# ecpoppenheimer/TensorFlowRayTrace

Hardware: AMD Instinct MI355X
Metric: ray-surface intersection tests/sec (fwd+bwd) (higher is better)
Workload: dtype f32 ray state, f32 filter + f64 decisions

## Files before the change

### include/tfrt_hip.h

```cpp
#ifndef TFRT_HIP_H
#define TFRT_HIP_H

#include <stddef.h>
#include <stdint.h>

#ifdef __cplusplus
extern "C" {
#endif

#define TFRT_VERSION 107

#define TFRT_F32 0
#define TFRT_F64 1
#define TFRT_F16 2

#define TFRT_OPTICAL 0
#define TFRT_STOP 1
#define TFRT_TARGET 2

#define TFRT_CLS_ACTIVE 0
#define TFRT_CLS_FINISHED 1
#define TFRT_CLS_STOPPED 2
#define TFRT_CLS_DEAD 3

#define TFRT_COMPILE_ACTIVE 1u
#define TFRT_COMPILE_FINISHED 2u
#define TFRT_COMPILE_STOPPED 4u
#define TFRT_COMPILE_DEAD 8u

#define TFRT_E_BADARG (-1)
#define TFRT_E_WORKSPACE (-2)
#define TFRT_E_LAUNCH (-3)
#define TFRT_E_UNSUPPORTED (-4)

int tfrt_version(void);
const char* tfrt_strerror(int code);

int tfrt_build_faces_forward(const double* vertices, int64_t n_vertices, const int32_t* faces,
                             int64_t n_faces, double* face_verts, double* norm, void* stream);

int tfrt_build_faces_backward(const double* grad_face_verts, const double* grad_norm,
                              const double* face_verts, const int32_t* faces,
                              const uint8_t* update_mask, int64_t n_faces, int64_t n_vertices,
                              const int32_t* corner_start, const int32_t* corner_list,
                              double* grad_vertices, void* stream);

int tfrt_param_faces_forward(const double* zero_points, const double* vectors,
                             const double* parameters, int64_t n_vertices, const int32_t* faces,
                             int64_t n_faces, double* face_verts, double* norm, void* stream);
int tfrt_param_faces_backward(const double* grad_face_verts, const double* grad_norm,
                              const double* face_verts, const int32_t* faces,
                              const uint8_t* update_mask, const double* vectors, int64_t n_faces,
                              int64_t n_vertices, const int32_t* corner_start,
                              const int32_t* corner_list, double* grad_parameters, void* stream);

#define TFRT_MAX_SURFACES 8
typedef struct tfrt_face_surface {
  const double* zero_points;
  const double* vectors;
  const double* parameters;
  const int32_t* faces;
  int64_t n_vertices, n_faces;
  double* face_verts;
  double* norm;
  const double* copy_from;
} tfrt_face_surface;
typedef struct tfrt_face_surface_grad {
  const double* grad_face_verts;
  const double* grad_norm;
  const double* face_verts;
  const uint8_t* update_mask;
  const double* vectors;
  const int32_t* corner_start;
  const int32_t* corner_list;
  int64_t n_vertices;
  double* grad_parameters;
} tfrt_face_surface_grad;
int tfrt_param_faces_forward_multi(const tfrt_face_surface* surfaces, int32_t n_surfaces,
                                   void* stream);
int tfrt_param_faces_backward_multi(const tfrt_face_surface_grad* surfaces, int32_t n_surfaces,
                                    void* stream);

int tfrt_sgd_process(const void* grad, void* processed, void* param, int64_t n, int32_t dtype,
                     double scale, double clip, double sgd_learning_rate, void* stream);

int tfrt_sgd_process_dev(const void* grad, void* processed, void* param, int64_t n, int32_t dtype,
                         const double* hyper, void* stream);

typedef struct tfrt_goal_pending {
  const double* partial;
  int32_t n_partial;
  const int32_t* n_finished;
  int32_t n_fields;
  double* error_out;
  const int32_t* tests_lo_hi;
  int64_t* tests_total;
  const int32_t* partial_counts;
  int64_t n_faces;
  int32_t* counts_tail;
} tfrt_goal_pending;

int tfrt_sgd_process_multi(int32_t n_tensors, const void* const* grad, void* const* processed,
                           void* const* param, const int64_t* n, const double* hyper,
                           void* stream);

int tfrt_sgd_process_multi_finish(int32_t n_tensors, const void* const* grad,
                                  void* const* processed, void* const* param, const int64_t* n,
                                  const double* hyper, const tfrt_goal_pending* pending,
                                  void* stream);

int tfrt_sgd_momentum_multi(int32_t n_tensors, const void* const* grad, void* const* processed,
                            void* const* param, void* const* velocity, const int64_t* n,
                            const double* hyper, void* stream);

int tfrt_sgd_momentum_multi_finish(int32_t n_tensors, const void* const* grad,
                                   void* const* processed, void* const* param,
                                   void* const* velocity, const int64_t* n, const double* hyper,
                                   const tfrt_goal_pending* pending, void* stream);

int tfrt_adam_multi(int32_t n_tensors, const void* const* grad, void* const* processed,
                    void* const* param, void* const* m, void* const* v, const int64_t* n,
                    const double* hyper, double* state, uint32_t* ticket, void* stream);

int tfrt_adam_multi_finish(int32_t n_tensors, const void* const* grad, void* const* processed,
                           void* const* param, void* const* m, void* const* v, const int64_t* n,
                           const double* hyper, double* state, uint32_t* ticket,
                           const tfrt_goal_pending* pending, void* stream);

int tfrt_csr_matvec(const int64_t* crow_indices, const int64_t* col_indices, const double* values,
                    const double* x, double* y, int64_t n_rows, void* stream);

typedef struct tfrt_scene3d {
  const double* face_verts;
  const int32_t* catagory;
  const int32_t* mat_in;
  const int32_t* mat_out;
  const double* n_in;
  const double* n_out;
  int64_t n_faces;
  const double* n_table;
  int64_t n_table_stride;
  int32_t n_materials;
  double intersect_epsilion;
  double size_epsilion;
  double ray_start_epsilion;
  const uint8_t* face_grad_mask;
  const int32_t* cluster_order;
  int32_t n_table_uniform;
  int32_t deterministic;
  int32_t coherent_rays;
  int32_t coherent_only;
  double* grad_n_in;
  double* grad_n_out;
  double* clear_buffer;
  int64_t clear_count;
  int32_t in_place;
  const int32_t* ray_slot;
  const int32_t* wave_schedule;
} tfrt_scene3d;

typedef struct tfrt_ray_out {
  void* rays;
  int32_t* ray_id;
  int32_t* face;
  int64_t capacity;
} tfrt_ray_out;

size_t tfrt_trace3d_workspace_bytes(int64_t n_rays, int64_t n_faces, int32_t max_passes,
                                    int32_t state_dtype);

#define TFRT_COUNTS_PER_PASS 8
#define TFRT_COUNTS_LEN(max_passes) (8 * ((max_passes) + 1))

int tfrt_trace3d_forward(const void* src_rays, int64_t src_stride, int64_t n_rays,
                         const tfrt_scene3d* scene, double new_ray_length,
                         double dead_ray_length, int32_t max_passes, int32_t state_dtype,
                         uint32_t flags, tfrt_ray_out* finished, tfrt_ray_out* active,
                         tfrt_ray_out* stopped, tfrt_ray_out* dead, void* unfinished,
                         int32_t* unfinished_id, int32_t* counts, void* workspace,
                         size_t workspace_bytes, void* stream);

int tfrt_trace3d_compact(const void* src_rays, int64_t src_stride, int64_t n_rays,
                         double dead_ray_length, int32_t max_passes, int32_t state_dtype,
                         uint32_t flags, tfrt_ray_out* finished, tfrt_ray_out* active,
                         tfrt_ray_out* stopped, tfrt_ray_out* dead, void* unfinished,
                         int32_t* unfinished_id, int32_t* counts, int64_t n_faces,
                         const int32_t* ray_slot, void* workspace, size_t workspace_bytes,
                         void* stream);

int tfrt_trace3d_in_place(const tfrt_scene3d* scene, int64_t n_rays, int32_t max_passes);

int tfrt_trace3d_executed(int64_t n_rays, int64_t n_faces, int32_t max_passes, int32_t state_dtype,
                          const void* workspace, size_t workspace_bytes, int64_t* executed,
                          void* stream);

int tfrt_trace3d_wave_schedule(int64_t n_rays, int64_t n_faces, int32_t max_passes,
                               int32_t state_dtype, const void* workspace, size_t workspace_bytes,
                               int32_t* schedule_out, void* stream);

int tfrt_trace3d_wave_rows(int64_t n_rays, int64_t n_faces, int32_t max_passes, int32_t state_dtype,
                           const void* workspace, size_t workspace_bytes, uint32_t* rows_out,
                           void* stream);

int tfrt_trace3d_backward(const void* src_rays, int64_t src_stride, int64_t n_rays,
                          const tfrt_scene3d* scene, double new_ray_length,
                          double dead_ray_length, int32_t max_passes, int32_t state_dtype,
                          const double* grad_finished, int64_t cap_finished,
                          const double* grad_active, int64_t cap_active,
                          const double* grad_stopped, int64_t cap_stopped,
                          const double* grad_dead, int64_t cap_dead, double* grad_face_verts,
                          double* grad_src_rays, const int32_t* counts, void* workspace,
                          size_t workspace_bytes, void* stream);

size_t tfrt_goal_error3d_workspace_bytes(int64_t capacity);
int tfrt_goal_error3d(const void* finished_rays, int64_t capacity, const int32_t* finished_id,
                      int32_t state_dtype, const int32_t* counts, int32_t max_passes,
                      const int32_t* fields, int32_t n_fields, const double* goal,
                      int64_t goal_stride, int64_t goal_ray_stride, double* grad_finished,
                      double* error_out, double* zero_buffer, int64_t zero_count,
                      int64_t* tests_total, void* workspace, size_t workspace_bytes,
                      void* stream);

int tfrt_goal_error3d_deferred(const void* finished_rays, int64_t capacity,
                               const int32_t* finished_id, int32_t state_dtype,
                               const int32_t* counts, int32_t max_passes, const int32_t* fields,
                               int32_t n_fields, const double* goal, int64_t goal_stride,
                               int64_t goal_ray_stride, double* grad_finished, double* error_out,
                               double* zero_buffer, int64_t zero_count, int64_t* tests_total,
                               void* workspace, size_t workspace_bytes,
                               tfrt_goal_pending* pending, void* stream);
int tfrt_goal_finish(const tfrt_goal_pending* pending, void* stream);

size_t tfrt_density_error_workspace_bytes(int64_t n, int32_t nx, int32_t ny);
int tfrt_density_error(const void* rows, int64_t stride, int64_t n, int32_t state_dtype,
                       const int32_t* mask, int32_t row_x, int32_t row_y, const double* goal,
                       int32_t nx, int32_t ny, double x0, double x1, double sx, double y0,
                       double y1, double sy, double oob_weight, double* grad, int64_t grad_stride,
                       double* error_out, int64_t* hq, int32_t splat_variant, void* workspace,
                       size_t workspace_bytes, void* stream);

int tfrt_density_error_fields(const void* rows, int64_t stride, int64_t n, int32_t state_dtype,
                              int32_t dimension, const int32_t* mask, int32_t field_x,
                              int32_t field_y, const double* goal, int32_t nx, int32_t ny,
                              double x0, double x1, double sx, double y0, double y1, double sy,
                              double oob_weight, double* grad, int64_t grad_stride,
                              double* error_out, int64_t* hq, int32_t splat_variant,
                              void* workspace, size_t workspace_bytes, void* stream);

size_t tfrt_spot_error_workspace_bytes(int64_t n, int32_t n_groups);
int tfrt_spot_error(const void* rows, int64_t stride, int64_t n, int32_t state_dtype,
                    const int32_t* mask, int32_t row_x, int32_t row_y, const int32_t* group,
                    int64_t n_source, const int32_t* perm, int32_t n_groups, double x0, double x1,
                    double qsx, double y0, double y1, double qsy, int32_t qbits,
                    double oob_weight, double* grad, int64_t grad_stride, double* error_out,
                    int64_t* acc, int32_t variant, void* workspace, size_t workspace_bytes,
                    void* stream);

int tfrt_spot_error_fields(const void* rows, int64_t stride, int64_t n, int32_t state_dtype,
                           int32_t dimension, const int32_t* mask, int32_t field_x,
                           int32_t field_y, const int32_t* group, int64_t n_source,
                           const int32_t* perm, int32_t n_groups, double x0, double x1, double qsx,
                           double y0, double y1, double qsy, int32_t qbits, double oob_weight,
                           double* grad, int64_t grad_stride, double* error_out, int64_t* acc,
                           int32_t variant, void* workspace, size_t workspace_bytes, void* stream);

int tfrt_density_error_weighted(const void* rows, int64_t stride, int64_t n, int32_t state_dtype,
                                int32_t dimension, const int32_t* mask, int32_t field_x,
                                int32_t field_y, const double* goal, const double* weight,
                                int64_t n_source, const int32_t* perm, int32_t nx, int32_t ny,
                                double x0, double x1, double sx, double y0, double y1, double sy,
                                double oob_weight, double* grad, int64_t grad_stride,
                                double* error_out, int64_t* hq, int32_t splat_variant,
                                void* workspace, size_t workspace_bytes, void* stream);

size_t tfrt_spot_error_weighted_workspace_bytes(int64_t n, int32_t n_groups);
int tfrt_spot_error_weighted(const void* rows, int64_t stride, int64_t n, int32_t state_dtype,
                             int32_t dimension, const int32_t* mask, int32_t field_x,
                             int32_t field_y, const int32_t* group, const double* weight,
                             int32_t wbits, int64_t n_source, const int32_t* perm,
                             int32_t n_groups, double x0, double x1, double qsx, double y0,
                             double y1, double qsy, int32_t qbits, double oob_weight, double* grad,
                             int64_t grad_stride, double* error_out, int64_t* acc, int32_t variant,
                             void* workspace, size_t workspace_bytes, void* stream);

size_t tfrt_trace3d_backward_goal_workspace_bytes(int64_t n_rays);
int tfrt_trace3d_backward_goal(const void* src_rays, int64_t src_stride, int64_t n_rays,
                               const tfrt_scene3d* scene, double new_ray_length,
                               double dead_ray_length, int32_t max_passes, int32_t state_dtype,
                               const tfrt_ray_out* finished, const int32_t* fields,
                               int32_t n_fields, const double* goal, int64_t goal_stride,
                               int64_t goal_ray_stride, double* error_out, int64_t* tests_total,
                               void* goal_workspace, size_t goal_workspace_bytes,
                               tfrt_goal_pending* pending, const double* grad_active,
                               int64_t cap_active, const double* grad_stopped,
                               int64_t cap_stopped, const double* grad_dead, int64_t cap_dead,
                               double* grad_face_verts, double* grad_src_rays,
                               const int32_t* counts, void* workspace, size_t workspace_bytes,
                               void* stream);

#define TFRT_PROF_INTERSECT 0
#define TFRT_PROF_REACT 1
#define TFRT_PROF_BACKWARD 2
#define TFRT_PROF_ACCUMULATE 3
int tfrt_profile_enable(int enable);
int tfrt_profile_read(float* ms, int32_t max_records);
int tfrt_profile_read_kind(int32_t kind, float* ms, int32_t max_records);


size_t tfrt_intersect3d_workspace_bytes(int64_t n_rays, int64_t n_faces);
int tfrt_intersect3d(const void* rays, int64_t stride, int64_t n_rays, int32_t state_dtype,
                     const double* face_verts, int64_t n_faces, double intersect_epsilion,
// ... 279 lines not shown
```

### tensorflowraytrace_amd/_lib.py

```python
import ctypes
import os
import typing

HERE = os.path.dirname(os.path.abspath(__file__))
LIB_PATH = os.environ.get("TFRT_LIB_PATH") or os.path.join(HERE, "libtfrt_hip.so")

ABI_VERSION = 107
F32, F64, F16 = 0, 1, 2
OPTICAL, STOP, TARGET = 0, 1, 2
CLS_ACTIVE, CLS_FINISHED, CLS_STOPPED, CLS_DEAD = 0, 1, 2, 3
COMPILE_ACTIVE, COMPILE_FINISHED, COMPILE_STOPPED, COMPILE_DEAD = 1, 2, 4, 8
COUNTS_PER_PASS = 8

c_i32, c_i64, c_f64, c_u32 = ctypes.c_int32, ctypes.c_int64, ctypes.c_double, ctypes.c_uint32
c_vp, c_sz = ctypes.c_void_p, ctypes.c_size_t


class Scene3D(ctypes.Structure):
    _fields_ = [
        ("face_verts", c_vp), ("catagory", c_vp), ("mat_in", c_vp), ("mat_out", c_vp),
        ("n_in", c_vp), ("n_out", c_vp), ("n_faces", c_i64),
        ("n_table", c_vp), ("n_table_stride", c_i64), ("n_materials", c_i32),
        ("intersect_epsilion", c_f64), ("size_epsilion", c_f64), ("ray_start_epsilion", c_f64),
        ("face_grad_mask", c_vp), ("cluster_order", c_vp), ("n_table_uniform", c_i32),
        ("deterministic", c_i32), ("coherent_rays", c_i32), ("coherent_only", c_i32),
        ("grad_n_in", c_vp), ("grad_n_out", c_vp), ("clear_buffer", c_vp), ("clear_count", c_i64),
        ("in_place", c_i32), ("ray_slot", c_vp), ("wave_schedule", c_vp),
    ]


class Scene2D(ctypes.Structure):
    _fields_ = [
        ("seg", c_vp), ("seg_cat", c_vp), ("seg_mat_in", c_vp), ("seg_mat_out", c_vp),
        ("seg_n_in", c_vp), ("seg_n_out", c_vp), ("n_segments", c_i64),
        ("arc", c_vp), ("arc_cat", c_vp), ("arc_mat_in", c_vp), ("arc_mat_out", c_vp),
        ("arc_n_in", c_vp), ("arc_n_out", c_vp), ("n_arcs", c_i64),
        ("n_table", c_vp), ("n_table_stride", c_i64), ("n_materials", c_i32),
        ("intersect_epsilion", c_f64), ("size_epsilion", c_f64), ("ray_start_epsilion", c_f64),
        ("finite_tir_gradient", c_i32),
        ("grad_seg_n_in", c_vp), ("grad_seg_n_out", c_vp),
        ("grad_arc_n_in", c_vp), ("grad_arc_n_out", c_vp),
        ("deterministic", c_i32),
    ]


MAX_SURFACES = 8


class FaceSurface(ctypes.Structure):
    _fields_ = [("zero_points", ctypes.c_void_p), ("vectors", ctypes.c_void_p),
                ("parameters", ctypes.c_void_p), ("faces", ctypes.c_void_p),
                ("n_vertices", ctypes.c_int64), ("n_faces", ctypes.c_int64),
                ("face_verts", ctypes.c_void_p), ("norm", ctypes.c_void_p),
                ("copy_from", ctypes.c_void_p)]


class FaceSurfaceGrad(ctypes.Structure):
    _fields_ = [("grad_face_verts", ctypes.c_void_p), ("grad_norm", ctypes.c_void_p),
                ("face_verts", ctypes.c_void_p), ("update_mask", ctypes.c_void_p),
                ("vectors", ctypes.c_void_p), ("corner_start", ctypes.c_void_p),
                ("corner_list", ctypes.c_void_p), ("n_vertices", ctypes.c_int64),
                ("grad_parameters", ctypes.c_void_p)]


class GoalPending(ctypes.Structure):
    _fields_ = [("partial", ctypes.c_void_p), ("n_partial", ctypes.c_int32),
                ("n_finished", ctypes.c_void_p), ("n_fields", ctypes.c_int32),
                ("error_out", ctypes.c_void_p), ("tests_lo_hi", ctypes.c_void_p),
                ("tests_total", ctypes.c_void_p), ("partial_counts", ctypes.c_void_p),
                ("n_faces", ctypes.c_int64), ("counts_tail", ctypes.c_void_p)]


class RayOut(ctypes.Structure):
    _fields_ = [("rays", c_vp), ("ray_id", c_vp), ("face", c_vp), ("capacity", c_i64)]


class PointsProgram(ctypes.Structure):
    _fields_ = [("kind", c_i32), ("stream", c_i32), ("count", c_i64), ("table", c_vp),
                ("p", c_f64 * 4), ("scale", c_f64 * 3), ("quat", c_f64 * 4), ("shift", c_f64 * 3),
                ("has_scale", c_i32), ("has_quat", c_i32), ("has_shift", c_i32),
                ("reserved0", c_i32), ("seed", ctypes.c_uint64), ("epoch", c_vp),
                ("x_count", c_i32), ("y_count", c_i32), ("density", c_vp),
                ("rank_density", c_vp), ("rank_scale", c_f64)]


class Source3DProgram(ctypes.Structure):
    _fields_ = [("kind", c_i32), ("swap", c_i32), ("a", PointsProgram), ("b", PointsProgram),
                ("center", c_f64 * 3), ("quat", c_f64 * 4), ("has_quat", c_i32),
                ("reserved0", c_i32), ("ray_length", c_f64), ("n_rays", c_i64),
                ("pool", c_vp), ("pool_count", c_i64), ("sigma_start", c_f64 * 3),
                ("sigma_end", c_f64 * 3), ("pool_downsample", c_i32), ("pool_stream", c_i32),
                ("pool_seed", ctypes.c_uint64), ("pool_epoch", c_vp)]


class SamplesProgram(ctypes.Structure):
    _fields_ = [("kind", c_i32), ("stream", c_i32), ("count", c_i64), ("table", c_vp),
                ("columns", c_i32), ("reserved0", c_i32), ("lo", c_f64), ("hi", c_f64),
                ("rank_scale", c_f64), ("p0", c_f64 * 2), ("p1", c_f64 * 2),
                ("seed", ctypes.c_uint64), ("epoch", c_vp)]


class Source2DProgram(ctypes.Structure):
    _fields_ = [("kind", c_i32), ("swap", c_i32), ("a", SamplesProgram), ("b", SamplesProgram),
                ("center", c_f64 * 2), ("central_angle", c_f64), ("rot", c_f64 * 2),
                ("ray_length", c_f64),
                ("n_rays", c_i64),
                ("pool", c_vp), ("pool_count", c_i64), ("sigma_start", c_f64 * 2),
                ("sigma_end", c_f64 * 2), ("pool_downsample", c_i32), ("pool_stream", c_i32),
                ("pool_seed", ctypes.c_uint64), ("pool_epoch", c_vp)]


PTS_TABLE, PTS_CIRCLE, PTS_SQUARE, PTS_SPHERE_UNIFORM, PTS_SPHERE_LAMBERT = 0, 1, 2, 3, 4
PTS_DENSITY = 5
SRC_APERTURE, SRC_POINT, SRC_ANGULAR, SRC_POOL = 0, 1, 2, 3
SMP_TABLE, SMP_UNIFORM_ANGLE, SMP_LAMBERT_ANGLE, SMP_BEAM, SMP_APERTURE_POINTS = 0, 1, 2, 3, 4

_P = ctypes.POINTER

SIGNATURES = {
    "tfrt_version": (c_i32, []),
    "tfrt_strerror": (ctypes.c_char_p, [c_i32]),
    "tfrt_profile_enable": (c_i32, [c_i32]),
    "tfrt_profile_read": (c_i32, [c_vp, c_i32]),
    "tfrt_profile_read_kind": (c_i32, [c_i32, c_vp, c_i32]),
    "tfrt_build_faces_forward": (c_i32, [c_vp, c_i64, c_vp, c_i64, c_vp, c_vp, c_vp]),
    "tfrt_build_faces_backward": (c_i32, [c_vp, c_vp, c_vp, c_vp, c_vp, c_i64, c_i64, c_vp, c_vp,
                                          c_vp, c_vp]),
    "tfrt_param_faces_forward": (c_i32, [c_vp, c_vp, c_vp, c_i64, c_vp, c_i64, c_vp, c_vp, c_vp]),
    "tfrt_param_faces_backward": (c_i32, [c_vp, c_vp, c_vp, c_vp, c_vp, c_vp, c_i64, c_i64, c_vp,
                                          c_vp, c_vp, c_vp]),
    "tfrt_param_faces_forward_multi": (c_i32, [c_vp, c_i32, c_vp]),
    "tfrt_param_faces_backward_multi": (c_i32, [c_vp, c_i32, c_vp]),
    "tfrt_line_intersect": (c_i32, [c_i64, c_i64, c_vp, c_i64, c_i64, c_vp, c_i64, c_i64, c_f64,
                                    c_vp, c_vp, c_vp, c_vp, c_vp, c_vp]),
    "tfrt_line_triangle_intersect": (c_i32, [c_i64, c_i64, c_vp, c_i64, c_i64, c_vp, c_i64, c_i64,
                                             c_f64, c_vp, c_vp, c_vp, c_vp, c_vp, c_vp, c_vp, c_vp]),
    "tfrt_line_circle_intersect": (c_i32, [c_i64, c_i64, c_vp, c_i64, c_i64, c_vp, c_i64, c_i64,
                                           c_f64, c_vp, c_vp, c_vp, c_vp, c_vp]),
    "tfrt_sgd_process": (c_i32, [c_vp, c_vp, c_vp, c_i64, c_i32, c_f64, c_f64, c_f64, c_vp]),
    "tfrt_sgd_process_dev": (c_i32, [c_vp, c_vp, c_vp, c_i64, c_i32, c_vp, c_vp]),
    "tfrt_sgd_process_multi": (c_i32, [c_i32, c_vp, c_vp, c_vp, c_vp, c_vp, c_vp]),
    "tfrt_sgd_process_multi_finish": (c_i32, [c_i32, c_vp, c_vp, c_vp, c_vp, c_vp, c_vp, c_vp]),
    "tfrt_sgd_momentum_multi": (c_i32, [c_i32, c_vp, c_vp, c_vp, c_vp, c_vp, c_vp, c_vp]),
    "tfrt_sgd_momentum_multi_finish": (c_i32, [c_i32, c_vp, c_vp, c_vp, c_vp, c_vp, c_vp, c_vp,
                                               c_vp]),
    "tfrt_adam_multi": (c_i32, [c_i32, c_vp, c_vp, c_vp, c_vp, c_vp, c_vp, c_vp, c_vp, c_vp, c_vp]),
    "tfrt_adam_multi_finish": (c_i32, [c_i32, c_vp, c_vp, c_vp, c_vp, c_vp, c_vp, c_vp, c_vp, c_vp,
                                       c_vp, c_vp]),
    "tfrt_csr_matvec": (c_i32, [c_vp, c_vp, c_vp, c_vp, c_vp, c_i64, c_vp]),
    "tfrt_trace3d_workspace_bytes": (c_sz, [c_i64, c_i64, c_i32, c_i32]),
    "tfrt_trace3d_forward": (c_i32, [
        c_vp, c_i64, c_i64, _P(Scene3D), c_f64, c_f64, c_i32, c_i32, c_u32,
        _P(RayOut), _P(RayOut), _P(RayOut), _P(RayOut), c_vp, c_vp, c_vp, c_vp, c_sz, c_vp]),
    "tfrt_trace3d_compact": (c_i32, [
        c_vp, c_i64, c_i64, c_f64, c_i32, c_i32, c_u32,
        _P(RayOut), _P(RayOut), _P(RayOut), _P(RayOut), c_vp, c_vp, c_vp, c_i64, c_vp, c_vp, c_sz,
        c_vp]),
    "tfrt_trace3d_in_place": (c_i32, [_P(Scene3D), c_i64, c_i32]),
    "tfrt_trace3d_executed": (c_i32, [c_i64, c_i64, c_i32, c_i32, c_vp, c_sz, c_vp, c_vp]),
    "tfrt_trace3d_wave_schedule": (c_i32, [c_i64, c_i64, c_i32, c_i32, c_vp, c_sz, c_vp, c_vp]),
    "tfrt_trace3d_wave_rows": (c_i32, [c_i64, c_i64, c_i32, c_i32, c_vp, c_sz, c_vp, c_vp]),
    "tfrt_trace3d_backward": (c_i32, [
        c_vp, c_i64, c_i64, _P(Scene3D), c_f64, c_f64, c_i32, c_i32,
        c_vp, c_i64, c_vp, c_i64, c_vp, c_i64, c_vp, c_i64, c_vp, c_vp, c_vp, c_vp, c_sz, c_vp]),
    "tfrt_goal_error3d_workspace_bytes": (c_sz, [c_i64]),
    "tfrt_goal_error3d": (c_i32, [c_vp, c_i64, c_vp, c_i32, c_vp, c_i32, c_vp, c_i32, c_vp, c_i64,
                                  c_i64, c_vp, c_vp, c_vp, c_i64, c_vp, c_vp, c_sz, c_vp]),
    "tfrt_goal_error3d_deferred": (c_i32, [c_vp, c_i64, c_vp, c_i32, c_vp, c_i32, c_vp, c_i32, c_vp, c_i64,
                                  c_i64, c_vp, c_vp, c_vp, c_i64, c_vp, c_vp, c_sz, c_vp, c_vp]),
    "tfrt_goal_finish": (c_i32, [c_vp, c_vp]),
    "tfrt_density_error_workspace_bytes": (c_sz, [c_i64, c_i32, c_i32]),
    "tfrt_density_error": (c_i32, [
        c_vp, c_i64, c_i64, c_i32, c_vp, c_i32, c_i32, c_vp, c_i32, c_i32,
        c_f64, c_f64, c_f64, c_f64, c_f64, c_f64, c_f64,
        c_vp, c_i64, c_vp, c_vp, c_i32, c_vp, c_sz, c_vp]),
    "tfrt_density_error_fields": (c_i32, [
        c_vp, c_i64, c_i64, c_i32, c_i32, c_vp, c_i32, c_i32, c_vp, c_i32, c_i32,
        c_f64, c_f64, c_f64, c_f64, c_f64, c_f64, c_f64,
        c_vp, c_i64, c_vp, c_vp, c_i32, c_vp, c_sz, c_vp]),
    "tfrt_spot_error_workspace_bytes": (c_sz, [c_i64, c_i32]),
    "tfrt_spot_error": (c_i32, [
        c_vp, c_i64, c_i64, c_i32, c_vp, c_i32, c_i32,
        c_vp, c_i64, c_vp, c_i32,
        c_f64, c_f64, c_f64, c_f64, c_f64, c_f64, c_i32, c_f64,
        c_vp, c_i64, c_vp, c_vp, c_i32, c_vp, c_sz, c_vp]),
    "tfrt_spot_error_fields": (c_i32, [
        c_vp, c_i64, c_i64, c_i32, c_i32, c_vp, c_i32, c_i32,
        c_vp, c_i64, c_vp, c_i32,
        c_f64, c_f64, c_f64, c_f64, c_f64, c_f64, c_i32, c_f64,
        c_vp, c_i64, c_vp, c_vp, c_i32, c_vp, c_sz, c_vp]),
    "tfrt_density_error_weighted": (c_i32, [
        c_vp, c_i64, c_i64, c_i32, c_i32, c_vp, c_i32, c_i32, c_vp,
        c_vp, c_i64, c_vp, c_i32, c_i32,
        c_f64, c_f64, c_f64, c_f64, c_f64, c_f64, c_f64,
        c_vp, c_i64, c_vp, c_vp, c_i32, c_vp, c_sz, c_vp]),
    "tfrt_spot_error_weighted_workspace_bytes": (c_sz, [c_i64, c_i32]),
    "tfrt_spot_error_weighted": (c_i32, [
        c_vp, c_i64, c_i64, c_i32, c_i32, c_vp, c_i32, c_i32,
        c_vp, c_vp, c_i32, c_i64, c_vp, c_i32,
        c_f64, c_f64, c_f64, c_f64, c_f64, c_f64, c_i32, c_f64,
        c_vp, c_i64, c_vp, c_vp, c_i32, c_vp, c_sz, c_vp]),
    "tfrt_trace3d_backward_goal_workspace_bytes": (c_sz, [c_i64]),
    "tfrt_trace3d_backward_goal": (c_i32, [
        c_vp, c_i64, c_i64, c_vp, c_f64, c_f64, c_i32, c_i32,
        c_vp, c_vp, c_i32, c_vp, c_i64, c_i64, c_vp, c_vp, c_vp, c_sz, c_vp,
        c_vp, c_i64, c_vp, c_i64, c_vp, c_i64, c_vp, c_vp, c_vp, c_vp, c_sz, c_vp]),
    "tfrt_intersect3d_workspace_bytes": (c_sz, [c_i64, c_i64]),
    "tfrt_intersect3d": (c_i32, [
        c_vp, c_i64, c_i64, c_i32, c_vp, c_i64, c_f64, c_f64, c_f64,
        c_vp, c_vp, c_vp, c_vp, c_vp, c_vp, c_vp, c_vp, c_vp, c_sz, c_vp]),
    "tfrt_snell3d": (c_i32, [c_i64] + [c_vp] * 9 + [c_f64, c_vp, c_vp]),
    "tfrt_snell2d": (c_i32, [c_i64] + [c_vp] * 7 + [c_f64, c_vp, c_vp]),
    "tfrt_selftest_f64": (c_i32, [c_i32, c_i64, c_vp, c_vp, c_vp, c_vp]),
    "tfrt_segment_intersection": (c_i32, [
        c_vp, c_i64, c_i64, c_i32, c_vp, c_i64, c_f64, c_f64, c_f64,
# ... 102 lines not shown
```

### tensorflowraytrace_amd/csrc/tfrt_faces.hip

```cpp
#include "tfrt_common.h"

namespace tfrt {

__global__ __launch_bounds__(BLOCK) void k_build_faces(const double* __restrict__ vertices,
                                                       int64_t V, const int32_t* __restrict__ faces,
                                                       int64_t F, double* __restrict__ fverts,
                                                       double* __restrict__ norm) {
  const int64_t f = (int64_t)blockIdx.x * BLOCK + threadIdx.x;
  if (f >= F) return;
  double P[9];
#pragma unroll
  for (int c = 0; c < 3; ++c) {
    int64_t v = faces[3 * f + c];
    if (v < 0 || v >= V) v = 0;
#pragma unroll
    for (int k = 0; k < 3; ++k) P[3 * c + k] = vertices[3 * v + k];
  }
#pragma unroll
  for (int q = 0; q < 9; ++q) fverts[9 * f + q] = P[q];
  if (norm != nullptr) {
    double N[3], C[3], clen;
    face_normal(P, N, C, &clen);
    norm[3 * f] = N[0];
    norm[3 * f + 1] = N[1];
    norm[3 * f + 2] = N[2];
  }
}

__global__ __launch_bounds__(BLOCK) void k_build_faces_bwd(
    const double* __restrict__ g_fverts, const double* __restrict__ g_norm,
    const double* __restrict__ fverts, const int32_t* __restrict__ faces,
    const uint8_t* __restrict__ mask, int64_t F, int64_t V, double* __restrict__ g_vertices) {
  const int64_t f = (int64_t)blockIdx.x * BLOCK + threadIdx.x;
  if (f >= F) return;
  double g[9];
#pragma unroll
  for (int q = 0; q < 9; ++q) g[q] = g_fverts ? g_fverts[9 * f + q] : 0.0;
  if (g_norm != nullptr) {
    double P[9], N[3], C[3], clen;
#pragma unroll
    for (int q = 0; q < 9; ++q) P[q] = fverts[9 * f + q];
    face_normal(P, N, C, &clen);
    const double gn[3] = {g_norm[3 * f], g_norm[3 * f + 1], g_norm[3 * f + 2]};
    const double nn = dot3(N, gn);
    double Cb[3];
    for (int k = 0; k < 3; ++k) Cb[k] = (gn[k] - N[k] * nn) / clen;
    const double A[3] = {P[3] - P[0], P[4] - P[1], P[5] - P[2]};
    const double B[3] = {P[6] - P[3], P[7] - P[4], P[8] - P[5]};
    double Ab[3], Bb[3];
    cross3(B, Cb, Ab);
    cross3(Cb, A, Bb);
    for (int k = 0; k < 3; ++k) {
      g[k] -= Ab[k];
      g[3 + k] += Ab[k] - Bb[k];
      g[6 + k] += Bb[k];
    }
  }
#pragma unroll
  for (int c = 0; c < 3; ++c) {
    if (mask != nullptr && mask[3 * f + c] == 0) continue;
    const int64_t v = faces[3 * f + c];
    if (v < 0 || v >= V) continue;
#pragma unroll
    for (int k = 0; k < 3; ++k) {
      const double x = g[3 * c + k];
      if (x != 0.0) unsafeAtomicAdd(g_vertices + 3 * v + k, x);
    }
  }
}

#pragma clang fp contract(off)
__global__ __launch_bounds__(BLOCK) void k_param_faces(
    const double* __restrict__ zero, const double* __restrict__ vectors,
    const double* __restrict__ params, int64_t V, const int32_t* __restrict__ faces, int64_t F,
    double* __restrict__ fverts, double* __restrict__ norm) {
  const int64_t f = (int64_t)blockIdx.x * BLOCK + threadIdx.x;
  if (f >= F) return;
  double P[9];
#pragma unroll
  for (int c = 0; c < 3; ++c) {
    int64_t v = faces[3 * f + c];
    if (v < 0 || v >= V) v = 0;
    const double p = params[v];
#pragma unroll
    for (int k = 0; k < 3; ++k) {
      const double step = p * vectors[3 * v + k];
      P[3 * c + k] = zero[3 * v + k] + step;
    }
  }
#pragma unroll
  for (int q = 0; q < 9; ++q) fverts[9 * f + q] = P[q];
  if (norm != nullptr) {
    double N[3], C[3], clen;
    face_normal(P, N, C, &clen);
    norm[3 * f] = N[0];
    norm[3 * f + 1] = N[1];
    norm[3 * f + 2] = N[2];
  }
}

__device__ inline void face_grad(const double* __restrict__ g_fverts,
                                 const double* __restrict__ g_norm,
                                 const double* __restrict__ fverts, int64_t f, double g[9]) {
#pragma unroll
  for (int q = 0; q < 9; ++q) g[q] = g_fverts ? g_fverts[9 * f + q] : 0.0;
  if (g_norm != nullptr) {
    double P[9], N[3], C[3], clen;
#pragma unroll
    for (int q = 0; q < 9; ++q) P[q] = fverts[9 * f + q];
    face_normal(P, N, C, &clen);
    const double gn[3] = {g_norm[3 * f], g_norm[3 * f + 1], g_norm[3 * f + 2]};
    const double nn = dot3(N, gn);
    double Cb[3];
    for (int k = 0; k < 3; ++k) Cb[k] = (gn[k] - N[k] * nn) / clen;
    const double A[3] = {P[3] - P[0], P[4] - P[1], P[5] - P[2]};
    const double B[3] = {P[6] - P[3], P[7] - P[4], P[8] - P[5]};
    double Ab[3], Bb[3];
    cross3(B, Cb, Ab);
    cross3(Cb, A, Bb);
    for (int k = 0; k < 3; ++k) {
      g[k] -= Ab[k];
      g[3 + k] += Ab[k] - Bb[k];
      g[6 + k] += Bb[k];
    }
  }
}

__global__ __launch_bounds__(BLOCK) void k_param_faces_bwd(
    const double* __restrict__ g_fverts, const double* __restrict__ g_norm,
    const double* __restrict__ fverts, const int32_t* __restrict__ faces,
    const uint8_t* __restrict__ mask, const double* __restrict__ vectors, int64_t F, int64_t V,
    double* __restrict__ g_params) {
  const int64_t f = (int64_t)blockIdx.x * BLOCK + threadIdx.x;
  if (f >= F) return;
  double g[9];
  face_grad(g_fverts, g_norm, fverts, f, g);
#pragma unroll
  for (int c = 0; c < 3; ++c) {
    if (mask != nullptr && mask[3 * f + c] == 0) continue;
    const int64_t v = faces[3 * f + c];
    if (v < 0 || v >= V) continue;
    const double x = g[3 * c] * vectors[3 * v] + g[3 * c + 1] * vectors[3 * v + 1] +
                     g[3 * c + 2] * vectors[3 * v + 2];
    if (x != 0.0) unsafeAtomicAdd(g_params + v, x);
  }
}

constexpr int GATHER_LANES = 8;

__global__ __launch_bounds__(BLOCK) void k_build_faces_bwd_gather(
    const double* __restrict__ g_fverts, const double* __restrict__ g_norm,
    const double* __restrict__ fverts, const uint8_t* __restrict__ mask,
    const int32_t* __restrict__ corner_start, const int32_t* __restrict__ corner_list, int64_t V,
    double* __restrict__ g_vertices) {
  const int64_t t = (int64_t)blockIdx.x * BLOCK + threadIdx.x;
  const int64_t v = t / GATHER_LANES;
  const int sub = (int)(t % GATHER_LANES);
  double acc[3] = {0.0, 0.0, 0.0};
  if (v < V) {
    for (int q = corner_start[v] + sub; q < corner_start[v + 1]; q += GATHER_LANES) {
      const int fc = corner_list[q], f = fc / 3, c = fc - 3 * f;
      if (mask != nullptr && mask[fc] == 0) continue;
      double g[9];
      face_grad(g_fverts, g_norm, fverts, f, g);
      acc[0] += g[3 * c];
      acc[1] += g[3 * c + 1];
      acc[2] += g[3 * c + 2];
    }
  }
#pragma unroll
  for (int d = GATHER_LANES / 2; d > 0; d >>= 1)
    for (int k = 0; k < 3; ++k) acc[k] += __shfl_xor(acc[k], d, 64);
  if (v < V && sub == 0) {
    g_vertices[3 * v] = acc[0];
    g_vertices[3 * v + 1] = acc[1];
    g_vertices[3 * v + 2] = acc[2];
  }
}

__global__ __launch_bounds__(BLOCK) void k_param_faces_bwd_gather(
    const double* __restrict__ g_fverts, const double* __restrict__ g_norm,
    const double* __restrict__ fverts, const uint8_t* __restrict__ mask,
    const double* __restrict__ vectors, const int32_t* __restrict__ corner_start,
    const int32_t* __restrict__ corner_list, int64_t V, double* __restrict__ g_params) {
  const int64_t t = (int64_t)blockIdx.x * BLOCK + threadIdx.x;
  const int64_t v = t / GATHER_LANES;
  const int sub = (int)(t % GATHER_LANES);
  double acc = 0.0;
  if (v < V) {
    for (int q = corner_start[v] + sub; q < corner_start[v + 1]; q += GATHER_LANES) {
      const int fc = corner_list[q], f = fc / 3, c = fc - 3 * f;
      if (mask != nullptr && mask[fc] == 0) continue;
      double g[9];
      face_grad(g_fverts, g_norm, fverts, f, g);
      acc += g[3 * c] * vectors[3 * v] + g[3 * c + 1] * vectors[3 * v + 1] +
             g[3 * c + 2] * vectors[3 * v + 2];
    }
  }
#pragma unroll
  for (int d = GATHER_LANES / 2; d > 0; d >>= 1) acc += __shfl_xor(acc, d, 64);
  if (v < V && sub == 0) g_params[v] = acc;
}

struct FaceSurfaces {
  int32_t count;
  int32_t first_block[TFRT_MAX_SURFACES + 1];
  tfrt_face_surface s[TFRT_MAX_SURFACES];
};
struct FaceSurfaceGrads {
  int32_t count;
  int32_t first_block[TFRT_MAX_SURFACES + 1];
  tfrt_face_surface_grad s[TFRT_MAX_SURFACES];
};

#pragma clang fp contract(off)
__global__ __launch_bounds__(BLOCK) void k_param_faces_multi(FaceSurfaces b) {
  int k = 0;
  while (k + 1 < b.count && (int)blockIdx.x >= b.first_block[k + 1]) ++k;
  const tfrt_face_surface& u = b.s[k];
  const int64_t f = (int64_t)((int)blockIdx.x - b.first_block[k]) * BLOCK + threadIdx.x;
  if (f >= u.n_faces) return;
  if (u.copy_from != nullptr) {
#pragma unroll
    for (int q = 0; q < 9; ++q) u.face_verts[9 * f + q] = u.copy_from[9 * f + q];
    return;
  }
  double P[9];
#pragma unroll
  for (int c = 0; c < 3; ++c) {
    int64_t v = u.faces[3 * f + c];
    if (v < 0 || v >= u.n_vertices) v = 0;
    const double p = u.parameters[v];
#pragma unroll
    for (int q = 0; q < 3; ++q) {
      const double step = p * u.vectors[3 * v + q];
      P[3 * c + q] = u.zero_points[3 * v + q] + step;
    }
  }
#pragma unroll
  for (int q = 0; q < 9; ++q) u.face_verts[9 * f + q] = P[q];
  if (u.norm != nullptr) {
    double N[3], C[3], clen;
    face_normal(P, N, C, &clen);
    u.norm[3 * f] = N[0];
    u.norm[3 * f + 1] = N[1];
    u.norm[3 * f + 2] = N[2];
  }
}

__global__ __launch_bounds__(BLOCK) void k_param_faces_bwd_gather_multi(FaceSurfaceGrads b) {
  int k = 0;
  while (k + 1 < b.count && (int)blockIdx.x >= b.first_block[k + 1]) ++k;
  const tfrt_face_surface_grad& u = b.s[k];
  const int64_t t = (int64_t)((int)blockIdx.x - b.first_block[k]) * BLOCK + threadIdx.x;
  const int64_t v = t / GATHER_LANES;
  const int sub = (int)(t % GATHER_LANES);
  double acc = 0.0;
  if (v < u.n_vertices) {
    for (int q = u.corner_start[v] + sub; q < u.corner_start[v + 1]; q += GATHER_LANES) {
      const int fc = u.corner_list[q], f = fc / 3, c = fc - 3 * f;
      if (u.update_mask != nullptr && u.update_mask[fc] == 0) continue;
      double g[9];
      face_grad(u.grad_face_verts, u.grad_norm, u.face_verts, f, g);
      acc += g[3 * c] * u.vectors[3 * v] + g[3 * c + 1] * u.vectors[3 * v + 1] +
             g[3 * c + 2] * u.vectors[3 * v + 2];
    }
  }
#pragma unroll
  for (int d = GATHER_LANES / 2; d > 0; d >>= 1) acc += __shfl_xor(acc, d, 64);
  if (v < u.n_vertices && sub == 0) u.grad_parameters[v] = acc;
}

__global__ __launch_bounds__(BLOCK) void k_snell3d(int64_t n, const double* xs, const double* ys,
                                                   const double* zs, const double* xe,
                                                   const double* ye, const double* ze,
                                                   const double* norm, const double* n_in,
                                                   const double* n_out, double L, double* out) {
  const int64_t i = (int64_t)blockIdx.x * BLOCK + threadIdx.x;
  if (i >= n) return;
  const double s[3] = {xs[i], ys[i], zs[i]}, h[3] = {xe[i], ye[i], ze[i]};
  const double N[3] = {norm[3 * i], norm[3 * i + 1], norm[3 * i + 2]};
  const Snell3 f = snell3d(s, h, N, n_in[i], n_out[i]);
  for (int k = 0; k < 3; ++k) {
    out[k * n + i] = h[k];
    out[(3 + k) * n + i] = advance(h[k], L, f.w[k]);
  }
}

__global__ __launch_bounds__(BLOCK) void k_snell2d(int64_t n, const double* xs, const double* ys,
                                                   const double* xe, const double* ye,
                                                   const double* norm, const double* n_in,
                                                   const double* n_out, double L, double* out) {
  const int64_t i = (int64_t)blockIdx.x * BLOCK + threadIdx.x;
  if (i >= n) return;
  const double a = snell2d_angle(xs[i], ys[i], xe[i], ye[i], norm[i], n_in[i], n_out[i]);
  out[i] = xe[i];
  out[n + i] = ye[i];
  out[2 * n + i] = advance(xe[i], L, cos(a));
  out[3 * n + i] = advance(ye[i], L, sin(a));
}

__global__ __launch_bounds__(BLOCK) void k_selftest_f64(int op, int64_t n, const double* a,
                                                        const double* b, double* out) {
  const int64_t i = (int64_t)blockIdx.x * BLOCK + threadIdx.x;
  if (i >= n) return;
  const double x = a[i], y = b ? b[i] : 0.0;
  double r;
  switch (op) {
    case TFRT_SELFTEST_DIV: r = x / y; break;
    case TFRT_SELFTEST_SQRT: r = sqrt(x); break;
    case TFRT_SELFTEST_RSQRT: r = 1.0 / sqrt(x); break;
    case TFRT_SELFTEST_MULADD: r = advance(x, y, y); break;
    case TFRT_SELFTEST_ADJ_RCP: r = adj_rcp(x); break;
    case TFRT_SELFTEST_ADJ_RSQRT: r = adj_rsqrt(x); break;
    default: r = 0.0;
  }
  out[i] = r;
}

}

using namespace tfrt;

extern "C" {

int tfrt_version(void) { return TFRT_VERSION; }

const char* tfrt_strerror(int code) {
  switch (code) {
    case 0: return "ok";
    case TFRT_E_BADARG: return "bad argument (null pointer, negative size, stride < n, or too many faces)";
    case TFRT_E_WORKSPACE: return "workspace too small (query tfrt_*_workspace_bytes)";
    case TFRT_E_LAUNCH: return "HIP kernel launch failed";
    case TFRT_E_UNSUPPORTED: return "unsupported state dtype or option";
    default: return "unknown tfrt error";
  }
}

int tfrt_build_faces_forward(const double* vertices, int64_t n_vertices, const int32_t* faces,
                             int64_t n_faces, double* face_verts, double* norm, void* stream) {
  if (n_faces < 0 || n_vertices < 0) return TFRT_E_BADARG;
  if (n_faces == 0) return 0;
  if (!vertices || !faces || !face_verts || n_vertices == 0) return TFRT_E_BADARG;
  hipLaunchKernelGGL(k_build_faces, dim3(cdiv(n_faces, BLOCK)), dim3(BLOCK), 0,
                     static_cast<hipStream_t>(stream), vertices, n_vertices, faces, n_faces,
                     face_verts, norm);
  return hipGetLastError() == hipSuccess ? 0 : TFRT_E_LAUNCH;
}

int tfrt_build_faces_backward(const double* grad_face_verts, const double* grad_norm,
                              const double* face_verts, const int32_t* faces,
                              const uint8_t* update_mask, int64_t n_faces, int64_t n_vertices,
                              const int32_t* corner_start, const int32_t* corner_list,
                              double* grad_vertices, void* stream) {
  if (n_faces < 0 || n_vertices < 0) return TFRT_E_BADARG;
  if (n_faces == 0) return 0;
  if (!faces || !grad_vertices || (!grad_face_verts && !grad_norm) ||
      (grad_norm && !face_verts) || ((corner_start == nullptr) != (corner_list == nullptr)))
    return TFRT_E_BADARG;
  if (corner_start != nullptr) {
    hipLaunchKernelGGL(k_build_faces_bwd_gather, dim3(cdiv(n_vertices * GATHER_LANES, BLOCK)),
                       dim3(BLOCK), 0,
                       static_cast<hipStream_t>(stream), grad_face_verts, grad_norm, face_verts,
                       update_mask, corner_start, corner_list, n_vertices, grad_vertices);
    return hipGetLastError() == hipSuccess ? 0 : TFRT_E_LAUNCH;
  }
  hipLaunchKernelGGL(k_build_faces_bwd, dim3(cdiv(n_faces, BLOCK)), dim3(BLOCK), 0,
                     static_cast<hipStream_t>(stream), grad_face_verts, grad_norm, face_verts,
                     faces, update_mask, n_faces, n_vertices, grad_vertices);
  return hipGetLastError() == hipSuccess ? 0 : TFRT_E_LAUNCH;
}

int tfrt_param_faces_forward(const double* zero_points, const double* vectors,
                             const double* parameters, int64_t n_vertices, const int32_t* faces,
                             int64_t n_faces, double* face_verts, double* norm, void* stream) {
  if (n_faces < 0 || n_vertices < 0) return TFRT_E_BADARG;
  if (n_faces == 0) return 0;
  if (!zero_points || !vectors || !parameters || !faces || !face_verts || n_vertices == 0)
    return TFRT_E_BADARG;
  hipLaunchKernelGGL(k_param_faces, dim3(cdiv(n_faces, BLOCK)), dim3(BLOCK), 0,
                     static_cast<hipStream_t>(stream), zero_points, vectors, parameters,
                     n_vertices, faces, n_faces, face_verts, norm);
  return hipGetLastError() == hipSuccess ? 0 : TFRT_E_LAUNCH;
}

int tfrt_param_faces_backward(const double* grad_face_verts, const double* grad_norm,
                              const double* face_verts, const int32_t* faces,
                              const uint8_t* update_mask, const double* vectors, int64_t n_faces,
                              int64_t n_vertices, const int32_t* corner_start,
                              const int32_t* corner_list, double* grad_parameters, void* stream) {
  if (n_faces < 0 || n_vertices < 0) return TFRT_E_BADARG;
  if (n_faces == 0) return 0;
  if (!faces || !vectors || !grad_parameters || (!grad_face_verts && !grad_norm) ||
      (grad_norm && !face_verts) || ((corner_start == nullptr) != (corner_list == nullptr)))
    return TFRT_E_BADARG;
  if (corner_start != nullptr) {
    hipLaunchKernelGGL(k_param_faces_bwd_gather, dim3(cdiv(n_vertices * GATHER_LANES, BLOCK)),
                       dim3(BLOCK), 0,
                       static_cast<hipStream_t>(stream), grad_face_verts, grad_norm, face_verts,
                       update_mask, vectors, corner_start, corner_list, n_vertices,
                       grad_parameters);
    return hipGetLastError() == hipSuccess ? 0 : TFRT_E_LAUNCH;
  }
  hipLaunchKernelGGL(k_param_faces_bwd, dim3(cdiv(n_faces, BLOCK)), dim3(BLOCK), 0,
                     static_cast<hipStream_t>(stream), grad_face_verts, grad_norm, face_verts,
                     faces, update_mask, vectors, n_faces, n_vertices, grad_parameters);
  return hipGetLastError() == hipSuccess ? 0 : TFRT_E_LAUNCH;
}

int tfrt_param_faces_forward_multi(const tfrt_face_surface* surfaces, int32_t n_surfaces,
                                   void* stream) {
  if (n_surfaces < 0 || n_surfaces > TFRT_MAX_SURFACES || (n_surfaces > 0 && !surfaces))
    return TFRT_E_BADARG;
  FaceSurfaces b;
  int blocks = 0;
  for (int k = 0; k < TFRT_MAX_SURFACES; ++k) {
    b.first_block[k] = blocks;
    if (k >= n_surfaces) {
      b.s[k] = tfrt_face_surface{};
      continue;
    }
    const tfrt_face_surface& u = surfaces[k];
    if (u.n_faces < 0 || u.n_vertices < 0) return TFRT_E_BADARG;
    if (u.n_faces > 0) {
      if (!u.face_verts) return TFRT_E_BADARG;
      if (!u.copy_from &&
          (!u.zero_points || !u.vectors || !u.parameters || !u.faces || u.n_vertices == 0))
        return TFRT_E_BADARG;
    }
    b.s[k] = u;
    blocks += cdiv(u.n_faces, BLOCK);
  }
  b.first_block[TFRT_MAX_SURFACES] = blocks;
  b.count = n_surfaces;
  if (blocks == 0) return 0;
  hipLaunchKernelGGL(k_param_faces_multi, dim3(blocks), dim3(BLOCK), 0,
                     static_cast<hipStream_t>(stream), b);
  return hipGetLastError() == hipSuccess ? 0 : TFRT_E_LAUNCH;
}

int tfrt_param_faces_backward_multi(const tfrt_face_surface_grad* surfaces, int32_t n_surfaces,
                                    void* stream) {
  if (n_surfaces < 0 || n_surfaces > TFRT_MAX_SURFACES || (n_surfaces > 0 && !surfaces))
    return TFRT_E_BADARG;
  FaceSurfaceGrads b;
  int blocks = 0;
  for (int k = 0; k < TFRT_MAX_SURFACES; ++k) {
    b.first_block[k] = blocks;
    if (k >= n_surfaces) {
      b.s[k] = tfrt_face_surface_grad{};
      continue;
    }
    const tfrt_face_surface_grad& u = surfaces[k];
    if (u.n_vertices < 0) return TFRT_E_BADARG;
    if (u.n_vertices > 0 &&
        (!u.vectors || !u.grad_parameters || !u.corner_start || !u.corner_list ||
         (!u.grad_face_verts && !u.grad_norm) || (u.grad_norm && !u.face_verts)))
      return TFRT_E_BADARG;
    b.s[k] = u;
    blocks += cdiv(u.n_vertices * GATHER_LANES, BLOCK);
  }
  b.first_block[TFRT_MAX_SURFACES] = blocks;
  b.count = n_surfaces;
  if (blocks == 0) return 0;
  hipLaunchKernelGGL(k_param_faces_bwd_gather_multi, dim3(blocks), dim3(BLOCK), 0,
                     static_cast<hipStream_t>(stream), b);
  return hipGetLastError() == hipSuccess ? 0 : TFRT_E_LAUNCH;
}

int tfrt_snell3d(int64_t n, const double* x_start, const double* y_start, const double* z_start,
                 const double* x_end, const double* y_end, const double* z_end,
                 const double* norm, const double* n_in, const double* n_out,
                 double new_ray_length, double* out6, void* stream) {
  if (n < 0) return TFRT_E_BADARG;
  if (n == 0) return 0;
  if (!x_start || !y_start || !z_start || !x_end || !y_end || !z_end || !norm || !n_in ||
      !n_out || !out6)
    return TFRT_E_BADARG;
  hipLaunchKernelGGL(k_snell3d, dim3(cdiv(n, BLOCK)), dim3(BLOCK), 0,
                     static_cast<hipStream_t>(stream), n, x_start, y_start, z_start, x_end, y_end,
                     z_end, norm, n_in, n_out, new_ray_length, out6);
  return hipGetLastError() == hipSuccess ? 0 : TFRT_E_LAUNCH;
}

int tfrt_snell2d(int64_t n, const double* x_start, const double* y_start, const double* x_end,
                 const double* y_end, const double* norm, const double* n_in,
                 const double* n_out, double new_ray_length, double* out4, void* stream) {
  if (n < 0) return TFRT_E_BADARG;
  if (n == 0) return 0;
  if (!x_start || !y_start || !x_end || !y_end || !norm || !n_in || !n_out || !out4)
    return TFRT_E_BADARG;
  hipLaunchKernelGGL(k_snell2d, dim3(cdiv(n, BLOCK)), dim3(BLOCK), 0,
                     static_cast<hipStream_t>(stream), n, x_start, y_start, x_end, y_end, norm,
                     n_in, n_out, new_ray_length, out4);
  return hipGetLastError() == hipSuccess ? 0 : TFRT_E_LAUNCH;
}

int tfrt_selftest_f64(int op, int64_t n, const double* a, const double* b, double* out,
                      void* stream) {
  if (n < 0 || op < TFRT_SELFTEST_DIV || op > TFRT_SELFTEST_ADJ_RSQRT) return TFRT_E_BADARG;
  if (n == 0) return 0;
  if (!a || !out || (!b && (op == TFRT_SELFTEST_DIV || op == TFRT_SELFTEST_MULADD)))
    return TFRT_E_BADARG;
  hipLaunchKernelGGL(k_selftest_f64, dim3(cdiv(n, BLOCK)), dim3(BLOCK), 0,
                     static_cast<hipStream_t>(stream), op, n, a, b, out);
  return hipGetLastError() == hipSuccess ? 0 : TFRT_E_LAUNCH;
}

}
```

### tensorflowraytrace_amd/csrc/tfrt_trace3d.hip

```cpp
#include <vector>

#include <type_traits>
#include "tfrt_common.h"
#include "goal_finish.h"
#include "wave_schedule.h"

namespace tfrt {

constexpr int TILE = 512;
constexpr int KC = 24;

constexpr int ERR_CAPACITY = 1;


__global__ __launch_bounds__(BLOCK) void k_center(const double* __restrict__ fverts, int M,
                                                  double* __restrict__ c0, int32_t* nrays0, int n,
                                                  int32_t* tail8, unsigned int* scan_ticket) {
  if (nrays0 != nullptr) {
    if (threadIdx.x == 0) *nrays0 = n;
    if (threadIdx.x < 8) tail8[threadIdx.x] = 0;
    if (threadIdx.x == 0 && scan_ticket != nullptr) *scan_ticket = 0u;
  }
  __shared__ double red[WAVES][3];
  __shared__ double ctr[3];
// ... 2366 lines not shown
      int at = base[cls] + rank;
      for (int w = 0; w < wave; ++w) at += wcnt[w][cls];
      if (at < G) sched[at] = g;
    }
    __syncthreads();
    if (tid < WAVE_SCHED_CLASSES) {
      int t = 0;
      for (int w = 0; w < 16; ++w) t += wcnt[w][tid];
      base[tid] += t;
    }
    __syncthreads();
  }
}

__global__ __launch_bounds__(64) void k_inplace_count(const uint8_t* __restrict__ rec_cls, int64_t n,
                                                      int N, int P, const int32_t* __restrict__ slot_of,
                                                      uint32_t* __restrict__ wcount, int wstride) {
  const int lane = threadIdx.x, qwave = blockIdx.x;
  const int r = qwave * 64 + lane;
  bool alive = r < N;
  const int64_t i = alive ? slot_of[r] : 0;
  int p = 0;
  for (; p < P; ++p) {
    if (__ballot(alive) == 0ull) break;
    const int cls = alive ? ((int)rec_cls[(size_t)p * n + i] & 3) : -1;
    uint32_t word = 0u;
#pragma unroll
    for (int c = 0; c < 4; ++c) word |= (uint32_t)__popcll(__ballot(cls == c)) << (8 * c);
    if (lane == 0) wcount[(size_t)p * wstride + qwave] = word;
    if (cls != CLS_ACTIVE) alive = false;
  }
  for (int pp = p + lane; pp < P; pp += 64) wcount[(size_t)pp * wstride + qwave] = 0u;
}

template <typename T>
struct GatherArgs {
  const T* src;
  int64_t src_stride;
  int32_t N, P, bundle, nwaves;
  const T* rays_ws;
  const int32_t* rec_tri;
  const double* rec_t;
  const uint8_t* rec_cls;
  int32_t* rec_slot;
  int64_t n;
  const int4* wbase;
  int32_t wstride;
  const int32_t* slot_of;
  const int32_t* counts;
  uint32_t flags;
  double dead_len;
  tfrt_ray_out fin, act, stp, dead;
  T* unfinished;
  int32_t* unfinished_id;
  int32_t* err;
};

template <typename T>
__global__ __launch_bounds__(64) void k_inplace_gather(GatherArgs<T> a) {
  const int lane = threadIdx.x, qwave = blockIdx.x;
  const int q = qwave * a.bundle + lane;
  const bool has = lane < a.bundle && q < a.N;
  const int rid = has ? q : 0;
  const int64_t i = a.slot_of != nullptr ? a.slot_of[rid] : rid;
  bool alive = has, ok = true;
  int p = 0;
  for (; p < a.P; ++p) {
    if (__ballot(alive) == 0ull) break;
    const size_t at = (size_t)p * a.n + i;
    const int cls = alive ? ((int)a.rec_cls[at] & 3) : -1;
    int rank = 0;
#pragma unroll
    for (int c = 0; c < 4; ++c) {
      const unsigned long long m = __ballot(cls == c);
      if (cls == c) rank = rank_below(m);
    }
    if (alive) {
      const int4 wb = a.wbase[(size_t)p * a.wstride + qwave];
      const int in_pass = (cls == 0 ? wb.x : (cls == 1 ? wb.y : (cls == 2 ? wb.z : wb.w))) + rank;
      const int64_t gslot = (int64_t)a.counts[(size_t)p * TFRT_COUNTS_PER_PASS + 4 + cls] + in_pass;
      const uint32_t want = cls == CLS_DEAD       ? TFRT_COMPILE_DEAD
                            : cls == CLS_FINISHED ? TFRT_COMPILE_FINISHED
                            : cls == CLS_STOPPED  ? TFRT_COMPILE_STOPPED
                                                  : TFRT_COMPILE_ACTIVE;
      if (a.flags & want) {
        a.rec_slot[at] = (int32_t)gslot;
        const T* rin = p == 0 ? a.src : a.rays_ws + (size_t)(p - 1) * 6 * a.n;
        const int64_t sin = p == 0 ? a.src_stride : a.n;
        double s[3], e[3];
        load_ray3(rin, sin, i, s, e);
        if (cls == CLS_DEAD) {
          double e2[3] = {e[0], e[1], e[2]};
          if (a.dead_len != 0.0)
            for (int k = 0; k < 3; ++k) e2[k] = advance_between(s[k], a.dead_len, e[k]);
          ok = emit<T>(a.dead, gslot, s, e2, rid, -1) && ok;
        } else {
          const int tri = a.rec_tri[at];
          double h[3];
          hit_point(s, e, a.rec_t[at], h);
          const tfrt_ray_out& o = cls == CLS_FINISHED ? a.fin : (cls == CLS_STOPPED ? a.stp : a.act);
          ok = emit<T>(o, gslot, s, h, rid, tri) && ok;
        }
      }
      if (cls != CLS_ACTIVE) alive = false;
    }
  }
  if (!ok) atomicOr(a.err, ERR_CAPACITY);
  if (p == a.P && a.P > 0 && a.unfinished != nullptr) {
    const unsigned long long m = __ballot(alive);
    if (alive) {
      const int slot = a.wbase[(size_t)(a.P - 1) * a.wstride + qwave].x + rank_below(m);
      const T* rin = a.rays_ws + (size_t)(a.P - 1) * 6 * a.n;
#pragma unroll
      for (int k = 0; k < 6; ++k) a.unfinished[(int64_t)k * a.N + slot] = rin[k * a.n + i];
      if (a.unfinished_id != nullptr) a.unfinished_id[slot] = rid;
    }
  }
}


template <typename G>
__device__ __forceinline__ void add6(const G* g, int64_t cap, int64_t slot, double a[3],
                                     double b[3]) {
  if (g == nullptr) return;
  for (int k = 0; k < 3; ++k) {
    a[k] += static_cast<double>(g[k * cap + slot]);
    b[k] += static_cast<double>(g[(3 + k) * cap + slot]);
  }
}

template <typename T>
struct SweepStore {
  using type = float;
};
template <>
struct SweepStore<double> {
  using type = double;
};

template <typename T>
__device__ __forceinline__ int backward_ray(
    int i, const T* __restrict__ rays_in, int64_t stride_in, const int32_t* __restrict__ ray_id_in,
    const int32_t* __restrict__ rec_tri, const double* __restrict__ rec_t,
    const uint8_t* __restrict__ rec_cls, const int32_t* __restrict__ rec_slot,
    const int32_t* __restrict__ pass_counts, const tfrt_scene3d& sc, double L, double dead_len,
    const typename SweepStore<T>::type* __restrict__ g_child, int64_t child_stride,
    const double* __restrict__ g_fin, int64_t cap_fin, const double* __restrict__ g_act,
    int64_t cap_act, const double* __restrict__ g_stp, int64_t cap_stp,
    const double* __restrict__ g_dead, int64_t cap_dead,
    typename SweepStore<T>::type* __restrict__ g_out, double* __restrict__ g_src_out,
    int64_t out_stride, double gP[9]);


constexpr int WSUM_SLOTS = 32, WSUM_CELLS = 592;
__device__ __forceinline__ constexpr int wsum_stride(int copies) {
  return WSUM_SLOTS * 9 * 2 / copies + 2;
}
static_assert(8 * wsum_stride(8) <= WSUM_CELLS && 4 * wsum_stride(4) <= WSUM_CELLS &&
              2 * wsum_stride(2) <= WSUM_CELLS, "wacc holds every tier");

__device__ __forceinline__ void wsum_clear(double* wacc) {
  for (int k = 2 * (threadIdx.x & 63); k < WSUM_CELLS; k += 128)
    *reinterpret_cast<double2*>(wacc + k) = make_double2(0.0, 0.0);
  wave_fence();
}
template <int COPIES>
__device__ __forceinline__ void wsum_fold(double* wacc, const int32_t* wface, int K, int lane,
                                          double* __restrict__ g_fverts) {
  for (int k = lane; k < K; k += 64) {
    double* w = wacc + k;
    double v = w[0];
#pragma unroll
    for (int c = 1; c < COPIES; ++c) v += w[c * wsum_stride(COPIES)];
#pragma unroll
    for (int c = 0; c < COPIES; ++c) w[c * wsum_stride(COPIES)] = 0.0;
    if (v != 0.0) {
      const int f = k / 9;
      unsafeAtomicAdd(g_fverts + 9 * (int64_t)wface[f] + (k - 9 * f), v);
    }
  }
}
__device__ __forceinline__ void wave_face_sums(int tri, const double gP[9], double* wacc,
                                               int32_t* wface, double* __restrict__ g_fverts) {
  const int lane = threadIdx.x & 63;
  int slot = -1, ns = 0;
  unsigned long long todo = __ballot(tri >= 0);
  if (todo == 0ull) return;
  while (todo != 0ull && ns < WSUM_SLOTS) {
    const int leader = __ffsll((long long)todo) - 1;
    const int k = __builtin_amdgcn_readlane(tri, leader);
    const bool mine = tri == k;
    if (mine) slot = ns;
    if (lane == leader) wface[ns] = k;
    ++ns;
    todo &= ~__ballot(mine);
  }
  const int copies = ns <= 8 ? 8 : (ns <= 16 ? 4 : 2);
  if (tri >= 0) {
    if (slot >= 0) {
      double* w = &wacc[(lane & (copies - 1)) * wsum_stride(copies) + slot * 9];
#pragma unroll
      for (int c = 0; c < 9; ++c)
        if (gP[c] != 0.0) unsafeAtomicAdd(w + c, gP[c]);
    } else {
      double* gp = g_fverts + 9 * (int64_t)tri;
#pragma unroll
      for (int c = 0; c < 9; ++c)
        if (gP[c] != 0.0) unsafeAtomicAdd(gp + c, gP[c]);
    }
  }
  wave_fence();
  if (copies == 8) wsum_fold<8>(wacc, wface, ns * 9, lane, g_fverts);
  else if (copies == 4) wsum_fold<4>(wacc, wface, ns * 9, lane, g_fverts);
  else wsum_fold<2>(wacc, wface, ns * 9, lane, g_fverts);
  wave_fence();
}

template <typename T, int BW>
__global__ __launch_bounds__(64 * BW) void k_backward3d(
    const T* __restrict__ rays_in, int64_t stride_in, const int32_t* __restrict__ n_ptr,
    const int32_t* __restrict__ ray_id_in, const int32_t* __restrict__ rec_tri,
    const double* __restrict__ rec_t, const uint8_t* __restrict__ rec_cls,
    const int32_t* __restrict__ rec_slot, const int32_t* __restrict__ pass_counts,
    tfrt_scene3d sc, double L, double dead_len,
    const typename SweepStore<T>::type* __restrict__ g_child, int64_t child_stride,
    const double* __restrict__ g_fin, int64_t cap_fin, const double* __restrict__ g_act,
    int64_t cap_act, const double* __restrict__ g_stp, int64_t cap_stp,
    const double* __restrict__ g_dead, int64_t cap_dead,
    typename SweepStore<T>::type* __restrict__ g_out, double* __restrict__ g_src_out,
    int64_t out_stride, double* __restrict__ g_fverts,
    typename SweepStore<T>::type* __restrict__ stash_g, int32_t* __restrict__ stash_face,
    int wave_sums) {
  const int n = *n_ptr;
  const int q0 = blockIdx.x * (64 * BW) + threadIdx.x;
  const int i = q0;
  if (wave_sums) {
    if ((q0 & ~63) >= n) return;
    __shared__ __align__(16) double wacc[BW][WSUM_CELLS];
    __shared__ int32_t wface[BW][WSUM_SLOTS];
    const int wave = threadIdx.x >> 6;
    wsum_clear(wacc[wave]);
    double gP[9];
    int tri = -1;
    if (i < n)
      tri = backward_ray<T>(i, rays_in, stride_in, ray_id_in, rec_tri, rec_t, rec_cls, rec_slot,
                            pass_counts, sc, L, dead_len, g_child, child_stride, g_fin, cap_fin,
                            g_act, cap_act, g_stp, cap_stp, g_dead, cap_dead, g_out, g_src_out,
                            out_stride, gP);
    wave_face_sums(tri, gP, wacc[wave], wface[wave], g_fverts);
    return;
  }
  if (i >= n) return;
  double gP[9];
  const int tri = backward_ray<T>(i, rays_in, stride_in, ray_id_in, rec_tri, rec_t, rec_cls,
                                  rec_slot, pass_counts, sc, L, dead_len, g_child, child_stride,
                                  g_fin, cap_fin, g_act, cap_act, g_stp, cap_stp, g_dead, cap_dead,
                                  g_out, g_src_out, out_stride, gP);
  if (stash_face != nullptr) {
    stash_face[i] = tri;
    if (tri >= 0) {
      using S = typename SweepStore<T>::type;
      S* o = stash_g + 9 * (int64_t)i;
#pragma unroll
      for (int c = 0; c < 9; ++c) o[c] = static_cast<S>(gP[c]);
    }
    return;
  }
  if (tri >= 0) {
    double* gp = g_fverts + 9 * (int64_t)tri;
#pragma unroll
    for (int c = 0; c < 9; ++c) {
      if (gP[c] != 0.0) unsafeAtomicAdd(gp + c, gP[c]);
    }
  }
}

constexpr int FACE_WINDOW = 2048;

template <typename S>
__global__ __launch_bounds__(1024) void k_face_accumulate(
    const int32_t* __restrict__ nrays, int passes, int64_t pass_stride,
    const int32_t* __restrict__ stash_face, const S* __restrict__ stash_g, int chunk, int M,
    double* __restrict__ g_fverts) {
  __shared__ double acc[FACE_WINDOW * 9];
  const int lo = blockIdx.x * chunk;
  if (lo >= nrays[0]) return;
  const int w0 = blockIdx.y * FACE_WINDOW;
  const int w1 = min(M, w0 + FACE_WINDOW);
  for (int k = threadIdx.x; k < FACE_WINDOW * 9; k += 1024) acc[k] = 0.0;
  __syncthreads();
  for (int p = 0; p < passes; ++p) {
    const int hi = min(nrays[p], lo + chunk);
    const int32_t* __restrict__ face = stash_face + (int64_t)p * pass_stride;
    const S* __restrict__ terms = stash_g + 9 * (int64_t)p * pass_stride;
    constexpr int U = 4;
    for (int base = lo + threadIdx.x; base < hi; base += 1024 * U) {
      int t[U];
#pragma unroll
      for (int u = 0; u < U; ++u) {
        const int i = base + u * 1024;
        t[u] = i < hi ? face[i] : -1;
      }
      double g[U][9];
#pragma unroll
      for (int u = 0; u < U; ++u) {
        if (t[u] >= w0 && t[u] < w1) {
          const S* src = terms + 9 * (int64_t)(base + u * 1024);
#pragma unroll
          for (int c = 0; c < 9; ++c) g[u][c] = static_cast<double>(src[c]);
        }
      }
#pragma unroll
      for (int u = 0; u < U; ++u) {
        if (t[u] >= w0 && t[u] < w1) {
          double* a = acc + 9 * (t[u] - w0);
#pragma unroll
          for (int c = 0; c < 9; ++c)
            if (g[u][c] != 0.0) unsafeAtomicAdd(a + c, g[u][c]);
        }
      }
    }
  }
  __syncthreads();
  for (int k = threadIdx.x; k < (w1 - w0) * 9; k += 1024) {
    const double v = acc[k];
    if (v != 0.0) unsafeAtomicAdd(g_fverts + 9 * (int64_t)w0 + k, v);
  }
}

constexpr int FIXED_BITS = 40;

template <typename S>
__global__ __launch_bounds__(BLOCK) void k_stash_absmax(const int32_t* __restrict__ n_ptr,
                                                        const int32_t* __restrict__ stash_face,
                                                        const S* __restrict__ stash_g,
                                                        unsigned long long* __restrict__ maxbits) {
  const int n = *n_ptr;
  const int i = blockIdx.x * BLOCK + threadIdx.x;
  double m = 0.0;
  if (i < n && stash_face[i] >= 0) {
    const S* g = stash_g + 9 * (int64_t)i;
#pragma unroll
    for (int c = 0; c < 9; ++c) {
      const double a = fabs(static_cast<double>(g[c]));
      if (a > m && a < INFINITY) m = a;
    }
  }
#pragma unroll
  for (int d = 32; d > 0; d >>= 1) m = fmax(m, __shfl_xor(m, d, 64));
  if (lane_id() == 0 && m > 0.0) atomicMax(maxbits, (unsigned long long)__double_as_longlong(m));
}

__device__ __forceinline__ double fixed_scale(unsigned long long maxbits) {
  if (maxbits == 0ull) return 0.0;
  int e;
  (void)frexp(__longlong_as_double((long long)maxbits), &e);
  int shift = FIXED_BITS - e;
  if (shift > 1000) shift = 1000;
  return ldexp(1.0, shift);
}

template <typename S>
__global__ __launch_bounds__(BLOCK) void k_face_accumulate_fixed(
    const int32_t* __restrict__ n_ptr, const int32_t* __restrict__ stash_face,
    const S* __restrict__ stash_g, const unsigned long long* __restrict__ maxbits,
    unsigned long long* __restrict__ acc, uint8_t* __restrict__ flag) {
  const int n = *n_ptr;
  const int i = blockIdx.x * BLOCK + threadIdx.x;
  if (i >= n) return;
  const int f = stash_face[i];
  if (f < 0) return;
  const double scale = fixed_scale(*maxbits);
  const S* g = stash_g + 9 * (int64_t)i;
#pragma unroll
  for (int c = 0; c < 9; ++c) {
    const double x = static_cast<double>(g[c]);
    if (!(fabs(x) < INFINITY)) {
      flag[9 * (int64_t)f + c] = 1;
    } else {
      const long long q = llrint(x * scale);
      if (q != 0) atomicAdd(acc + 9 * (int64_t)f + c, (unsigned long long)q);
    }
  }
}

__global__ __launch_bounds__(BLOCK) void k_fixed_finish(int64_t m9,
                                                        const unsigned long long* __restrict__ max_this,
                                                        unsigned long long* __restrict__ max_next,
                                                        unsigned long long* __restrict__ acc,
                                                        uint8_t* __restrict__ flag,
                                                        double* __restrict__ g_fverts) {
  const int64_t i = (int64_t)blockIdx.x * BLOCK + threadIdx.x;
  const double scale = fixed_scale(*max_this);
  if (i < m9) {
    const long long q = (long long)acc[i];
    if (flag[i] != 0) {
      g_fverts[i] = __builtin_nan("");
    } else if (q != 0) {
      g_fverts[i] += (double)q / scale;
    }
    acc[i] = 0ull;
    flag[i] = 0;
  }
  if (i == 0) *max_next = 0ull;
}

template <typename T, bool GN = true>
__device__ __forceinline__ int backward_core(
    int i, int tape, int slot, const T* __restrict__ rays_in, int64_t stride_in,
    const int32_t* __restrict__ ray_id_in, const int32_t* __restrict__ rec_tri,
    const double* __restrict__ rec_t, const int32_t* __restrict__ pass_counts,
    const tfrt_scene3d& sc, double L, double dead_len, bool child_pass, const double child[6],
    const double* seed_fin,
    const double* __restrict__ g_fin, int64_t cap_fin, const double* __restrict__ g_act,
    int64_t cap_act, const double* __restrict__ g_stp, int64_t cap_stp,
    const double* __restrict__ g_dead, int64_t cap_dead, double gs[3], double ge[3],
    double gP[9], int tri_known = -2, const double* __restrict__ feta = nullptr,
    bool slot_global = false) {
  int face_out = -1;
  const int cls = tape & 3;
  double s[3], e[3];
  load_ray3(rays_in, stride_in, i, s, e);
  for (int k = 0; k < 3; ++k) gs[k] = ge[k] = 0.0;
  double P[9], t_rec = 0.0, n_in = 1.0, n_out = 1.0;
  int tri = tri_known;
  auto load_face = [&](bool with_indices) {
    const double* fp = sc.face_verts + 9 * (int64_t)tri;
#pragma unroll
    for (int q = 0; q < 9; ++q) P[q] = fp[q];
    t_rec = rec_t[i];
    if (with_indices) {
      if (feta != nullptr) {
        n_in = feta[4 * (int64_t)tri + 2];
        n_out = feta[4 * (int64_t)tri + 3];
      } else {
        face_indices(sc, tri, ray_id_in ? ray_id_in[i] : i, &n_in, &n_out);
      }
    }
  };
  const bool early = tri_known >= 0 && cls != CLS_DEAD;
  if (early) load_face(child_pass && cls == CLS_ACTIVE);

  if (cls == CLS_DEAD) {
    if (g_dead != nullptr) {
      double a[3] = {0, 0, 0}, b[3] = {0, 0, 0};
      add6(g_dead, cap_dead, slot, a, b);
      const double dl = (dead_len != 0.0) ? dead_len : 1.0;
      for (int k = 0; k < 3; ++k) {
        gs[k] = a[k] + (1.0 - dl) * b[k];
        ge[k] = dl * b[k];
      }
    }
  } else {
    double g_s[3] = {0, 0, 0}, g_h[3] = {0, 0, 0}, g_ce[3] = {0, 0, 0};
    bool has_child = false;
    if (cls == CLS_FINISHED) {
      if (seed_fin != nullptr) {
        for (int k = 0; k < 3; ++k) {
          g_s[k] += seed_fin[k];
          g_h[k] += seed_fin[3 + k];
        }
      } else {
        add6(g_fin, cap_fin, slot, g_s, g_h);
      }
    } else if (cls == CLS_STOPPED) {
      add6(g_stp, cap_stp, slot, g_s, g_h);
    } else {
      if (g_act != nullptr)
        add6(g_act, cap_act, (slot_global ? 0 : (int64_t)pass_counts[4 + CLS_ACTIVE]) + slot, g_s, g_h);
      if (child_pass) {
        has_child = true;
        for (int k = 0; k < 3; ++k) {
          g_h[k] += child[k];
          g_ce[k] += child[3 + k];
        }
      }
    }
    bool nz = has_child;
    for (int k = 0; k < 3; ++k) nz = nz || g_s[k] != 0.0 || g_h[k] != 0.0;
    if (nz) {
      if (!early) {
        if (tri_known < -1) tri = rec_tri[i];
        load_face(has_child);
      }
      double gn[2];
      const bool want_n = GN && has_child && sc.grad_n_in != nullptr && sc.n_table == nullptr;
      const int branch = ((tape & TAPE_INTERNAL) ? 1 : 0) | ((tape & TAPE_REFLECT) ? 2 : 0);
      adjoint3d(s, e, P, t_rec, has_child, n_in, n_out, L, g_s, g_h, g_ce, gs, ge, gP, gn, branch,
                want_n);
      if (want_n) {
        if (gn[0] != 0.0) unsafeAtomicAdd(sc.grad_n_in + tri, gn[0]);
        if (gn[1] != 0.0) unsafeAtomicAdd(sc.grad_n_out + tri, gn[1]);
      }
      if (sc.face_grad_mask == nullptr || sc.face_grad_mask[tri] != 0) face_out = tri;
    }
  }
  return face_out;
}

template <bool FIN = true, bool CHILD = true>
__device__ __forceinline__ int backward_core_loaded(
    int tape, int tri, bool child_pass, const double s[3], const double e[3], const double P[9],
    double t_rec, double n_a, double n_b, bool face_wanted, double L, const double child[6],
    const double seed[6], double gs[3], double ge[3], double gP[9]) {
  int face_out = -1;
  const int cls = tape & 3;
  for (int k = 0; k < 3; ++k) gs[k] = ge[k] = 0.0;
  if (cls != CLS_DEAD) {
    double g_s[3] = {0, 0, 0}, g_h[3] = {0, 0, 0}, g_ce[3] = {0, 0, 0};
    bool has_child = false;
    if (FIN && cls == CLS_FINISHED) {
      for (int k = 0; k < 3; ++k) {
        g_s[k] += seed[k];
        g_h[k] += seed[3 + k];
      }
    } else if (CHILD && cls == CLS_ACTIVE && child_pass) {
      has_child = true;
      for (int k = 0; k < 3; ++k) {
        g_h[k] += child[k];
        g_ce[k] += child[3 + k];
      }
    }
    bool nz = has_child;
    for (int k = 0; k < 3; ++k) nz = nz || g_s[k] != 0.0 || g_h[k] != 0.0;
    if (nz) {
      const int branch = ((tape & TAPE_INTERNAL) ? 1 : 0) | ((tape & TAPE_REFLECT) ? 2 : 0);
      const double ratios[2] = {n_a, n_b};
      adjoint3d(s, e, P, t_rec, has_child, 1.0, 1.0, L, g_s, g_h, g_ce, gs, ge, gP, nullptr,
                branch, false, face_wanted, ratios);
      if (face_wanted) face_out = tri;
    }
  }
  return face_out;
}

template <typename T>
__device__ __forceinline__ int backward_ray(
    int i, const T* __restrict__ rays_in, int64_t stride_in, const int32_t* __restrict__ ray_id_in,
    const int32_t* __restrict__ rec_tri, const double* __restrict__ rec_t,
    const uint8_t* __restrict__ rec_cls, const int32_t* __restrict__ rec_slot,
    const int32_t* __restrict__ pass_counts, const tfrt_scene3d& sc, double L, double dead_len,
    const typename SweepStore<T>::type* __restrict__ g_child, int64_t child_stride,
    const double* __restrict__ g_fin, int64_t cap_fin, const double* __restrict__ g_act,
    int64_t cap_act, const double* __restrict__ g_stp, int64_t cap_stp,
    const double* __restrict__ g_dead, int64_t cap_dead,
    typename SweepStore<T>::type* __restrict__ g_out, double* __restrict__ g_src_out,
    int64_t out_stride, double gP[9]) {
  const int tape = rec_cls[i];
  const int slot = rec_slot[i];
  double child[6] = {0, 0, 0, 0, 0, 0};
  const bool child_pass = g_child != nullptr;
  if (child_pass && (tape & 3) == CLS_ACTIVE) {
    for (int k = 0; k < 6; ++k) child[k] = static_cast<double>(g_child[k * child_stride + slot]);
  }
  double gs[3], ge[3];
  const int face_out = backward_core<T>(i, tape, slot, rays_in, stride_in, ray_id_in, rec_tri,
                                        rec_t, pass_counts, sc, L, dead_len, child_pass, child,
                                        nullptr, g_fin, cap_fin, g_act, cap_act, g_stp, cap_stp, g_dead,
                                        cap_dead, gs, ge, gP);
  if (g_out != nullptr) {
    using G = typename SweepStore<T>::type;
    for (int k = 0; k < 3; ++k) {
      g_out[k * out_stride + i] = static_cast<G>(gs[k]);
      g_out[(3 + k) * out_stride + i] = static_cast<G>(ge[k]);
    }
  } else if (g_src_out != nullptr) {
    for (int k = 0; k < 3; ++k) {
      g_src_out[k * out_stride + i] = gs[k];
      g_src_out[(3 + k) * out_stride + i] = ge[k];
    }
  }
  return face_out;
}

constexpr int CHAIN_MAXP = 8;

template <typename T>
struct ChainArgs {
  const T* src;
  int64_t src_stride;
  const T* rays_ws;
  const int32_t* nrays;
  const int32_t* rayid;
  const int32_t* rec_tri;
  const int32_t* rec_slot;
  const double* rec_t;
  const uint8_t* rec_cls;
  const int32_t* counts;
  int64_t n;
  int32_t P;
  double L, dead_len;
  const double *g_fin, *g_act, *g_stp, *g_dead;
  int64_t cap_fin, cap_act, cap_stp, cap_dead;
  double* g_src;
  int64_t N;
  double* g_fverts;
  const T* fin_rays;
  int64_t fin_cap;
  GoalFields gf;
  const double* goal;
  int64_t goal_stride, goal_ray_stride;
  double* partial;
  int32_t* partial_cnt;
  const double* feta;
  int32_t inplace;
  int32_t chain_in_lds;
};

#ifndef TFRT_CHAIN_WAVES
#define TFRT_CHAIN_WAVES 4
#endif
template <typename T, int BW, bool GOAL, bool GN>
__global__ __launch_bounds__(64 * BW)
__attribute__((amdgpu_waves_per_eu(TFRT_CHAIN_WAVES, TFRT_CHAIN_WAVES))) void k_backward_chain(
    ChainArgs<T> a, tfrt_scene3d sc) {
#pragma clang fp contract(off)
  const int n0 = a.nrays[0];
  const int i0 = blockIdx.x * (64 * BW) + threadIdx.x;
  if ((i0 & ~63) >= n0) {
    if (GOAL && (threadIdx.x & 63) == 0) {
      a.partial[i0 >> 6] = 0.0;
      if (a.partial_cnt != nullptr) a.partial_cnt[2 * (i0 >> 6)] = a.partial_cnt[2 * (i0 >> 6) + 1] = 0;
    }
    return;
  }
  __shared__ __align__(16) double wacc[BW][WSUM_CELLS];
  __shared__ int32_t wface[BW][WSUM_SLOTS];
  extern __shared__ int4 chain_lds[];
  const int lane = threadIdx.x & 63, wave = threadIdx.x >> 6;
  const int P = a.P;
  int4* chain = chain_lds + (size_t)wave * P * 64;
  wsum_clear(wacc[wave]);
  int last = -1;
  if (i0 < n0) {
    int j = i0;
    for (int p = 0; p < P; ++p) {
      const size_t at = (size_t)p * a.n + j;
      const int tape = a.rec_cls[at], tri = a.rec_tri[at];
      const int slot = a.inplace >= 2 ? j : a.rec_slot[at];
      if (a.chain_in_lds) chain[p * 64 + lane] = make_int4(j, tape, slot, tri);
      last = p;
      if ((tape & 3) != CLS_ACTIVE || p == P - 1) break;
      if (!a.inplace) j = slot;
    }
  }
  int top = last;
#pragma unroll
  for (int d = 32; d > 0; d >>= 1) top = max(top, __shfl_xor(top, d, 64));
  double child[6] = {0, 0, 0, 0, 0, 0};
  double err = 0.0;
  int n_fin = 0, n_entered = 0;
  for (int p = top; p >= 0; --p) {
    double gP[9];
    int tri = -1;
    bool fin_here = false;
    if (p <= last) {
      int4 rec;
      if (a.chain_in_lds) {
        rec = chain[p * 64 + lane];
      } else {
        const size_t at = (size_t)p * a.n + i0;
        rec = make_int4(i0, a.rec_cls[at], a.inplace >= 2 ? i0 : a.rec_slot[at], a.rec_tri[at]);
      }
      const int j = rec.x, tape = rec.y, slot = rec.z;
      const size_t off = (size_t)p * a.n;
      const T* rin = p == 0 ? a.src : a.rays_ws + (size_t)(p - 1) * 6 * a.n;
      const int64_t sin = p == 0 ? a.src_stride : a.n;
      const int32_t* idin = (p == 0 || a.inplace) ? nullptr : a.rayid + (size_t)(p - 1) * a.n;
      double seed[6] = {0, 0, 0, 0, 0, 0};
      if (GOAL && p == last && (tape & 3) == CLS_FINISHED) {
        fin_here = true;
        double fin_row[6] = {0, 0, 0, 0, 0, 0};
        if (a.inplace) {
          double s0[3], e0[3], h0[3];
          load_ray3(rin, sin, j, s0, e0);
          hit_point(s0, e0, a.rec_t[off + j], h0);
#pragma unroll
          for (int k = 0; k < 3; ++k) {
            fin_row[k] = s0[k];
            fin_row[3 + k] = static_cast<double>(static_cast<T>(h0[k]));
          }
        }
        for (int c = 0; c < a.gf.n; ++c) {
          const int row = a.gf.row[c];
          double out_c = 0.0;
          if (a.inplace) {
#pragma unroll
            for (int k = 0; k < 6; ++k)
              if (k == row) out_c = fin_row[k];
          } else {
            out_c = ldd(a.fin_rays, (int64_t)row * a.fin_cap + slot);
          }
          const double r = out_c -
                           a.goal[(int64_t)c * a.goal_stride + (int64_t)i0 * a.goal_ray_stride];
          const double g = 2.0 * r;
#pragma unroll
          for (int q = 0; q < 6; ++q)
            if (q == row) seed[q] = g;
          err += r * r;
        }
      }
      double gs[3], ge[3];
      tri = backward_core<T, GN>(j, tape, slot, rin, sin, idin, a.rec_tri + off, a.rec_t + off,
                                 a.counts + (size_t)p * TFRT_COUNTS_PER_PASS, sc, a.L, a.dead_len,
                                 p < P - 1, child, GOAL ? seed : nullptr, a.g_fin, a.cap_fin, a.g_act,
                             a.cap_act, a.g_stp, a.cap_stp, a.g_dead, a.cap_dead, gs, ge, gP,
                             rec.w, a.feta, a.inplace != 0);
      for (int k = 0; k < 3; ++k) {
        child[k] = gs[k];
        child[3 + k] = ge[k];
      }
    }
    if (GOAL) {
      n_fin += __popcll(__ballot(fin_here));
      n_entered += __popcll(__ballot(p <= last));
    }
    wave_face_sums(tri, gP, wacc[wave], wface[wave], a.g_fverts);
  }
  if (a.g_src != nullptr && i0 < n0) {
    for (int k = 0; k < 6; ++k) a.g_src[k * a.N + i0] = child[k];
  }
  if (GOAL) {
#pragma unroll
    for (int d = 32; d > 0; d >>= 1) err += __shfl_xor(err, d, 64);
    if (lane == 0) {
      a.partial[i0 >> 6] = err;
      if (a.partial_cnt != nullptr) {
        a.partial_cnt[2 * (i0 >> 6)] = n_fin;
        a.partial_cnt[2 * (i0 >> 6) + 1] = n_entered;
      }
    }
  }
}

template <typename T>
struct ChainGoalArgs {
  const T* src;
  int64_t src_stride;
  const T* rays_ws;
  const int32_t* nrays;
  const int32_t* rec_tri;
  const double* rec_t;
  const uint8_t* rec_cls;
  int64_t n;
  int32_t P;
  double L;
  double* g_src;
  int64_t N;
  double* g_fverts;
  GoalFields gf;
  const double* goal;
  int64_t goal_stride, goal_ray_stride;
  double* partial;
  int32_t* partial_cnt;
  const double* feta;
  const double* face_verts;
  const uint8_t* face_grad_mask;
  const int32_t* sched;
  int32_t ngroups;
  int32_t goal_col[6];
  uint32_t rows_packed;
  int32_t rows_ascending;
};

template <typename T>
static void chain_goal_columns(ChainGoalArgs<T>& g) {
  bool asc = true;
  for (int c = 1; c < g.gf.n; ++c) asc = asc && g.gf.row[c] > g.gf.row[c - 1];
  g.rows_ascending = asc ? 1 : 0;
  g.rows_packed = 0;
  for (int j = 0; j < 6; ++j) g.goal_col[j] = (!asc && j < g.gf.n) ? j : -1;
  for (int c = 0; c < g.gf.n; ++c) {
    g.rows_packed |= (uint32_t)(g.gf.row[c] & 7) << (4 * c);
    if (asc) g.goal_col[g.gf.row[c]] = c;
  }
}

template <typename U>
__device__ __forceinline__ U ld_scalar_base(const U* base, unsigned long long byte_offset) {
  unsigned long long v = reinterpret_cast<unsigned long long>(base);
  __asm__ volatile("" : "+s"(v));
  typedef const U __attribute__((address_space(1))) G;
  return *reinterpret_cast<G*>(v + byte_offset);
}
template <typename U>
__device__ __forceinline__ U ld_lane(const U* base, uint32_t i) {
  return ld_scalar_base(base, (unsigned long long)(i * (uint32_t)sizeof(U)));
}

template <typename T, bool FIN, bool CHILD>
__device__ __forceinline__ int chain_goal_pass(const ChainGoalArgs<T>& a, int p, int wave, int lane,
                                               int tape, int face, bool fin_lane, double child[6],
                                               double& err, double gP[9]) {
#pragma clang fp contract(off)
  const int cls = tape & 3;
  const size_t off = (size_t)p * a.n;
  const T* rin = p == 0 ? a.src : a.rays_ws + (size_t)(p - 1) * 6 * a.n;
  const int64_t sin = p == 0 ? a.src_stride : a.n;
  const bool child_pass = CHILD && p < a.P - 1;
  const bool fin_here = FIN && fin_lane;
  const bool on_face = face >= 0 && cls != CLS_DEAD;
  const bool with_child = on_face && child_pass && cls == CLS_ACTIVE;
  T ray_w[6];
  double t_rec = 0.0;
  double goal_w[6] = {0, 0, 0, 0, 0, 0};
  uint32_t lv = lane;
  __asm__ volatile("" : "+v"(lv));
  const size_t w0 = (size_t)wave * 64;
#pragma unroll
  for (int k = 0; k < 6; ++k) ray_w[k] = ld_lane(rin + k * sin + w0, lv);
  if (fin_here || on_face) t_rec = ld_lane(a.rec_t + off + w0, lv);
  if (FIN) {
    const int64_t gl = (int64_t)lv * a.goal_ray_stride;
#pragma unroll
    for (int j = 0; j < 6; ++j) {
      int cj = a.goal_col[j];
      __asm__ volatile("" : "+s"(cj));
      if (cj >= 0) {
        const double* gb = a.goal + (int64_t)cj * a.goal_stride + (int64_t)w0 * a.goal_ray_stride;
        if (fin_here) goal_w[j] = ld_scalar_base(gb, (unsigned long long)gl * sizeof(double));
      }
    }
  }
  double Pf[9] = {0, 0, 0, 0, 0, 0, 0, 0, 0}, n_a = 1.0, n_b = 1.0;
  uint8_t mask_w = 1;
  if (on_face) {
    const double* fp = a.face_verts + 9 * (int64_t)face;
#pragma unroll
    for (int q = 0; q < 9; ++q) Pf[q] = fp[q];
    if (a.face_grad_mask != nullptr && (with_child || (FIN && cls == CLS_FINISHED)))
      mask_w = a.face_grad_mask[face];
  }
  if (with_child) {
    n_a = a.feta[4 * (int64_t)face];
    n_b = a.feta[4 * (int64_t)face + 1];
  }
  double s0[3], e0[3];
#pragma unroll
  for (int k = 0; k < 3; ++k) {
    s0[k] = static_cast<double>(ray_w[k]);
    e0[k] = static_cast<double>(ray_w[3 + k]);
  }
  int mask_i = mask_w;
  __asm__ volatile("" : "+v"(mask_i));
  double seed[6] = {0, 0, 0, 0, 0, 0};
  if (fin_here) {
    double fin_row[6], h0[3];
    hit_point(s0, e0, t_rec, h0);
#pragma unroll
    for (int k = 0; k < 3; ++k) {
      fin_row[k] = s0[k];
      fin_row[3 + k] = static_cast<double>(static_cast<T>(h0[k]));
    }
    if (a.rows_ascending) {
#pragma unroll
      for (int k = 0; k < 6; ++k) {
        if (a.goal_col[k] >= 0) {
          const double r = fin_row[k] - goal_w[k];
          seed[k] = 2.0 * r;
          err += r * r;
        }
      }
    } else {
#pragma nounroll
      for (int c = 0; c < a.gf.n; ++c) {
        const int row = (a.rows_packed >> (4 * c)) & 7;
        double out_c = 0.0, goal_c = 0.0;
#pragma unroll
        for (int k = 0; k < 6; ++k) {
          if (k == row) out_c = fin_row[k];
          if (k == c) goal_c = goal_w[k];
        }
        const double r = out_c - goal_c;
        const double g = 2.0 * r;
#pragma unroll
        for (int q = 0; q < 6; ++q)
          if (q == row) seed[q] = g;
        err += r * r;
      }
    }
  }
  double gs[3], ge[3];
  const int tri = backward_core_loaded<FIN, CHILD>(tape, face, child_pass, s0, e0, Pf, t_rec, n_a,
                                                   n_b, mask_i != 0, a.L, child, seed, gs, ge, gP);
  for (int k = 0; k < 3; ++k) {
    child[k] = gs[k];
    child[3 + k] = ge[k];
  }
  return tri;
}

template <typename T>
__global__ __launch_bounds__(64)
__attribute__((amdgpu_waves_per_eu(TFRT_CHAIN_WAVES, TFRT_CHAIN_WAVES))) void k_backward_chain_goal_inplace(
    ChainGoalArgs<T> a) {
#pragma clang fp contract(off)
  const int n0 = a.nrays[0];
  int wave = blockIdx.x;
  if (a.sched != nullptr) {
    wave = __builtin_amdgcn_readfirstlane(a.sched[blockIdx.x]);
    if ((unsigned)wave >= (unsigned)a.ngroups) return;
  }
  const int i0 = wave * 64 + threadIdx.x;
  const int lane = threadIdx.x;
  if ((i0 & ~63) >= n0) {
    if (lane == 0) {
      a.partial[i0 >> 6] = 0.0;
      if (a.partial_cnt != nullptr) a.partial_cnt[2 * (i0 >> 6)] = a.partial_cnt[2 * (i0 >> 6) + 1] = 0;
    }
    return;
  }
  __builtin_assume(a.feta != nullptr);
  __shared__ __align__(16) double wacc[WSUM_CELLS];
  __shared__ int32_t wface[WSUM_SLOTS];
  extern __shared__ int2 chain_goal_lds[];
  int2* chain = chain_goal_lds;
  wsum_clear(wacc);
  const int P = a.P;
  int last = -1;
  if (i0 < n0) {
    for (int p = 0; p < P; ++p) {
      const size_t at = (size_t)p * a.n + i0;
      const int tape = a.rec_cls[at], tri = a.rec_tri[at];
      chain[p * 64 + lane] = make_int2(tape, tri);
      last = p;
      if ((tape & 3) != CLS_ACTIVE) break;
    }
  }
  int top = last;
#pragma unroll
  for (int d = 32; d > 0; d >>= 1) top = max(top, __shfl_xor(top, d, 64));
  top = __builtin_amdgcn_readfirstlane(top);
  double child[6] = {0, 0, 0, 0, 0, 0};
  double err = 0.0;
  int n_fin = 0, n_entered = 0;
  for (int p = top; p >= 0; --p) {
    double gP[9];
    int tri = -1;
    const bool here = p <= last;
    int tape = CLS_DEAD, face = -1;
    if (here) {
      const int2 rec = chain[p * 64 + lane];
      tape = rec.x;
      face = max(rec.y, -1);
    }
    const bool fin_here = here && p == last && (tape & 3) == CLS_FINISHED;
    const unsigned long long fin_m = __ballot(fin_here);
    const bool fin_role = here && fin_m != 0ull && !(p < P - 1 && (tape & 3) == CLS_ACTIVE);
    if (fin_role)
      tri = chain_goal_pass<T, true, false>(a, p, wave, lane, tape, face, fin_here, child, err, gP);
    if (here && !fin_role)
      tri = chain_goal_pass<T, false, true>(a, p, wave, lane, tape, face, false, child, err, gP);
    n_fin += __popcll(fin_m);
    n_entered += __popcll(__ballot(here));
    wave_face_sums(tri, gP, wacc, wface, a.g_fverts);
  }
  if (a.g_src != nullptr && i0 < n0) {
    for (int k = 0; k < 6; ++k) a.g_src[k * a.N + i0] = child[k];
  }
#pragma unroll
  for (int d = 32; d > 0; d >>= 1) err += __shfl_xor(err, d, 64);
  if (lane == 0) {
    a.partial[i0 >> 6] = err;
    if (a.partial_cnt != nullptr) {
      a.partial_cnt[2 * (i0 >> 6)] = n_fin;
      a.partial_cnt[2 * (i0 >> 6) + 1] = n_entered;
    }
  }
}


template <typename T>
__global__ __launch_bounds__(BLOCK) void k_finalize_seam(
    const T* __restrict__ rays, int64_t stride, int n, int chunks,
    const double* __restrict__ part_t, const int32_t* __restrict__ part_i, int64_t part_stride,
    const double* __restrict__ fverts, int M, double eps_int, double eps_size, double eps_start,
    double* x, double* y, double* z, uint8_t* valid, double* ray_u, double* trig_u,
    double* trig_v, int32_t* gather_trig) {
  const int i = blockIdx.x * BLOCK + threadIdx.x;
  if (i >= n) return;
  double bt = INFINITY;
  int bi = -1;
  for (int c = 0; c < chunks; ++c) {
    const double t = part_t[c * part_stride + i];
    if (t < bt) {
      bt = t;
      bi = part_i[c * part_stride + i];
    }
  }
  const int tri = bi < 0 ? 0 : bi;
  double s[3], e[3], P[9], h[3] = {0, 0, 0};
  TriHit th;
  th.ray_u = th.trig_u = th.trig_v = 0.0;
  th.valid = false;
  if (M > 0) {
    load_ray3(rays, stride, i, s, e);
    for (int q = 0; q < 9; ++q) P[q] = fverts[9 * (int64_t)tri + q];
    th = exact_triangle(s, e, P, eps_int, eps_size, eps_start);
    hit_point(s, e, th.ray_u, h);
  }
  x[i] = h[0];
  y[i] = h[1];
  z[i] = h[2];
  valid[i] = bi >= 0;
  ray_u[i] = bi >= 0 ? th.ray_u : INFINITY;
  trig_u[i] = th.trig_u;
  trig_v[i] = th.trig_v;
  gather_trig[i] = tri;
}


struct Plan3 {
  int R, ray_blocks, chunks, chunk_faces, nblk;
  int g_blocks, g_chunks, g_chunk_clusters;
};

struct Accel3 {
  const int32_t* order;
  int n_clusters;
  float4* csphere;
  int32_t* cface;
  float4* clsphere;
  float4* susphere;
  float4* crec;
};

static Plan3 make_plan(int64_t N, int64_t M) {
  Plan3 p;
  p.R = (N >= 32768) ? 4 : (N >= 8192 ? 2 : 1);
  p.ray_blocks = cdiv(N > 0 ? N : 1, (int64_t)BLOCK * p.R);
  int target = 4096;
  int chunks = cdiv(target, p.ray_blocks);
  const int max_chunks = cdiv(M > 0 ? M : 1, 256);
  if (chunks > max_chunks) chunks = max_chunks;
  if (chunks < 1) chunks = 1;
  p.chunk_faces = cdiv(M > 0 ? M : 1, chunks);
  p.chunks = cdiv(M > 0 ? M : 1, p.chunk_faces);
  p.nblk = cdiv(N > 0 ? N : 1, BLOCK);
  const int n_clusters = cdiv(M > 0 ? M : 1, 16);
  p.g_blocks = cdiv(N > 0 ? N : 1, (int64_t)BLOCK);
  int gtarget = 64;
  int gch = cdiv(gtarget, p.g_blocks);
  const int gmax = cdiv(n_clusters, 64);
  if (gch > gmax) gch = gmax;
  if (gch > p.chunks) gch = p.chunks;
  if (gch < 1) gch = 1;
  p.g_chunk_clusters = (cdiv(n_clusters, gch) + 7) / 8 * 8;
  p.g_chunks = cdiv(n_clusters, p.g_chunk_clusters);
  return p;
}

struct Layout3 {
  size_t c0, sphere, nrays, blockcnt, blockoff, rowtot, rowbase, ticket, part_t, part_i, prep;
  size_t csphere, cface, clsphere, susphere, crec, fnorm, feta, hist_a, hist_b, left_list, wcount,
      wbase, tape_args;
  size_t rays, rayid, lasttri, rec_tri, rec_slot, rec_t, rec_cls, gbuf, stash_g, stash_face, fix_acc,
      fix_flag, fix_max, total;
};

struct Carver {
  size_t o = 0;
  size_t operator()(size_t bytes) {
    const size_t at = o;
    o = align_up(o + bytes);
    return at;
  }
};

static Layout3 make_layout(int64_t N, int64_t M, int P, int dtype, const Plan3& pl) {
  Layout3 L;
  const size_t esz = state_bytes(dtype);
  const size_t n = N > 0 ? N : 1, m = M > 0 ? M : 1;
  Carver take;
  L.c0 = take(4 * sizeof(double));
  L.sphere = take(m * sizeof(float4));
  L.nrays = take((P + 2) * sizeof(int32_t));
  L.blockcnt = take((size_t)pl.nblk * 4 * sizeof(int32_t));
  L.blockoff = take((size_t)pl.nblk * 4 * sizeof(int32_t));
  L.rowtot = take((size_t)cdiv(pl.nblk, 1024) * 4 * sizeof(int32_t));
  L.rowbase = take((size_t)cdiv(pl.nblk, 1024) * 4 * sizeof(int32_t));
  L.ticket = take(sizeof(unsigned int));
  L.part_t = take((size_t)pl.chunks * n * sizeof(double));
  L.part_i = take((size_t)pl.chunks * n * sizeof(int32_t));
  L.prep = take((size_t)8 * n * sizeof(float));
  const size_t ncl = (m + CLUSTER - 1) / CLUSTER;
  L.csphere = take(ncl * CLUSTER * sizeof(float4));
  L.cface = take(ncl * CLUSTER * sizeof(int32_t));
  L.clsphere = take(ncl * sizeof(float4));
  L.susphere = take((ncl + SUPER - 1) / SUPER * sizeof(float4));
  L.crec = take(ncl * CLUSTER * 3 * sizeof(float4));
  L.fnorm = take(m * 3 * sizeof(double));
  L.feta = take(m * 4 * sizeof(double));
  L.hist_a = take(((size_t)pl.nblk * 4 + 1) * sizeof(int32_t));
  L.hist_b = take(((size_t)pl.nblk * 4 + 1) * sizeof(int32_t));
  L.left_list = take((n + 63) / 64 * sizeof(int32_t));
  L.wcount = take((size_t)(2 * (P > 0 ? P : 1) + 2) * inplace_wstride(n) * sizeof(uint32_t));
  L.wbase = take((size_t)(P > 0 ? P : 1) * inplace_wstride(n) * sizeof(int4));
  L.tape_args = take(sizeof(InplaceTape));
  L.rays = take((size_t)P * 6 * n * esz);
  L.rayid = take((size_t)P * n * sizeof(int32_t));
  L.lasttri = take((size_t)P * n * sizeof(int32_t));
  L.rec_tri = take((size_t)P * n * sizeof(int32_t));
  L.rec_slot = take((size_t)P * n * sizeof(int32_t));
  L.rec_t = take((size_t)P * n * sizeof(double));
  L.rec_cls = take((size_t)P * n);
  L.gbuf = take((size_t)2 * 6 * n * sizeof(double));
  L.stash_g = take((size_t)(P > 0 ? P : 1) * 9 * n * sizeof(double));
  L.stash_face = take((size_t)(P > 0 ? P : 1) * n * sizeof(int32_t));
// ... 406 lines not shown

  if (M <= 0) hipLaunchKernelGGL(k_init<>, dim3(1), dim3(64), 0, st, nrays, (int)N, tail, ticket);
  if (M <= 0 && sc->clear_buffer != nullptr && sc->clear_count > 0)
    (void)hipMemsetAsync(sc->clear_buffer, 0, (size_t)sc->clear_count * sizeof(double), st);
  const Accel3 ac = {has_hierarchy(sc, M) ? sc->cluster_order : nullptr,
                     cdiv(M > 0 ? M : 1, CLUSTER), f4(lay.csphere), i32(lay.cface),
                     f4(lay.clsphere), f4(lay.susphere), f4(lay.crec)};
  const bool coherent = sc->coherent_rays != 0 && ac.order != nullptr && N >= 64;
  if (coherent) {
    pl.g_blocks = cdiv(N, (int64_t)BLOCK);
    pl.g_chunks = 1;
    pl.g_chunk_clusters = (ac.n_clusters + 7) / 8 * 8;
  }
  const bool inplace = inplace_trace(sc, N, M, P);
  const bool rows_in_place = inplace && sc->in_place == 2;
  const bool other_sets = (c.act && c.act->rays) || (c.stp && c.stp->rays) ||
                          (c.dead && c.dead->rays) || c.unfinished != nullptr;
  if (rows_in_place && (!c.fin || !c.fin->rays || !c.fin->face || !c.fin->ray_id ||
                        c.fin->capacity < N || other_sets))
    return TFRT_E_BADARG;
  const InplaceWaves waves = inplace_waves(N);
  const InplaceTape it =
      inplace ? inplace_tape_of(tape, sc, ft, c.L, waves, rows_in_place ? c.fin : nullptr)
              : InplaceTape{};
  if (M > 0) {
    if (ac.order != nullptr) {
      const int cl_blocks = cdiv((int64_t)ac.n_clusters * CLUSTER, BLOCK);
      const int n_super = cdiv(ac.n_clusters, SUPER);
      hipLaunchKernelGGL(k_hierarchy_spheres, dim3(n_super + cl_blocks), dim3(BLOCK), 0, st,
                         sc->face_verts, M, ac.order, c0, sc->size_epsilion, ac.n_clusters,
                         n_super, ac.csphere, ac.cface, ac.clsphere, ac.crec, ac.susphere, nrays,
                         (int)N, tail, ticket, hist_ab[0],
                         (coherent && !inplace) ? pl.nblk * 4 + 1 : 0, ft,
                         sc->clear_buffer, sc->clear_buffer ? sc->clear_count : 0, it,
                         inplace ? tape.tape_args : nullptr);
    } else {
      hipLaunchKernelGGL(k_center, dim3(1), dim3(BLOCK), 0, st, sc->face_verts, M, c0, nrays,
                         (int)N, tail, ticket);
      hipLaunchKernelGGL(k_spheres, dim3(cdiv(M, BLOCK)), dim3(BLOCK), 0, st, sc->face_verts, M,
                         c0, sc->size_epsilion, sphere, ft, sc->clear_buffer,
                         sc->clear_buffer ? sc->clear_count : 0);
    }
  }
  if (inplace) {
    const InplaceArgs<T> a = inplace_args_of<T>(c, tape, waves);
    const int n_groups_waves = a.sched != nullptr ? a.ngroups << a.gshift : a.nwaves;
    const BeamScene bs = {ac.susphere, ac.clsphere, ac.csphere, ac.crec, sc->face_verts, c0,
                          ac.n_clusters, cdiv(ac.n_clusters, SUPER), sc->intersect_epsilion,
                          sc->size_epsilion, sc->ray_start_epsilion};
    {
      ProfScope prof(TFRT_PROF_INTERSECT, st);
      if (rows_in_place)
        hipLaunchKernelGGL((k_trace_inplace_rows<T>), dim3(n_groups_waves), dim3(64), 0, st, a, bs);
      else
        hipLaunchKernelGGL((k_trace_inplace<T>), dim3(n_groups_waves), dim3(64), 0, st, a, bs);
    }
    const bool want_rows = !rows_in_place && ((c.fin && c.fin->rays) || other_sets);
    if (want_rows) return inplace_gather_t<T>(c, M, sc->ray_slot, lay);
    return hipGetLastError() == hipSuccess ? 0 : TFRT_E_LAUNCH;
  }
  const int chunks_used = ac.order == nullptr ? pl.chunks : pl.g_chunks;
  float* prep = tape.template at<float>(lay.prep);
  const Intersect3 isect = {pl, st, &ac, sphere, sc->face_verts, c0, M, sc->intersect_epsilion,
                            sc->size_epsilion, sc->ray_start_epsilion, prep,
                            tape.template at<double>(lay.part_t), i32(lay.part_i), n};
  for (int p = 0; p < P; ++p) {
    const PassIn<T> in = tape.input(p, c.src, c.src_stride);
    int32_t* pass_counts = c.counts + (size_t)p * TFRT_COUNTS_PER_PASS;
    Classify3 fz = {sc->catagory, tape.rec_tri(p), tape.rec_t(p), tape.rec_cls(p), blockcnt};
    Ordered3 od;
    if (coherent) {
      od.nq = (int)N;
      od.hist = hist_ab[p & 1];
      od.left_list = left_list, od.left_count = od.hist + (size_t)pl.nblk * 4;
      od.left_total = tail + 7;
      od.coherent_only = sc->coherent_only != 0;
      od.n_super = cdiv(ac.n_clusters, SUPER);
      fz.blockcnt = od.hist;
    }
    const IntersectPass3<T> pass = {in.rays, in.stride, nrays + p, in.last, p > 0,
                                    &fz, coherent ? &od : nullptr};
    const bool classified = launch_intersect<T>(isect, pass);
    int32_t* blockcnt_p = coherent ? od.hist : blockcnt;
    if (!classified)
      hipLaunchKernelGGL(k_classify3d, dim3(pl.nblk), dim3(BLOCK), 0, st, nrays + p, chunks_used,
                         isect.part_t, isect.part_i, n, sc->catagory, tape.rec_tri(p),
                         tape.rec_t(p), tape.rec_cls(p), blockcnt_p);
    const bool grid_scan = pl.nblk >= SCAN_GRID_MIN_ROWS;
    SelfScan ss;
    if (coherent) {
      ss.hist_next = hist_ab[(p + 1) & 1];
      ss.hist_rows = pl.nblk;
    }
    if (pl.nblk <= SELF_SCAN_MAX_BLOCKS) {
      ss.blockcnt = blockcnt_p;
      ss.prev_counts = p > 0 ? c.counts + (size_t)(p - 1) * TFRT_COUNTS_PER_PASS : nullptr;
      ss.counts_row = pass_counts;
      ss.totals = tail;
      ss.n_next = nrays + p + 1;
      ss.n_tests = reinterpret_cast<unsigned long long*>(tail + 4);
      ss.M = M;
    } else if (grid_scan)
      hipLaunchKernelGGL(k_scan3d, dim3(cdiv(pl.nblk, 1024)), dim3(1024), 0, st, nrays + p,
                         blockcnt_p, blockoff, rowtot, rowbase, ticket, pass_counts,
                         tail, nrays + p + 1, reinterpret_cast<unsigned long long*>(tail + 4), M);
    else
      hipLaunchKernelGGL(k_scan3d_one, dim3(1), dim3(1024), 0, st, nrays + p, blockcnt_p,
                         blockoff, pass_counts, tail, nrays + p + 1,
                         reinterpret_cast<unsigned long long*>(tail + 4), M);
    ProfScope prof_react(TFRT_PROF_REACT, st);
    hipLaunchKernelGGL((k_react3d<T>), dim3(pl.nblk), dim3(BLOCK), 0, st, in.rays, in.stride,
                       nrays + p, in.ids, tape.rec_tri(p), tape.rec_t(p), tape.rec_cls(p),
                       blockoff, grid_scan ? rowbase : static_cast<int32_t*>(nullptr),
                       pass_counts, *sc, c.L, c.dead_len, c.flags, tape.rays_out(p), n, tape.ids(p),
                       tape.last(p), tape.rec_slot(p), c.fin ? *c.fin : NO_RAYS,
                       c.act ? *c.act : NO_RAYS, c.stp ? *c.stp : NO_RAYS,
                       c.dead ? *c.dead : NO_RAYS, tail + 6,
                       (p + 1 < P && !coherent) ? prep : nullptr, n, c0, ss, ft.fnorm, ft.feta);
  }
  if (c.unfinished != nullptr && P > 0) {
    hipLaunchKernelGGL((k_copy_rays<T, 6>), dim3(pl.nblk), dim3(BLOCK), 0, st, tape.rays_out(P - 1),
                       n, tape.ids(P - 1), nrays + P, static_cast<T*>(c.unfinished), (int64_t)N,
                       c.unfinished_id);
  }
  return hipGetLastError() == hipSuccess ? 0 : TFRT_E_LAUNCH;
}

template <typename T>
static int trace3d_backward_t(const SweepCall3& c) {
  const tfrt_scene3d* sc = c.sc;
  const int64_t N = c.N;
  const int P = c.P;
  hipStream_t st = c.st;
  const int M = (int)sc->n_faces;
  const Frame3 fr(N, M, P, c.dtype);
  if (fr.check(c.workspace_bytes)) return TFRT_E_WORKSPACE;
  const Layout3& lay = fr.lay;
  const Plan3& pl = fr.pl;
  const Tape3<const T> tape(c.workspace, lay, N);
  const Tape3<T> own(c.workspace, lay, N);
  const int32_t* nrays = tape.nrays;
  using G = typename SweepStore<T>::type;
  G* gbuf = own.template at<G>(lay.gbuf);
  G* stash_g_all = own.template at<G>(lay.stash_g);
  int32_t* stash_face_all = own.template at<int32_t>(lay.stash_face);
  unsigned long long* fix_acc = own.template at<unsigned long long>(lay.fix_acc);
  uint8_t* fix_flag = own.template at<uint8_t>(lay.fix_flag);
  unsigned long long* fix_max = own.template at<unsigned long long>(lay.fix_max);
  const int64_t n = (int64_t)tape.n;
  const int windows = cdiv(M > 0 ? M : 1, FACE_WINDOW);
  const bool ordered = sc->deterministic != 0 && M > 0 && c.g_fverts != nullptr;
  const bool wave_sums = !ordered && sc->coherent_rays != 0 && M > 0 && c.g_fverts != nullptr;
  const bool stash = ordered || (!wave_sums && M > 0 && N >= 16384 && windows <= 32);
  if (ordered)
    (void)hipMemsetAsync(fix_acc, 0, lay.total - lay.fix_acc, st);
  int acc_chunk = 8192;
  while (acc_chunk > 1024 && (int64_t)cdiv(N, acc_chunk) * windows < 256) acc_chunk /= 2;

  const bool inplace = inplace_trace(sc, N, M, P);
  const bool class_grads = c.g_fin || c.g_act || c.g_stp || c.g_dead;
  const int tape_mode = !inplace ? 0
                        : (sc->in_place == 2 ? 3 : ((class_grads || c.goal == nullptr) ? 1 : 2));
  const bool chain = wave_sums && P >= 1 && (P <= CHAIN_MAXP || inplace);
  const bool goal_inplace = chain && c.goal != nullptr && tape_mode == 2 && P <= CHAIN_MAXP &&
                            per_face_indices(sc) && sc->grad_n_in == nullptr;
  if (inplace && !wave_sums) return TFRT_E_UNSUPPORTED;
  if (c.goal != nullptr && !chain) return TFRT_E_UNSUPPORTED;
  if (chain && tape_mode == 3 &&
      (c.g_act || c.g_stp || c.g_dead || c.goal != nullptr || c.cap_fin < N))
    return TFRT_E_BADARG;

  if (chain) {
    const ChainArgs<T> a = chain_args_of<T>(c, tape, tape_mode);
    ProfScope prof_bwd(TFRT_PROF_BACKWARD, st);
    if (N > 0 && goal_inplace) {
      hipLaunchKernelGGL((k_backward_chain_goal_inplace<T>), dim3(cdiv(N, 64)), dim3(64),
                         (size_t)P * 64 * sizeof(int2), st, chain_goal_args_of(a, sc));
    } else if (N > 0) {
      using Kernel = void (*)(ChainArgs<T>, tfrt_scene3d);
      const Kernel kernel[2][2] = {
          {k_backward_chain<T, 1, false, false>, k_backward_chain<T, 1, false, true>},
          {k_backward_chain<T, 1, true, false>, k_backward_chain<T, 1, true, true>}};
      const size_t chain_lds = a.chain_in_lds ? (size_t)P * 64 * sizeof(int4) : 0;
      hipLaunchKernelGGL(kernel[c.goal != nullptr][sc->grad_n_in != nullptr], dim3(cdiv(N, 64)),
                         dim3(64), chain_lds, st, a, *sc);
    }
    return hipGetLastError() == hipSuccess ? 0 : TFRT_E_LAUNCH;
  }
  for (int p = P - 1; p >= 0; --p) {
    const PassIn<T> in = tape.input(p, c.src, c.src_stride);
    const G* g_child = (p == P - 1) ? nullptr : gbuf + (size_t)((p + 1) & 1) * 6 * n;
    G* g_out = p == 0 ? nullptr : gbuf + (size_t)(p & 1) * 6 * n;
    double* g_src_out = p == 0 ? c.g_src : nullptr;
    const int64_t out_stride = p == 0 ? N : n;
    G* stash_g = stash_g_all + (size_t)p * 9 * n;
    int32_t* stash_face = stash_face_all + (size_t)p * n;
    ProfScope prof_bwd(TFRT_PROF_BACKWARD, st);
    constexpr int BWD_BW = 1;
    hipLaunchKernelGGL((k_backward3d<T, BWD_BW>), dim3(cdiv(N, 64 * BWD_BW)), dim3(64 * BWD_BW), 0,
                       st, in.rays, in.stride, nrays + p, in.ids, tape.rec_tri(p), tape.rec_t(p),
                       tape.rec_cls(p), tape.rec_slot(p),
                       c.counts + (size_t)p * TFRT_COUNTS_PER_PASS, *sc, c.L, c.dead_len, g_child,
                       n, c.g_fin, c.cap_fin, c.g_act, c.cap_act, c.g_stp, c.cap_stp,
                       c.g_dead, c.cap_dead, g_out, g_src_out, out_stride, c.g_fverts,
                       stash ? stash_g : nullptr, stash ? stash_face : nullptr, wave_sums ? 1 : 0);
    if (ordered) {
      unsigned long long* mx = fix_max + ((P - 1 - p) & 1);
      hipLaunchKernelGGL((k_stash_absmax<G>), dim3(pl.nblk), dim3(BLOCK), 0, st, nrays + p, stash_face,
                         stash_g, mx);
      hipLaunchKernelGGL((k_face_accumulate_fixed<G>), dim3(pl.nblk), dim3(BLOCK), 0, st, nrays + p,
                         stash_face, stash_g, mx, fix_acc, fix_flag);
      hipLaunchKernelGGL(k_fixed_finish, dim3(cdiv((int64_t)M * 9, BLOCK)), dim3(BLOCK), 0, st,
                         (int64_t)M * 9, mx, fix_max + (((P - 1 - p) & 1) ^ 1), fix_acc,
                         fix_flag, c.g_fverts);
    }
  }
  if (stash && !ordered && P > 0) {
    ProfScope prof_acc(TFRT_PROF_ACCUMULATE, st);
    hipLaunchKernelGGL((k_face_accumulate<G>), dim3(cdiv(N, acc_chunk), windows), dim3(1024), 0, st,
                       nrays, P, n, stash_face_all, stash_g_all, acc_chunk, M, c.g_fverts);
  }
  return hipGetLastError() == hipSuccess ? 0 : TFRT_E_LAUNCH;
}

}

using namespace tfrt;

extern "C" {

size_t tfrt_trace3d_workspace_bytes(int64_t n_rays, int64_t n_faces, int32_t max_passes,
                                    int32_t state_dtype) {
  if (n_rays < 0 || n_faces < 0 || max_passes < 0) return 0;
  return Frame3(n_rays, n_faces, max_passes, state_dtype).lay.total;
}

int tfrt_trace3d_forward(const void* src_rays, int64_t src_stride, int64_t n_rays,
                         const tfrt_scene3d* scene, double new_ray_length,
                         double dead_ray_length, int32_t max_passes, int32_t state_dtype,
                         uint32_t flags, tfrt_ray_out* finished, tfrt_ray_out* active,
                         tfrt_ray_out* stopped, tfrt_ray_out* dead, void* unfinished,
                         int32_t* unfinished_id, int32_t* counts, void* workspace,
                         size_t workspace_bytes, void* stream) {
  if (!scene_ok(scene) || n_rays < 0 || n_rays >= (1ll << 31) - 4096 || max_passes < 0 ||
      !counts || !workspace || (n_rays > 0 && !src_rays) || src_stride < n_rays)
    return TFRT_E_BADARG;
  const TraceCall<tfrt_scene3d> c = {
      src_rays, src_stride, n_rays, scene, new_ray_length, dead_ray_length, max_passes,
      state_dtype, flags, finished, active, stopped, dead, unfinished, unfinished_id, counts,
      workspace, workspace_bytes, static_cast<hipStream_t>(stream)};
  return dispatch_state(state_dtype, TFRT_E_UNSUPPORTED, [&](auto tag) {
    return trace3d_forward_t<typename decltype(tag)::type>(c);
  });
}

int tfrt_trace3d_in_place(const tfrt_scene3d* scene, int64_t n_rays, int32_t max_passes) {
  if (!scene_ok(scene) || n_rays < 0 || max_passes < 0) return TFRT_E_BADARG;
  return inplace_trace(scene, n_rays, scene->n_faces, max_passes) ? 1 : 0;
}

int tfrt_trace3d_executed(int64_t n_rays, int64_t n_faces, int32_t max_passes, int32_t state_dtype,
                          const void* workspace, size_t workspace_bytes, int64_t* executed,
                          void* stream) {
  if (n_rays < 64 || n_faces < 0 || max_passes < 1 || !workspace || !executed) return TFRT_E_BADARG;
  const Frame3 fr(n_rays, n_faces, max_passes, state_dtype);
  if (fr.check(workspace_bytes)) return TFRT_E_WORKSPACE;
  const InplaceWaves w = inplace_waves(n_rays);
  const uint32_t* rows =
      Tape3<const void>(workspace, fr.lay, n_rays).wcount + (size_t)max_passes * w.wstride;
  hipLaunchKernelGGL(k_inplace_work, dim3(2), dim3(BLOCK), 0, static_cast<hipStream_t>(stream), rows,
                     w.nwaves, w.wstride, reinterpret_cast<unsigned long long*>(executed));
  return hipGetLastError() == hipSuccess ? 0 : TFRT_E_LAUNCH;
}

int tfrt_trace3d_wave_schedule(int64_t n_rays, int64_t n_faces, int32_t max_passes,
                               int32_t state_dtype, const void* workspace, size_t workspace_bytes,
                               int32_t* schedule_out, void* stream) {
  if (n_rays < 64 || n_rays >= (1ll << 31) - 4096 || n_faces < 0 || max_passes < 1 || !workspace ||
      !schedule_out)
    return TFRT_E_BADARG;
  const Frame3 fr(n_rays, n_faces, max_passes, state_dtype);
  if (fr.check(workspace_bytes)) return TFRT_E_WORKSPACE;
  const InplaceWaves w = inplace_waves(n_rays);
  hipLaunchKernelGGL(k_wave_schedule, dim3(1), dim3(1024), 0, static_cast<hipStream_t>(stream),
                     Tape3<const void>(workspace, fr.lay, n_rays).wcount, w.wstride,
                     (int)max_passes, w.nwaves, 64 / w.bundle, w.ngroups, schedule_out);
  return hipGetLastError() == hipSuccess ? 0 : TFRT_E_LAUNCH;
}

int tfrt_trace3d_wave_rows(int64_t n_rays, int64_t n_faces, int32_t max_passes, int32_t state_dtype,
                           const void* workspace, size_t workspace_bytes, uint32_t* rows_out,
                           void* stream) {
  if (n_rays < 64 || n_rays >= (1ll << 31) - 4096 || n_faces < 0 || max_passes < 1 || !workspace)
    return TFRT_E_BADARG;
  const Frame3 fr(n_rays, n_faces, max_passes, state_dtype);
  if (fr.check(workspace_bytes)) return TFRT_E_WORKSPACE;
  const InplaceWaves w = inplace_waves(n_rays);
  if (rows_out != nullptr &&
      hipMemcpy2DAsync(rows_out, (size_t)w.nwaves * sizeof(uint32_t),
                       Tape3<const void>(workspace, fr.lay, n_rays).wcount,
                       (size_t)w.wstride * sizeof(uint32_t), (size_t)w.nwaves * sizeof(uint32_t),
                       (size_t)max_passes + 2, hipMemcpyDeviceToDevice,
                       static_cast<hipStream_t>(stream)) != hipSuccess)
    return TFRT_E_LAUNCH;
  return w.nwaves;
}

int tfrt_trace3d_compact(const void* src_rays, int64_t src_stride, int64_t n_rays,
                         double dead_ray_length, int32_t max_passes, int32_t state_dtype,
                         uint32_t flags, tfrt_ray_out* finished, tfrt_ray_out* active,
                         tfrt_ray_out* stopped, tfrt_ray_out* dead, void* unfinished,
                         int32_t* unfinished_id, int32_t* counts, int64_t n_faces,
                         const int32_t* ray_slot, void* workspace, size_t workspace_bytes,
                         void* stream) {
  if (n_rays < 64 || n_rays >= (1ll << 31) - 4096 || max_passes < 1 || !counts || !workspace ||
      !src_rays || src_stride < n_rays || n_faces < 0)
    return TFRT_E_BADARG;
  const Frame3 fr(n_rays, n_faces, max_passes, state_dtype);
  if (fr.check(workspace_bytes)) return TFRT_E_WORKSPACE;
  const TraceCall<tfrt_scene3d> c = {
      src_rays, src_stride, n_rays, nullptr, 0.0, dead_ray_length, max_passes, state_dtype, flags,
      finished, active, stopped, dead, unfinished, unfinished_id, counts, workspace,
      workspace_bytes, static_cast<hipStream_t>(stream)};
  return dispatch_state(state_dtype, TFRT_E_UNSUPPORTED, [&](auto tag) {
    return inplace_gather_t<typename decltype(tag)::type>(c, n_faces, ray_slot, fr.lay);
  });
}

int tfrt_trace3d_backward(const void* src_rays, int64_t src_stride, int64_t n_rays,
                          const tfrt_scene3d* scene, double new_ray_length,
                          double dead_ray_length, int32_t max_passes, int32_t state_dtype,
                          const double* grad_finished, int64_t cap_finished,
                          const double* grad_active, int64_t cap_active,
                          const double* grad_stopped, int64_t cap_stopped,
                          const double* grad_dead, int64_t cap_dead, double* grad_face_verts,
                          double* grad_src_rays, const int32_t* counts, void* workspace,
                          size_t workspace_bytes, void* stream) {
  if (!scene_ok(scene) || n_rays < 0 || max_passes < 0 || !counts || !workspace ||
// ... 171 lines not shown
```

### tensorflowraytrace_amd/csrc/trace_math.h

```cpp
#pragma once
#include <math.h>

#if defined(__HIPCC__)
#define TFRT_HD __host__ __device__ __forceinline__
#else
#define TFRT_HD inline
#endif

namespace tfrt {

constexpr int CLS_ACTIVE = 0;
constexpr int CLS_FINISHED = 1;
constexpr int CLS_STOPPED = 2;
constexpr int CLS_DEAD = 3;

constexpr int CAT_OPTICAL = 0, CAT_STOP = 1, CAT_TARGET = 2;

struct TriHit {
  double ray_u, trig_u, trig_v;
  bool valid;
};

TFRT_HD TriHit exact_triangle(const double s[3], const double e[3], const double P[9],
                              double eps_int, double eps_size, double eps_start) {
// ... 54 lines not shown
TFRT_HD void face_normal(const double P[9], double N[3], double C[3], double* clen) {
#pragma clang fp contract(off)
  const double A[3] = {P[3] - P[0], P[4] - P[1], P[5] - P[2]};
  const double B[3] = {P[6] - P[3], P[7] - P[4], P[8] - P[5]};
  cross3(A, B, C);
  const double len = sqrt(dot3(C, C));
  *clen = len;
  N[0] = C[0] / len;
  N[1] = C[1] / len;
  N[2] = C[2] / len;
}

TFRT_HD double l2_normalize3(const double v[3], double o[3]) {
#pragma clang fp contract(off)
  double sq = dot3(v, v);
  if (sq < 1e-12) sq = 1e-12;
  const double inv = 1.0 / sqrt(sq);
  o[0] = v[0] * inv;
  o[1] = v[1] * inv;
  o[2] = v[2] * inv;
  return inv;
}

struct Snell3 {
  double u[3], n[3];
  double nu, eta, k;
  bool reflect;
  double w[3];
};

TFRT_HD void snell_normal(const double P[9], double n[3]) {
  double N[3], C[3], clen;
  face_normal(P, N, C, &clen);
  l2_normalize3(N, n);
}

TFRT_HD void snell_ratios(double n_in, double n_out, double* n1, double* n2) {
#pragma clang fp contract(off)
  const bool in_safe = n_in != 0.0, out_safe = n_out != 0.0;
  const double nis = in_safe ? n_in : 1.0, nos = out_safe ? n_out : 1.0;
  *n1 = out_safe ? nis / nos : 0.0;
  *n2 = in_safe ? nos / nis : 0.0;
}

TFRT_HD Snell3 snell3d_core(const double s[3], const double h[3], const double un[3], double n1,
                            double n2, bool mirror) {
#pragma clang fp contract(off)
  Snell3 o;
  const double r[3] = {h[0] - s[0], h[1] - s[1], h[2] - s[2]};
  l2_normalize3(r, o.u);
  o.n[0] = un[0];
  o.n[1] = un[1];
  o.n[2] = un[2];
  o.nu = dot3(o.n, o.u);
  const bool internal = o.nu > 0.0;
  o.eta = internal ? n1 : n2;
  const double nu_eta = o.eta * o.nu;
  o.k = 1.0 - o.eta * o.eta + nu_eta * nu_eta;
  const bool tir = o.k < 0.0;
  o.reflect = tir || mirror;
  if (o.reflect) {
    for (int i = 0; i < 3; ++i) o.w[i] = -2.0 * o.nu * o.n[i] + o.u[i];
  } else {
    const double sg = (o.nu > 0.0) ? 1.0 : ((o.nu < 0.0) ? -1.0 : 0.0);
    const double alpha = sg * sqrt(o.k) - nu_eta;
    for (int i = 0; i < 3; ++i) o.w[i] = alpha * o.n[i] + o.eta * o.u[i];
  }
  return o;
}

TFRT_HD Snell3 snell3d_unit(const double s[3], const double h[3], const double un[3],
                            double n_in, double n_out) {
  double n1, n2;
  snell_ratios(n_in, n_out, &n1, &n2);
  return snell3d_core(s, h, un, n1, n2, n_in == 0.0);
}

TFRT_HD Snell3 snell3d(const double s[3], const double h[3], const double norm[3],
                       double n_in, double n_out) {
  double un[3];
  l2_normalize3(norm, un);
  return snell3d_unit(s, h, un, n_in, n_out);
}

TFRT_HD double fmod_floor(double x, double m) {
  double r = fmod(x, m);
  if (r != 0.0 && ((r < 0.0) != (m < 0.0))) r += m;
  return r;
}

TFRT_HD double snell2d_angle(double xs, double ys, double xe, double ye, double norm,
                             double n_in, double n_out) {
#pragma clang fp contract(off)
  const double PI = 3.141592653589793;
  norm = fmod_floor(norm, 2 * PI);
  double ray_angle = atan2(ys - ye, xs - xe);
  ray_angle = fmod_floor(ray_angle, 2 * PI);
  double theta1 = norm - ray_angle;
  if (theta1 > PI) theta1 = theta1 - 2 * PI;
  if (theta1 < -PI) theta1 = theta1 + 2 * PI;
  const bool internal = fabs(theta1) >= PI / 2;
  const bool in_safe = n_in != 0.0, out_safe = n_out != 0.0;
  const double nis = in_safe ? n_in : 1.0, nos = out_safe ? n_out : 1.0;
  const double n1 = out_safe ? nis / nos : 0.0;
  const double n2 = in_safe ? nos / nis : 0.0;
  const double n = internal ? n1 : n2;
  if (!internal) norm = norm + PI;
  if (internal) theta1 = theta1 + PI;
  const double theta2 = n * sin(theta1);
  if (fabs(theta2) <= 1.0 && n != 0.0) return norm - asin(theta2);
  return norm + theta1 + PI;
}

TFRT_HD double adj_rcp(double x) {
#if defined(__HIP_DEVICE_COMPILE__)
  double r = __builtin_amdgcn_rcp(x);
  r = __builtin_fma(__builtin_fma(-x, r, 1.0), r, r);
  r = __builtin_fma(__builtin_fma(-x, r, 1.0), r, r);
  return r;
#else
  return 1.0 / x;
#endif
}
TFRT_HD double adj_rsqrt(double x) {
#if defined(__HIP_DEVICE_COMPILE__)
  double y = __builtin_amdgcn_rsq(x);
  double e = __builtin_fma(-x * y, y, 1.0);
  y = __builtin_fma(0.5 * y, e, y);
  e = __builtin_fma(-x * y, y, 1.0);
  y = __builtin_fma(0.5 * y, e, y);
  return y;
#else
  return 1.0 / sqrt(x);
#endif
}

TFRT_HD double adj_dot3(const double a[3], const double b[3]) {
#if defined(__HIP_DEVICE_COMPILE__)
  return __builtin_fma(a[2], b[2], __builtin_fma(a[1], b[1], a[0] * b[0]));
#else
  return dot3(a, b);
#endif
}
TFRT_HD void adj_cross3(const double a[3], const double b[3], double o[3]) {
#if defined(__HIP_DEVICE_COMPILE__)
  o[0] = __builtin_fma(a[1], b[2], -(a[2] * b[1]));
  o[1] = __builtin_fma(a[2], b[0], -(a[0] * b[2]));
  o[2] = __builtin_fma(a[0], b[1], -(a[1] * b[0]));
#else
  cross3(a, b, o);
#endif
}

TFRT_HD void adjoint3d(const double s[3], const double e[3], const double P[9], double ray_u,
                       bool has_child, double n_in, double n_out, double L,
                       const double g_s[3], const double g_h[3], const double g_ce[3],
                       double gs[3], double ge[3], double gP[9], double* gn = nullptr,
                       int branch = -1, bool gn_wanted = true, bool face_terms = true,
                       const double* ratios = nullptr) {
  if (gn != nullptr) gn[0] = gn[1] = 0.0;
  const double d[3] = {e[0] - s[0], e[1] - s[1], e[2] - s[2]};
  const double E1[3] = {P[3] - P[0], P[4] - P[1], P[5] - P[2]};
  const double E2[3] = {P[6] - P[0], P[7] - P[1], P[8] - P[2]};
  double C[3];
  adj_cross3(E1, E2, C);
  const double t = ray_u;
  double h[3] = {s[0] + t * d[0], s[1] + t * d[1], s[2] + t * d[2]};

  double hb[3] = {g_h[0], g_h[1], g_h[2]};
  double sb[3] = {g_s[0], g_s[1], g_s[2]};
  double Cn[3] = {0.0, 0.0, 0.0};

  if (has_child) {
    const double inv_c = adj_rsqrt(adj_dot3(C, C));
    const double n[3] = {C[0] * inv_c, C[1] * inv_c, C[2] * inv_c};
    const double r[3] = {h[0] - s[0], h[1] - s[1], h[2] - s[2]};
    const double rsq = adj_dot3(r, r);
    const bool clamped = rsq < 1e-12;
    const double inv_r = clamped ? 1e6 : adj_rsqrt(rsq);
    const double u[3] = {r[0] * inv_r, r[1] * inv_r, r[2] * inv_r};
    const double nu = adj_dot3(n, u);
    const bool in_safe = n_in != 0.0, out_safe = n_out != 0.0;
    const double nis = in_safe ? n_in : 1.0, nos = out_safe ? n_out : 1.0;
    const bool internal = branch >= 0 ? (branch & 1) != 0 : nu > 0.0;
    const double eta = ratios != nullptr
                           ? (internal ? ratios[0] : ratios[1])
                           : (internal ? (out_safe ? nis / nos : 0.0) : (in_safe ? nos / nis : 0.0));
    const double nu_eta = eta * nu;
    double k = 1.0 - eta * eta + nu_eta * nu_eta;
    const bool reflect = branch >= 0 ? (branch & 2) != 0 : ((k < 0.0) || (n_in == 0.0));
    if (!reflect && k < 0.0) k = 0.0;
    double wb[3], ub[3], nb[3];
    for (int i = 0; i < 3; ++i) {
      hb[i] += g_ce[i];
      wb[i] = L * g_ce[i];
    }
    double nub;
    if (reflect) {
      nub = -2.0 * adj_dot3(wb, n);
      for (int i = 0; i < 3; ++i) {
        ub[i] = wb[i];
        nb[i] = -2.0 * nu * wb[i];
      }
    } else {
      const double sg = branch >= 0 ? (internal ? 1.0 : (nu < 0.0 ? -1.0 : 0.0))
                                    : ((nu > 0.0) ? 1.0 : ((nu < 0.0) ? -1.0 : 0.0));
      const double irk = k > 0.0 ? adj_rsqrt(k) : INFINITY;
      const double rk = k > 0.0 ? k * irk : 0.0;
      const double alpha = sg * rk - nu_eta;
      const double ab = adj_dot3(wb, n);
      nub = ab * (sg * eta * nu_eta * irk - eta);
      if (gn != nullptr && gn_wanted) {
        const double etab = adj_dot3(wb, u) + ab * (sg * eta * (nu * nu - 1.0) * irk - nu);
        if (internal) {
          if (out_safe) {
            gn[0] = in_safe ? etab / nos : 0.0;
            gn[1] = -etab * eta / nos;
          }
        } else if (in_safe) {
          gn[1] = out_safe ? etab / nis : 0.0;
          gn[0] = -etab * eta / nis;
        }
      }
      for (int i = 0; i < 3; ++i) {
        nb[i] = alpha * wb[i];
        ub[i] = eta * wb[i];
      }
    }
    for (int i = 0; i < 3; ++i) {
      nb[i] += nub * u[i];
      ub[i] += nub * n[i];
    }
    if (!clamped) {
      const double uu = adj_dot3(u, ub);
      for (int i = 0; i < 3; ++i) {
        const double rb = (ub[i] - u[i] * uu) * inv_r;
        hb[i] += rb;
        sb[i] -= rb;
      }
    } else {
      for (int i = 0; i < 3; ++i) {
        hb[i] += ub[i] * 1e6;
        sb[i] -= ub[i] * 1e6;
      }
    }
    if (face_terms) {
      const double nn = adj_dot3(n, nb);
      for (int i = 0; i < 3; ++i) Cn[i] = (nb[i] - n[i] * nn) * inv_c;
    }
  }

  double db[3];
  double tb = 0.0;
  for (int i = 0; i < 3; ++i) {
    sb[i] += hb[i];
    tb += hb[i] * d[i];
    db[i] = t * hb[i];
  }
  const double den = adj_dot3(d, C);
  const double numb = tb * adj_rcp(den);
  const double denb = -numb * t;
  if (face_terms) {
    double Cb[3];
    for (int i = 0; i < 3; ++i) Cb[i] = Cn[i] + (numb * (P[i] - s[i]) + denb * d[i]);
    double E1b[3], E2b[3];
    adj_cross3(E2, Cb, E1b);
    adj_cross3(Cb, E1, E2b);
    for (int i = 0; i < 3; ++i) {
      gP[3 + i] = E1b[i];
      gP[6 + i] = E2b[i];
      gP[i] = numb * C[i] - (E1b[i] + E2b[i]);
    }
  }
  for (int i = 0; i < 3; ++i) {
    sb[i] -= numb * C[i];
    db[i] += denb * C[i];
    ge[i] = db[i];
    gs[i] = sb[i] - db[i];
  }
}

}
```

### tensorflowraytrace_amd/fused_step.py

```python
import ctypes
import gc

import numpy as np
import torch

from . import _lib, ops
from . import distributed as tdist
from ._lib import RayOut, check

_GEO3 = ("x_start", "y_start", "z_start", "x_end", "y_end", "z_end")
_GEO2 = ("x_start", "y_start", "x_end", "y_end")
_FIELDS3 = _GEO3 + ("x_dir", "y_dir", "z_dir")
_FIELDS2 = _GEO2 + ("x_dir", "y_dir")

_CLASS_FLAGS = (("finished", _lib.COMPILE_FINISHED), ("active", _lib.COMPILE_ACTIVE),
                ("stopped", _lib.COMPILE_STOPPED), ("dead", _lib.COMPILE_DEAD))


class _NotInPlace(RuntimeError):
    """The fixed-shape path of a RowwiseError needs an in-place trace; this step takes the generic
    path instead."""


class GoalError:

    def __init__(self, fields=("y_end", "z_end"), goal=None, rowwise=False):
        self.fields = tuple(fields)
        self.rowwise = bool(rowwise)
        if not self.fields or any(f not in _GEO3 for f in self.fields):
            raise ValueError(f"GoalError: fields must be taken from {_GEO3}, got {fields!r}")
        if goal is None:
            raise ValueError("GoalError: a goal (callable or tensor) is required")
        if len(set(self.fields)) != len(self.fields):
            raise ValueError(f"GoalError: duplicate fields in {fields!r}")
        self.rows = [_GEO3.index(f) for f in self.fields]
        self.goal = goal
        self._cache = None

    def rows_for(self, dimension):
        if dimension == 3:
            return self.rows
        bad = [f for f in self.fields if f not in _GEO2]
        if bad:
            raise ValueError(f"GoalError: field(s) {bad} do not exist on a {dimension}-D engine "
                             f"(fields of its rays: {_GEO2})")
        return [_GEO2.index(f) for f in self.fields]

    def table(self, src, by_ray=False):
        if hasattr(src, "cache_key"):
            vals, key = [src], src.cache_key
        else:
            vals = list(src.values()) if hasattr(src, "values") else [src[k] for k in src.keys()]
            key = tuple((id(v), getattr(v, "_version", None)) for v in vals)
        key = (key, bool(by_ray))
        if self._cache is not None and self._cache[0] == key:
            return self._cache[1]
        g = self.goal(src) if callable(self.goal) else self.goal
        if hasattr(src, "n_rays"):
            n, dev = src.n_rays, src.device
        else:
            n, dev = src["x_start"].shape[0], src["x_start"].device
        g = torch.as_tensor(g, dtype=torch.float64, device=dev).detach()
        if g.dim() == 1:
            g = g.reshape(-1, 1)
        if tuple(g.shape) != (n, len(self.fields)):
            raise ValueError(f"GoalError: goal has shape {tuple(g.shape)}, expected "
                             f"({n}, {len(self.fields)}) -- one row per source ray")
        table = g.contiguous() if by_ray else g.t().contiguous()
        self._cache = (key, table, vals)
        return table

    def __call__(self, engine):
        self.rows_for(engine.dimension)
        fin = engine.finished_rays
        if not bool(fin):
            return torch.zeros((0, len(self.fields)), dtype=torch.float64)
        ids = engine.last_trace["finished_id"].long()
        table = self.table(engine._trace_src)
        out = torch.stack([fin[f] for f in self.fields], dim=1).double()
        return (out - table[:, ids].t()) ** 2


class RowwiseError:

    def __init__(self, fn):
        if not callable(fn):
            raise ValueError("RowwiseError: fn must be callable")
        self.fn = fn
        self.rows = []

    def __call__(self, engine):
        return self.fn(engine.finished_rays)


def _field_codes(what, fields, dimension):
    names = _FIELDS3 if dimension == 3 else _FIELDS2
    bad = [f for f in fields if f not in names]
    if bad:
        raise ValueError(f"{what}: field(s) {bad} do not exist on a {dimension}-D engine "
                         f"(fields of its rays: {names})")
    return [names.index(f) for f in fields]


def _geometry_block(engine, fin):
    dim = engine.dimension
    return dim, torch.stack([fin[f] for f in (_GEO3 if dim == 3 else _GEO2)], dim=0)


def _source_buffer(owner, name, given, convert, src, what, noun, keep=False):
    if hasattr(src, "n_rays"):
        n, dev = src.n_rays, src.device
    else:
        n, dev = src["x_start"].shape[0], src["x_start"].device
    value = getattr(owner, name)
    if callable(given):
        if hasattr(src, "cache_key"):
            vals, key = [src], src.cache_key
        else:
            vals = list(src.values()) if hasattr(src, "values") else [src[k] for k in src.keys()]
            key = tuple((id(v), getattr(v, "_version", None)) for v in vals)
        hit = owner._caches.get(name)
        if hit is None or hit[0] != key:
            new = convert(given(src), dev)
            if keep and value is not None and value.shape == new.shape \
                    and value.device == new.device:
                value.copy_(new)
            else:
                value = new
                setattr(owner, name, value)
            owner._caches[name] = (key, vals)
    elif value.device != dev:
        value = value.to(dev)
        setattr(owner, name, value)
    if value.numel() != n:
        raise ValueError(f"{what}: {value.numel()} {noun}s for {n} source rays -- one {noun} per "
                         "source ray")
    return value


def _as_weights(what, weights, device):
    w = weights if isinstance(weights, torch.Tensor) else torch.as_tensor(np.asarray(weights))
    if w.dim() != 1 or not w.dtype.is_floating_point:
        raise ValueError(f"{what}: weights must be floats of shape (N,), one weight per source "
                         f"ray; got shape {tuple(w.shape)}, {w.dtype}")
    w = w.detach().to(device=device, dtype=torch.float64)
    if w.numel() == 0:
        raise ValueError(f"{what}: at least one weight must be > 0")
    if not (w.is_cuda and torch.cuda.is_current_stream_capturing()):
        if not bool(torch.isfinite(w).all()) or bool((w < 0).any()):
            raise ValueError(f"{what}: weights must be finite and >= 0")
        if not bool((w > 0).any()):
            raise ValueError(f"{what}: at least one weight must be > 0")
# ... 289 lines not shown

class _SpotTerms(torch.autograd.Function):

    @staticmethod
    def forward(ctx, block, erf, labels, ids, weights=None, dimension=None, codes=None):
        rows = block.detach().contiguous()
        ctx.chained = codes is not None
        if codes is None:
            codes = (0, 1)[:rows.shape[0]]
        err, grad, acc = erf.evaluate(rows, codes[0], codes[1] if len(codes) == 2 else -1, labels,
                                      perm=ids, dimension=dimension, weights=weights)
        ctx.save_for_backward(grad)
        ctx.dtype = block.dtype
        if ctx.chained:
            link = ops._link_torch(rows, dimension)
            v = torch.stack([ops._link_field_torch(link, c, dimension) for c in codes], dim=0)
            return _spot_terms(erf, v, labels, ids, acc, weights)
        half = 0.5 * grad
        return _spot_terms(erf, rows.double(), labels, ids, acc, weights,
                           inside=half * half if weights is None else None)

    @staticmethod
    def backward(ctx, upstream):
        grad, = ctx.saved_tensors
        if not ctx.chained:
            return (upstream.t() * grad).to(ctx.dtype), None, None, None, None, None, None
        if upstream.shape[1] == 2 and not torch.equal(upstream[:, 0], upstream[:, 1]):
            raise ValueError("SpotError with a direction field: the upstream gradient must weigh "
                             "both fields of a ray alike")
        return (upstream[:, 0] * grad).to(ctx.dtype), None, None, None, None, None, None


class _RowFields:

    def __init__(self, geo, inherited):
        self._geo, self._inh = geo, inherited

    def __getitem__(self, key):
        if key in self._geo:
            return self._geo[key]
        return self._inh(key)

    def keys(self):
        return list(self._geo.keys())

    def __bool__(self):
        return True


class _HyperTable:

    def __init__(self, n, device, slots=8, width=3):
        self.width = width
        self.dev = torch.zeros((n, width), dtype=torch.float64, device=device)
        self._host = [torch.zeros((n, width), dtype=torch.float64).pin_memory()
                      for _ in range(slots)]
        self._events = [None] * slots
        self._at = 0
        self._current = None

    def set(self, rows):
        if rows == self._current:
            return
        k = self._at
        self._at = (k + 1) % len(self._host)
        if self._events[k] is not None:
            self._events[k].synchronize()
        self._host[k].copy_(torch.tensor(rows, dtype=torch.float64))
        self.dev.copy_(self._host[k], non_blocking=True)
        ev = torch.cuda.Event()
        ev.record(torch.cuda.current_stream(self.dev.device))
        self._events[k] = ev
        self._current = rows



class _Override:
    __slots__ = ("_sc", "_new", "_old")

    def __init__(self, sc, fields):
        self._sc, self._new = sc, fields

    def __enter__(self):
        sc = self._sc
        self._old = [(name, getattr(sc, name)) for name in self._new]
        for name, value in self._new.items():
            setattr(sc, name, value)
        return sc

    def __exit__(self, *exc):
        for name, value in self._old:
            setattr(self._sc, name, value)
        return False


def _override(sc, **fields):
    return _Override(sc, fields)


class _StepState:
    __slots__ = (
        "sig", "dim", "N", "M", "Ms", "Ma", "P", "dt", "flags", "capN",
        "full", "aux", "outs", "no_outs", "counts", "ints", "ws", "wsb",
        "err", "goal_ws", "gws", "fields",
        "g_fin", "g_fv", "g_n",
        "g_prim", "g_seg", "g_arc", "g_index",
        "rows", "row_face", "row_passes", "row_outs",
        "density_ws", "hq",
        "spot_ws", "acc",
        "chain_ws", "inherited",
        "sched", "sched_key", "sched_checked",
        "block", "stream", "perm", "inplace")

    def __init__(self, sig, block, dim, P, flags, fields, workspace_bytes):
        for name in self.__slots__:
            setattr(self, name, None)
        n_rows, dev = 2 * dim, block.device
        N = block.shape[1]
        capN = max(N, 1)
        self.sig, self.dim, self.N, self.P, self.flags, self.capN = sig, dim, N, P, flags, capN
        self.dt = ops._DT[block.dtype]
        ints = ops._IntPool(dev, True, _lib.COUNTS_PER_PASS * (P + 1), flags, capN, P)
        caps = {"finished": capN, "active": capN * max(P, 1), "stopped": capN, "dead": capN}
        full, aux, outs = {}, {"counts": ints.counts}, {}
        for name, flag in _CLASS_FLAGS:
            if flags & flag:
                rays = torch.empty((n_rows, caps[name]), dtype=block.dtype, device=dev)
                ids, faces = ints.take(caps[name]), ints.take(caps[name])
                full[name], aux[name + "_id"], aux[name + "_face"] = rays, ids, faces
                outs[name] = ops._ray_out(rays, ids, faces)
            else:
                aux[name + "_id"] = aux[name + "_face"] = None
                outs[name] = ops._ray_out(None, None, None)
        aux["unfinished"] = torch.empty((n_rows, 0), dtype=block.dtype, device=dev)
        aux["unfinished_id"] = torch.empty(0, dtype=torch.int32, device=dev)
        self.full, self.aux, self.outs = full, aux, outs
        self.no_outs = {name: ops._ray_out(None, None, None) for name, _ in _CLASS_FLAGS}
        self.counts, self.ints = ints.counts, ints
        wsb, gws = workspace_bytes
        self.ws, self.wsb = torch.empty(max(wsb, 1), dtype=torch.uint8, device=dev), wsb
        self.err = torch.zeros(3, dtype=torch.float64, device=dev)
        self.goal_ws, self.gws = torch.zeros(max(gws, 1), dtype=torch.uint8, device=dev), gws
        self.fields = (ctypes.c_int32 * n_rows)(*(list(fields) + [0] * n_rows)[:n_rows])

    def __getitem__(self, name):
        return getattr(self, name)


class FusedStep:

    fold_backward = True
    folded_backward = False
    in_place = False
    capture_collective = "auto"
    collective_in_graph = False
    schedule_min_waves = None

    def __init__(self, optimizer, graph="auto", graph_warmup=3):
        self.opt = optimizer
        self.graph_mode = graph
        self.graph_warmup = int(graph_warmup)
        self._state = None
        self._graphs = None
        self._stream = None
        self._last_sig = None
        self._eager_steps = 0
        self.tests_total = None
        self.steps = 0
        self.graph_replays = 0
        self.capture_error = None
        self.collective_capture_error = None
        self.untapped = False
        self._tap_checks = 0
        self._goal_perm = None
        self._goal_pending = None
        self._hyper = self._hyper_apply = None
        self._err_view = None
        self._flat_buf = self._flat = self._err_sink = None
        self._flat_views = False

    @staticmethod
    def eligible(optimizer, args, kwargs):
        eng = optimizer.engine
        erf = optimizer.error_function
        if not isinstance(erf, (GoalError, RowwiseError, DensityError, SpotError)) or args or kwargs:
            return False
        if (isinstance(erf, (RowwiseError, DensityError, SpotError)) and eng.dimension == 3
                and not FusedStep.rowwise_ready(eng)):
            return False
        if isinstance(erf, (DensityError, SpotError)) and tdist.is_distributed():
            return False
        if not bool(eng.optical_system):
            return False
        if eng.dimension == 2 and not FusedStep.eligible2d(optimizer):
            return False
        try:
            eng._reaction()
        except RuntimeError:
            return False
        return all(isinstance(p, torch.Tensor) and p.is_cuda and p.dtype == torch.float64
                   and p.is_contiguous() for p in optimizer.parameters)

    @staticmethod
    def eligible2d(optimizer):
        eng, erf = optimizer.engine, optimizer.error_function
        if not isinstance(erf, (GoalError, RowwiseError)) or tdist.is_distributed() \
                or eng._custom_ops():
            return False
        if eng.ray_shard not in (None, "auto"):
            return False
        if isinstance(erf, RowwiseError):
            return True
        try:
            erf.rows_for(2)
        except ValueError:
            return False
        return True

    @staticmethod
    def rowwise_ready(eng):
        return (eng.in_place is not False and eng.coherent is not False and not eng.deterministic
                and getattr(eng, "_visit_all_key", None) is not None
                and not getattr(eng, "_rowwise_off", False))

    def _buffers(self, block, fv, P, flags, index=False):
        N, M = block.shape[1], fv.shape[0]
        dt = ops._DT[block.dtype]
        rows = self.opt.error_function.rows
        sig = (N, M, P, dt, flags, str(block.device), tuple(rows), bool(index))
        st = self._state
        if st is None or st.sig != sig:
            L = _lib.lib()
            st = _StepState(sig, block, 3, P, flags, rows,
                            (L.tfrt_trace3d_workspace_bytes(N, M, P, dt),
                             L.tfrt_goal_error3d_workspace_bytes(max(N, 1))))
            dev = block.device
            st.M = M
            st.g_fin = torch.zeros((6, st.capN), dtype=torch.float64, device=dev)
            st.g_fv = torch.zeros((max(M, 1), 9), dtype=torch.float64, device=dev)
            if index:
                st.g_n = torch.zeros((2, max(M, 1)), dtype=torch.float64, device=dev)
            self._install(st)
        st.block, st.stream = block, ops._stream(block)
        return st

    def _buffers2d(self, block, det, P, flags, rows, index):
        N = block.shape[1]
        Ms, Ma = (0 if g is None else g.shape[0] for g in det)
        dt = ops._DT[block.dtype]
        index = tuple(i is not None for i in index)
        sig = (2, N, Ms, Ma, P, dt, flags, str(block.device), tuple(rows or ()), rows is None,
               index)
        st = self._state
        if st is None or st.sig != sig:
            L = _lib.lib()
            st = _StepState(sig, block, 2, P, flags, rows or (),
                            (L.tfrt_trace2d_workspace_bytes(N, Ms, Ma, P, dt),
                             L.tfrt_trace2d_backward_goal_workspace_bytes(N)))
            dev = block.device
            st.Ms, st.Ma = Ms, Ma
            n_index = 2 * (Ms + Ma) if any(index) else 0
            at = 4 * Ms + 5 * Ma
            g = st.g_prim = torch.zeros(max(at + n_index, 1), dtype=torch.float64, device=dev)
            st.g_seg, st.g_arc = g[:4 * Ms].view(Ms, 4), g[4 * Ms:at].view(Ma, 5)
            st.g_index = [None] * 4
            if n_index:
                cuts = (at, at + Ms, at + 2 * Ms, at + 2 * Ms + Ma, at + n_index)
                st.g_index = [g[a:b] if want else None
                              for a, b, want in zip(cuts, cuts[1:], index)]
            if rows is None:
                st.rows = torch.empty((4, st.capN), dtype=block.dtype, device=dev)
                st.row_face = torch.empty(st.capN, dtype=torch.int32, device=dev)
            self._install(st)
        st.block, st.stream = block, ops._stream(block)
        return st

    def _install(self, st):
        self._state = st
        self._graphs = None
        dev = st.err.device
        if self.tests_total is None or self.tests_total.device != dev:
            self.tests_total = torch.zeros(1, dtype=torch.int64, device=dev)

    def _lengths(self):
        eng = self.opt.engine
        return float(eng.new_ray_length), float(eng.dead_ray_length or 0.0)

    def _trace_forward(self, st, sc, outs):
        name = "tfrt_trace3d_forward" if st.dim == 3 else "tfrt_trace2d_forward"
        block = st.block
        check(getattr(_lib.lib(), name)(
            ops._p(block), block.shape[1], st.N, ctypes.byref(sc), *self._lengths(), st.P, st.dt,
            st.flags, ctypes.byref(outs["finished"]), ctypes.byref(outs["active"]),
            ctypes.byref(outs["stopped"]), ctypes.byref(outs["dead"]),
            None, None,
            ops._p(st.counts), ops._p(st.ws), st.wsb, st.stream), name)

    def _trace3d_backward(self, st, sc, seeds, capacity):
        block = st.block
        check(_lib.lib().tfrt_trace3d_backward(
            ops._p(block), block.shape[1], st.N, ctypes.byref(sc), *self._lengths(), st.P, st.dt,
            ops._p(seeds), capacity, None, 0, None, 0, None, 0, ops._p(st.g_fv), None,
            ops._p(st.counts), ops._p(st.ws), st.wsb, st.stream), "tfrt_trace3d_backward")

    @staticmethod
    def _goal_finish(pending, stream):
        check(_lib.lib().tfrt_goal_finish(ctypes.byref(pending), stream), "tfrt_goal_finish")

    def _enqueue_gradient(self):
        opt, eng = self.opt, self.opt.engine
        eng.clear_ray_history()
        from . import boundaries
        with boundaries.collect_taps() as tap_log:
            eng.optical_system.update()
        src = eng._source_set()
        if not src:
            raise RuntimeError("FusedStep: the optical system has no source rays")
        inputs = eng._trace_inputs(src)
        P, flags = int(opt.trace_depth), eng._flags() | _lib.COMPILE_FINISHED
        rowwise = isinstance(opt.error_function, (RowwiseError, DensityError, SpotError))
        if eng.dimension == 2:
            body = self._rowwise2d if rowwise else self._goal2d
        else:
            body = self._rowwise3d if rowwise else self._goal3d
        grads, st = body(src, inputs, tap_log, P, flags)
        self._publish_lazily(st, src)
        return ([None] * len(opt.parameters) if grads is None else grads), st.err

    def _goal3d(self, src, inputs, tap_log, P, flags):
        erf = self.opt.error_function
        block, scene, fv = inputs
        perm = self.opt.engine._trace_perm
        goal, goal_by_ray = self._goal_rows(erf, src, perm)
        fvc = self._faces(fv)
        index = self._index3d(scene, fvc)
        st = self._buffers(block, fvc, P, flags, any(n is not None for n in index))
        sink = self._err_sink
        if tdist.is_distributed() and sink is not None and st.err.data_ptr() != sink.data_ptr():
            st.err = sink
        sc = scene.struct(fvc)
        need_back = bool((fv.requires_grad or st.g_n is not None) and st.M > 0)
        folded = bool(self.fold_backward and need_back and sc.coherent_rays
                      and not sc.deterministic and 1 <= P <= 8)
        inplace = bool(folded and sc.in_place and st.N >= 64 and P >= 1)
        self.folded_backward, self.in_place = folded, inplace
        st.perm = perm
        st.inplace = (block, self._lengths()[1]) if inplace else None
        clear = {"clear_buffer": st.g_fv.data_ptr(), "clear_count": st.g_fv.numel()} if folded \
            else {}
        sched = self._wave_schedule(st) if inplace else None
        with _override(sc, in_place=1 if inplace else 0,
                       wave_schedule=None if sched is None else sched.data_ptr()):
            with _override(sc, **clear):
                self._trace_forward(st, sc, st.no_outs if inplace else st.outs)
            with self._index_grads3d(sc, st, need_back):
                self._goal_backward3d(st, sc, (goal, goal_by_ray), folded, need_back)
        if inplace:
            self._make_wave_schedule(st, perm)
        if not need_back:
            return None, st
        return self._parameter_gradients(*self._outs3d(fv, st, index), tap_log), st

    def _wave_schedule(self, st):
        given = self.opt.engine.wave_schedule
        if isinstance(given, torch.Tensor):
            key = (id(given), given._version)
            if st.sched_checked != key:
                if given.device != st.block.device:
                    raise RuntimeError("FusedStep: wave_schedule must be on the rays' device")
                ops.check_wave_schedule(given, st.N)
                st.sched_checked = key
            return given
        if given != "auto":
            if given is not False:
                raise ValueError("OpticalEngine.wave_schedule must be 'auto', False or an int32 "
                                 f"tensor, got {given!r}")
            return None
        return st.sched if st.sched_key is not None else None

    def _make_wave_schedule(self, st, perm):
        eng = self.opt.engine
        if not isinstance(eng.wave_schedule, str) or eng.wave_schedule != "auto":
            return
        G = ops.wave_groups(st.N)
        least = self.schedule_min_waves
        if least is None:
            least = 20 * torch.cuda.get_device_properties(st.block.device).multi_processor_count
        key = (id(perm), eng.optical_system.scene_signature())
        if G <= least or st.sched_key == key or torch.cuda.is_current_stream_capturing():
            return
        if st.sched is None:
            st.sched = torch.empty(G, dtype=torch.int32, device=st.block.device)
        ops.wave_schedule(st.N, st.M, st.P, st.block.dtype, st.ws, out=st.sched)
        st.sched_key = key

    def _goal_rows(self, erf, src, perm):
        if perm is None:
            return erf.table(src), False
        rowwise = bool(erf.rowwise and callable(erf.goal) and hasattr(src, "permuted"))
        base = None if rowwise else erf.table(src)
        gkey = (id(erf), src.cache_key if rowwise else id(base), id(perm), rowwise)
        cached = self._goal_perm
        if cached is None or cached[0] != gkey:
            if rowwise:
                rows, by_ray = erf.table(src.permuted(perm), by_ray=True), True
            else:
                rows, by_ray = ops.gather_rows(base, perm), False
            cached = self._goal_perm = (gkey, rows, perm, by_ray, base)
        return cached[1], cached[3]

    def _goal_backward3d(self, st, sc, goal_rows, folded, need_back):
        L = _lib.lib()
        goal, by_ray = goal_rows
        n_fields = len(self.opt.error_function.rows)
        strides = (1, goal.shape[1]) if by_ray else (goal.shape[1], 1)
        block, stream = st.block, st.stream
        several = tdist.is_distributed()
        pending = _lib.GoalPending()
        self._goal_pending = None
        if folded:
            if st.chain_ws is None:
                cwb = L.tfrt_trace3d_backward_goal_workspace_bytes(st.N)
                st.chain_ws = (torch.zeros(max(cwb, 1), dtype=torch.uint8, device=block.device), cwb)
            check(L.tfrt_trace3d_backward_goal(
                ops._p(block), block.shape[1], st.N, ctypes.byref(sc), *self._lengths(), st.P,
                st.dt, ctypes.byref(st.outs["finished"]), st.fields, n_fields, ops._p(goal),
                *strides, ops._p(st.err), ops._p(self.tests_total), ops._p(st.chain_ws[0]),
                st.chain_ws[1], ctypes.byref(pending), None, 0, None, 0, None, 0,
                ops._p(st.g_fv), None, ops._p(st.counts), ops._p(st.ws), st.wsb, stream),
                "tfrt_trace3d_backward_goal")
            if several:
                self._goal_finish(pending, stream)
        else:
            goal_args = (
                ops._p(st.full["finished"]), st.capN, ops._p(st.aux["finished_id"]), st.dt,
                ops._p(st.counts), st.P, st.fields, n_fields, ops._p(goal), *strides,
                ops._p(st.g_fin), ops._p(st.err), ops._p(st.g_fv) if need_back else None,
                st.g_fv.numel() if need_back else 0, ops._p(self.tests_total),
                ops._p(st.goal_ws), st.gws)
            if several:
                check(L.tfrt_goal_error3d(*goal_args, stream), "tfrt_goal_error3d")
            else:
                check(L.tfrt_goal_error3d_deferred(*goal_args, ctypes.byref(pending), stream),
                      "tfrt_goal_error3d_deferred")
        if not several:
            self._goal_pending = (pending, stream)
        if need_back and not folded:
            self._trace3d_backward(st, sc, st.g_fin, st.capN)

    @staticmethod
    def _faces(fv):
        fvc = fv.detach()
        if fvc.dtype != torch.float64 or not fvc.is_contiguous():
            raise RuntimeError("FusedStep: merged faces must be contiguous float64")
        return fvc

    @staticmethod
    def _index3d(scene, fvc):
        if scene.n_table is not None or fvc.shape[0] == 0:
            return (None, None)
        return tuple(n if isinstance(n, torch.Tensor) and n.requires_grad else None
                     for n in (scene.n_in_arg, scene.n_out_arg))

    @staticmethod
    def _outs3d(fv, st, index):
        outs, g_outs = ([fv], [st.g_fv]) if fv.requires_grad else ([], [])
        for k, n in enumerate(index):
            if n is not None:
                outs.append(n)
                g_outs.append(st.g_n[k, :n.shape[0]])
        return outs, g_outs

    @staticmethod
    def _index_grads3d(sc, st, on):
        g = st.g_n
        if not on or g is None:
            return _override(sc)
        g.zero_()
        return _override(sc, grad_n_in=g[0].data_ptr(), grad_n_out=g[1].data_ptr())

    def _rowwise3d(self, src, inputs, tap_log, P, flags):
        eng = self.opt.engine
        block, scene, fv = inputs
        perm = eng._trace_perm
        fvc = self._faces(fv)
        index = self._index3d(scene, fvc)
        st = self._buffers(block, fvc, P, flags, any(n is not None for n in index))
        N, M, dev = st.N, st.M, block.device
        sc = scene.struct(fvc)
        if not (scene.in_place and sc.coherent_rays
                and _lib.lib().tfrt_trace3d_in_place(ctypes.byref(sc), N, P) == 1):
            eng._rowwise_off = True
            raise _NotInPlace()
        if st.rows is None:
            st.rows = torch.zeros((6, st.capN), dtype=block.dtype, device=dev)
            st.row_face = torch.full((st.capN,), -1, dtype=torch.int32, device=dev)
            st.row_passes = torch.zeros(st.capN, dtype=torch.int32, device=dev)
            st.row_outs = dict(st.no_outs,
                               finished=ops._ray_out(st.rows, st.row_passes, st.row_face))
        need_back = bool((fv.requires_grad or st.g_n is not None) and M > 0)
        self.folded_backward, self.in_place = False, True
        self._goal_pending = None
        st.perm, st.inplace = perm, (block, self._lengths()[1])
        clear = {"clear_buffer": st.g_fv.data_ptr(), "clear_count": st.g_fv.numel()} if need_back \
            else {}
        grads = None
        with _override(sc, in_place=2, **clear):
            self._trace_forward(st, sc, st.row_outs)
            if isinstance(self.opt.error_function, (DensityError, SpotError)):
                if isinstance(self.opt.error_function, DensityError):
                    g64 = self._density_seeds3d(st, src, perm)
                else:
                    g64 = self._spot_seeds3d(st, src, perm)
                if not need_back:
                    g64 = None
            else:
                g64 = self._rowwise_seeds3d(st, src, perm, need_back)
            if g64 is not None:
                with self._index_grads3d(sc, st, True):
                    self._trace3d_backward(st, sc, g64, g64.shape[1])
                grads = self._parameter_gradients(*self._outs3d(fv, st, index), tap_log)
        return grads, st

    def _density_seeds3d(self, st, src, perm):
        erf = self.opt.error_function
        dev = st.rows.device
        goal = erf.goal_on(dev)
        if st.hq is None or st.hq.shape != goal.shape:
            nx, ny = goal.shape[-1], (goal.shape[0] if goal.dim() == 2 else 1)
            wsb = _lib.lib().tfrt_density_error_workspace_bytes(st.N, nx, ny)
            st.density_ws = torch.empty(max(wsb, 1), dtype=torch.uint8, device=dev)
            st.hq = torch.zeros(goal.shape, dtype=torch.int64, device=dev)
        rows = erf.rows
        erf.evaluate(st.rows[:, :st.N], rows[0], rows[1] if len(rows) == 2 else -1,
                     mask=st.row_face, dimension=3, weights=erf.weights_of(src), perm=perm,
                     grad=st.g_fin, err=st.err, hq=st.hq, workspace=st.density_ws)
        with torch.no_grad():
            self.tests_total += st.row_passes[:st.N].sum() * st.M
        return st.g_fin

    def _spot_seeds3d(self, st, src, perm):
        erf = self.opt.error_function
        dev = st.rows.device
        labels = erf.labels_of(src)
        weights = erf.weights_of(src)
        record = 4 if weights is None else 8
        if st.acc is None or tuple(st.acc.shape) != (erf.n_groups, record):
            wsb = _lib.lib().tfrt_spot_error_workspace_bytes(st.N, erf.n_groups)
            st.spot_ws = torch.empty(max(wsb, 1), dtype=torch.uint8, device=dev)
            st.acc = torch.zeros((erf.n_groups, record), dtype=torch.int64, device=dev)
        rows = erf.rows
        erf.evaluate(st.rows[:, :st.N], rows[0], rows[1] if len(rows) == 2 else -1, labels,
                     mask=st.row_face, perm=perm, dimension=3, weights=weights, grad=st.g_fin,
                     err=st.err, acc=st.acc, workspace=st.spot_ws)
        with torch.no_grad():
            self.tests_total += st.row_passes[:st.N].sum() * st.M
        return st.g_fin

    def _rowwise_seeds3d(self, st, src, perm, need_back):
        N, M, dev = st.N, st.M, st.rows.device
        if perm is None:
            inherited = src.__getitem__
        else:
            if st.inherited is None:
                st.inherited = {}
            cache = st.inherited

            def inherited(key):
                v = src[key]
                hit = cache.get(key)
                if hit is None or hit[0] is not v or hit[1] is not perm or hit[2] != v._version:
                    hit = cache[key] = (v, perm, v._version, v.index_select(0, perm.long()))
                return hit[3]
        leaf, e = self._rowwise_terms(st, _GEO3, inherited)
        mask = st.row_face[:N] >= 0
        err_sum = torch.where(mask.unsqueeze(1), e.double(), torch.zeros((), dtype=torch.float64,
                                                                       device=dev)).sum()
        terms = mask.sum().double() * e.shape[1]
        with torch.no_grad():
            st.err[0] = err_sum.detach()
            st.err[1] = terms
            st.err[2] = torch.where(terms > 0, err_sum.detach() / torch.clamp(terms, min=1.0),
                                    torch.full_like(terms, float("nan")))
            self.tests_total += st.row_passes[:N].sum() * M
        if need_back and err_sum.requires_grad:
            with torch.autograd.set_multithreading_enabled(False):
                g_rows, = torch.autograd.grad(err_sum, [leaf])
            return g_rows.to(torch.float64).contiguous()
        return None

    def _rowwise_terms(self, st, names, inherited):
        leaf = st.rows.detach().requires_grad_(True)
        geo = {name: leaf[k] for k, name in enumerate(names)}
        e = self.opt.error_function.fn(_RowFields(geo, inherited))
        if e.dim() == 1:
            e = e.reshape(-1, 1)
        if e.shape[0] != st.N or (st.dim == 2 and e.dim() != 2):
            raise RuntimeError(f"RowwiseError: fn returned {tuple(e.shape)}, expected one row "
                               f"per ray ({st.N})")
        return leaf, e

    def _parameter_gradients(self, outs, g_outs, tap_log):
        opt = self.opt
        grads = [None] * len(opt.parameters)
        capturing = torch.cuda.is_current_stream_capturing()
        inputs, owner = [], []
        for i, p in enumerate(opt.parameters):
            taps = tap_log.get(id(p), [])
            if not taps:
                self.untapped = True
            checked = self._tap_checks >= self.graph_warmup and not self.untapped
            if (capturing or checked) and taps:
                inputs.extend(taps)
                owner.extend([i] * len(taps))
            else:
                inputs.extend(taps + [p])
                owner.extend([i] * len(taps) + [-1 - i])
        with torch.autograd.set_multithreading_enabled(False):
            got = torch.autograd.grad(outs, inputs, grad_outputs=g_outs, allow_unused=True)
        total = {}
        for i, g in zip(owner, got):
            if g is None:
                continue
            if i < 0:
                total[-1 - i] = g
            else:
                grads[i] = g if grads[i] is None else grads[i] + g
        for i, g in total.items():
            if (not self.untapped and self._tap_checks < self.graph_warmup
                    and not self._same_gradient(grads[i], g)):
                self.untapped = True
                self.capture_error = RuntimeError(
                    f"FusedStep: parameter {i} reaches the faces without boundaries.tap "
                    "(its leaf gradient differs from the sum over its aliases): the step "
                    "is never captured in a launch graph")
            grads[i] = g
        if not capturing:
            self._tap_checks += 1
        return grads

    @staticmethod
    def _same_gradient(aliases, leaf):
        if aliases is None or not bool(torch.isfinite(leaf).eq(torch.isfinite(aliases)).all()):
            return False
        finite = dict(nan=0.0, posinf=0.0, neginf=0.0)
        return float(torch.nan_to_num(aliases - leaf, **finite).abs().max()) \
            <= 1e-9 * float(torch.nan_to_num(leaf, **finite).abs().max())

    def _setup2d(self, inputs, P, flags, rows):
        block, scene, _ = inputs
        geo = [None if k is None else k["geo"] for k in (scene.segments, scene.arcs)]
        det = [None if g is None else g.detach() for g in geo]
        if any(g is not None and (g.dtype != torch.float64 or not g.is_contiguous()) for g in det):
            raise RuntimeError("FusedStep: merged segments / arcs must be contiguous float64")
        index = [n if isinstance(n, torch.Tensor) and n.requires_grad and n.shape[0] > 0 else None
                 for n in scene.index_args()]
        st = self._buffers2d(block, det, P, flags, rows, index)
        st.perm = st.inplace = None
        back = [(g, grad) for g, grad in zip(geo, (st.g_seg, st.g_arc))
                if g is not None and g.requires_grad and g.shape[0] > 0]
        back += [(n, g) for n, g in zip(index, st.g_index) if n is not None]
        return st, scene.struct(det[0], det[1]), back

    @staticmethod
    def _index_grads2d(sc, st, on):
        return _override(sc, **{name: g.data_ptr() for name, g in zip(ops._GRAD_INDEX_2D, st.g_index)
                                if on and g is not None})

    def _goal2d(self, src, inputs, tap_log, P, flags):
        erf = self.opt.error_function
        rows = erf.rows_for(2)
        goal = erf.table(src)
        st, sc, back = self._setup2d(inputs, P, flags, rows)
        block = st.block
# ... 355 lines not shown
```

### tensorflowraytrace_amd/ops.py

```python
import ctypes

import numpy as np
import torch

from . import _lib
from ._lib import TfrtError, RayOut, Scene3D, check

_DT = {torch.float32: _lib.F32, torch.float64: _lib.F64, torch.float16: _lib.F16}


def _need_gpu(*tensors):
    for t in tensors:
        if t is not None and not t.is_cuda:
            raise TfrtError(
                "tfrt kernels need tensors on a HIP device (got a CPU tensor); the hot path has "
                "no CPU fallback")


def _p(t):
    return None if t is None else ctypes.c_void_p(t.data_ptr())


_raw_stream = getattr(torch._C, "_cuda_getCurrentRawStream", None)

# ... 43 lines not shown
    return _corner_cache[key][1], _corner_cache[key][2]


class _BuildFaces(torch.autograd.Function):

    @staticmethod
    def forward(ctx, vertices, faces, update_mask):
        _need_gpu(vertices, faces, update_mask)
        vertices = _c(vertices, torch.float64)
        F = faces.shape[0]
        corners = vertex_corners(faces, vertices.shape[0]) if F > 0 else None
        fv = torch.empty((F, 9), dtype=torch.float64, device=vertices.device)
        norm = torch.empty((F, 3), dtype=torch.float64, device=vertices.device)
        check(_lib.lib().tfrt_build_faces_forward(
            _p(vertices), vertices.shape[0], _p(faces), F, _p(fv), _p(norm), _stream(vertices)),
            "tfrt_build_faces_forward")
        ctx.save_for_backward(fv, faces, update_mask)
        ctx.n_vertices = vertices.shape[0]
        ctx.corners = corners
        ctx.set_materialize_grads(False)
        return fv, norm

    @staticmethod
    def backward(ctx, g_fv, g_norm):
        fv, faces, update_mask = ctx.saved_tensors
        g_fv = _c(g_fv, torch.float64)
        g_norm = _c(g_norm, torch.float64)
        if (g_fv is None and g_norm is None) or faces.shape[0] == 0:
            return torch.zeros((ctx.n_vertices, 3), dtype=torch.float64, device=fv.device), None, None
        start, lst = ctx.corners
        gv = torch.empty((ctx.n_vertices, 3), dtype=torch.float64, device=fv.device)
        check(_lib.lib().tfrt_build_faces_backward(
            _p(g_fv), _p(g_norm), _p(fv), _p(faces), _p(update_mask), faces.shape[0],
            ctx.n_vertices, _p(start), _p(lst), _p(gv), _stream(fv)), "tfrt_build_faces_backward")
        return gv, None, None


def build_faces(vertices, faces, update_mask=None):
    faces = _c(faces, torch.int32)
    if update_mask is not None:
        update_mask = _c(update_mask, torch.uint8)
    return _BuildFaces.apply(vertices, faces, update_mask)


class _ParamFaces(torch.autograd.Function):

    @staticmethod
    def forward(ctx, parameters, zero_points, vectors, faces, update_mask):
        _need_gpu(parameters, zero_points, vectors, faces, update_mask)
        parameters = _c(parameters, torch.float64).reshape(-1)
        V, F = zero_points.shape[0], faces.shape[0]
        if parameters.shape[0] != V or vectors.shape != zero_points.shape:
            raise TfrtError("param_faces: parameters (V,), zero_points (V,3) and vectors (V,3) "
                            "must describe the same vertices")
        corners = vertex_corners(faces, V) if F > 0 else None
        fv = torch.empty((F, 9), dtype=torch.float64, device=parameters.device)
        norm = torch.empty((F, 3), dtype=torch.float64, device=parameters.device)
        check(_lib.lib().tfrt_param_faces_forward(
            _p(zero_points), _p(vectors), _p(parameters), V, _p(faces), F, _p(fv), _p(norm),
            _stream(parameters)), "tfrt_param_faces_forward")
        ctx.save_for_backward(fv, faces, update_mask, vectors)
        ctx.shape = parameters.shape
        ctx.corners = corners
        ctx.set_materialize_grads(False)
        return fv, norm

    @staticmethod
    def backward(ctx, g_fv, g_norm):
        fv, faces, update_mask, vectors = ctx.saved_tensors
        g_fv = _c(g_fv, torch.float64)
        g_norm = _c(g_norm, torch.float64)
        if (g_fv is None and g_norm is None) or faces.shape[0] == 0:
            return torch.zeros(ctx.shape, dtype=torch.float64, device=fv.device), None, None, None, None
        start, lst = ctx.corners
        gp = torch.empty(ctx.shape, dtype=torch.float64, device=fv.device)
        check(_lib.lib().tfrt_param_faces_backward(
            _p(g_fv), _p(g_norm), _p(fv), _p(faces), _p(update_mask), _p(vectors),
            faces.shape[0], vectors.shape[0], _p(start), _p(lst), _p(gp), _stream(fv)),
            "tfrt_param_faces_backward")
        return gp, None, None, None, None


def param_faces(parameters, zero_points, vectors, faces, update_mask=None):
    faces = _c(faces, torch.int32)
    zero_points = _c(zero_points.detach(), torch.float64)
    vectors = _c(vectors.detach(), torch.float64)
    if update_mask is not None:
        update_mask = _c(update_mask, torch.uint8)
    return _ParamFaces.apply(parameters, zero_points, vectors, faces, update_mask)


class _ParamFacesMulti(torch.autograd.Function):

    @staticmethod
    def forward(ctx, spec, *parameters):
        dev = parameters[0].device if parameters else spec[0][1].device
        rows = [e[3].shape[0] if e[0] == "param" else e[1].shape[0] for e in spec]
        M = int(sum(rows))
        fv = torch.empty((M, 9), dtype=torch.float64, device=dev)
        norms = []
        descs, keep, pars = [], [], []
        at = k = 0
        for e, F in zip(spec, rows):
            d = _lib.FaceSurface()
            d.n_faces = F
            d.face_verts = fv.data_ptr() + at * 72
            if e[0] == "param":
                _, zero, vectors, faces, mask = e
                par = _c(parameters[k], torch.float64).reshape(-1)
                k += 1
                V = zero.shape[0]
                if par.shape[0] != V or vectors.shape != zero.shape:
                    raise TfrtError("param_faces: parameters (V,), zero_points (V,3) and vectors "
                                    "(V,3) must describe the same vertices")
                d.zero_points, d.vectors, d.parameters = _p(zero), _p(vectors), _p(par)
                d.faces, d.n_vertices = _p(faces), V
                norms.append(torch.empty((F, 3), dtype=torch.float64, device=dev))
                d.norm = _p(norms[-1])
                pars.append((at, F, V, faces, mask, vectors, par.shape))
                keep.append(par)
            else:
                d.copy_from = _p(e[1])
            descs.append(d)
            at += F
        stream = _stream(fv)
        for i in range(0, len(descs), _lib.MAX_SURFACES):
            chunk = descs[i:i + _lib.MAX_SURFACES]
            arr = (_lib.FaceSurface * len(chunk))(*chunk)
            check(_lib.lib().tfrt_param_faces_forward_multi(arr, len(chunk), stream),
                  "tfrt_param_faces_forward_multi")
        ctx.pars = pars
        ctx.corners = [vertex_corners(f, V) if F > 0 else None for (_, F, V, f, _, _, _) in pars]
        ctx.save_for_backward(fv)
        ctx.set_materialize_grads(False)
        return (fv, *norms)

    @staticmethod
    def backward(ctx, g_fv, *g_norms):
        (fv,) = ctx.saved_tensors
        g_fv = _c(g_fv, torch.float64)
        out, descs, keep = [], [], []
        for (at, F, V, faces, mask, vectors, shape), corners, g_norm in zip(ctx.pars, ctx.corners,
                                                                            g_norms):
            g_norm = _c(g_norm, torch.float64)
            keep.append(g_norm)
            if (g_fv is None and g_norm is None) or F == 0:
                out.append(torch.zeros(shape, dtype=torch.float64, device=fv.device))
                continue
            sink = GradSink._active
            gp = sink.take(shape) if sink is not None else None
            if gp is None:
                gp = torch.empty(shape, dtype=torch.float64, device=fv.device)
            d = _lib.FaceSurfaceGrad()
            d.grad_face_verts = g_fv.data_ptr() + at * 72 if g_fv is not None else None
            d.grad_norm = _p(g_norm)
            d.face_verts = fv.data_ptr() + at * 72
            d.update_mask, d.vectors = _p(mask), _p(vectors)
            d.corner_start, d.corner_list = _p(corners[0]), _p(corners[1])
            d.n_vertices, d.grad_parameters = V, _p(gp)
            descs.append(d)
            out.append(gp)
        stream = _stream(fv)
        for i in range(0, len(descs), _lib.MAX_SURFACES):
            chunk = descs[i:i + _lib.MAX_SURFACES]
            arr = (_lib.FaceSurfaceGrad * len(chunk))(*chunk)
            check(_lib.lib().tfrt_param_faces_backward_multi(arr, len(chunk), stream),
                  "tfrt_param_faces_backward_multi")
        return (None, *out)


_faces_batch = None


class GradSink:

    _active = None

    def __init__(self, flat):
        self.flat, self.at, self.taken = flat, 0, []

    def __enter__(self):
        self._prev, GradSink._active = GradSink._active, self
        return self

    def __exit__(self, *exc):
        GradSink._active = self._prev
        return False

    def take(self, shape):
        n = 1
        for d in shape:
            n *= int(d)
        if self.at + n > self.flat.numel():
            return None
        view = self.flat[self.at:self.at + n].view(shape)
        self.at += n
        self.taken.append(view)
        return view

    def holds(self, t):
        return any(v.data_ptr() == t.data_ptr() and v.numel() == t.numel() for v in self.taken)


def current_faces_batch():
    return _faces_batch


class ParamFacesBatch:

    def __init__(self):
        self.requests = []
        self.merged = None
        self._outer = None

    def __enter__(self):
        global _faces_batch
        self._outer, _faces_batch = _faces_batch, self
        return self

    def __exit__(self, *exc):
        global _faces_batch
        _faces_batch = self._outer
        return False

    def add(self, boundary, parameters, zero_points, vectors, faces, mask):
        faces = _c(faces, torch.int32)
        zero_points = _c(zero_points.detach(), torch.float64)
        vectors = _c(vectors.detach(), torch.float64)
        if mask is not None:
            mask = _c(mask, torch.uint8)
        _need_gpu(parameters, zero_points, vectors, faces, mask)
        if faces.shape[0] > 0:
            vertex_corners(faces, zero_points.shape[0])
        self.requests.append((boundary, parameters, zero_points, vectors, faces, mask))
        boundary.__dict__["_faces_pending"] = self

    def flush(self, order=None):
        if not self.requests:
            return
        reqs, self.requests = self.requests, []
        by_boundary = {id(r[0]): r for r in reqs}
        layout = None
        if order is not None:
            layout = []
            for b in order:
                r = by_boundary.get(id(b))
                if r is not None:
                    layout.append(("param", r))
                    continue
                fv = b.__dict__.get("_face_verts_value")
                overridden = any(k in getattr(b, "_fields", {}) for k in
                                 ("xp", "yp", "zp", "x1", "y1", "z1", "x2", "y2", "z2"))
                if (fv is None or overridden or fv.requires_grad or not fv.is_cuda
                        or fv.dtype != torch.float64
                        or not fv.is_contiguous() or fv.dim() != 2 or fv.shape[1] != 9):
                    layout = None
                    break
                layout.append(("copy", b, fv))
            if layout is not None and sum(1 for e in layout if e[0] == "param") != len(reqs):
                layout = None
        if layout is None:
            layout = [("param", r) for r in reqs]
        spec = [("param", e[1][2], e[1][3], e[1][4], e[1][5]) if e[0] == "param"
                else ("copy", e[2]) for e in layout]
        pars = [e[1][1] for e in layout if e[0] == "param"]
        fv, *norms = _ParamFacesMulti.apply(spec, *pars)
        at = k = 0
        rows = []
        for e in layout:
            if e[0] == "param":
                b, F = e[1][0], e[1][4].shape[0]
                b.__dict__["_faces_pending"] = None
                b._face_verts = fv[at:at + F]
                b._norm = norms[k]
                rows.append((b, at, at + F))
                k += 1
            else:
                F = e[2].shape[0]
                rows.append((e[1], at, at + F))
            at += F
        if order is not None and len(layout) == len(order):
            self.merged = (fv, rows)



def _ptr_array(tensors):
    arr = (ctypes.c_void_p * len(tensors))(*[t.data_ptr() for t in tensors])
    return ctypes.cast(arr, ctypes.c_void_p), arr


def _pairwise(first, second, grid):
    first = [_c(torch.as_tensor(t), torch.float64) for t in first]
    dev = first[0].device
    second = [_c(torch.as_tensor(t, device=dev), torch.float64) for t in second]
    _need_gpu(*first, *second)
    if grid:
        first = [t.reshape(-1) for t in first]
        second = [t.reshape(-1) for t in second]
        n_cols, n_rows = first[0].numel(), second[0].numel()
        if any(t.numel() != n_cols for t in first) or any(t.numel() != n_rows for t in second):
            raise TfrtError("pairwise geometry: operands of one set must have equal lengths")
        return n_cols, n_rows, first, (1, 0), second, (0, 1), (n_rows, n_cols)
    shape = torch.broadcast_shapes(*[t.shape for t in first + second])
    first = [t.expand(shape).contiguous().reshape(-1) for t in first]
    second = [t.expand(shape).contiguous().reshape(-1) for t in second]
    return first[0].numel(), 1, first, (1, 0), second, (1, 0), tuple(shape)


def line_intersect(first, second, epsilion, grid):
    nc, nr, f, fs, s2, ss, shape = _pairwise(first, second, grid)
    dev = f[0].device
    new = lambda: torch.empty(shape, dtype=torch.float64, device=dev)
    x, y, u, v = new(), new(), new(), new()
    valid = torch.empty(shape, dtype=torch.uint8, device=dev)
    fp, keep1 = _ptr_array(f)
    sp, keep2 = _ptr_array(s2)
    check(_lib.lib().tfrt_line_intersect(nc, nr, fp, fs[0], fs[1], sp, ss[0], ss[1],
                                         float(epsilion), _p(x), _p(y), _p(valid), _p(u), _p(v),
                                         _stream(x)), "tfrt_line_intersect")
    return x, y, valid.bool(), u, v


def line_triangle_intersect(rays, triangles, epsilion, grid):
    nc, nr, f, fs, s2, ss, shape = _pairwise(rays, triangles, grid)
    dev = f[0].device
    new = lambda: torch.empty(shape, dtype=torch.float64, device=dev)
    x, y, z, ru, tu, tv = new(), new(), new(), new(), new(), new()
    valid = torch.empty(shape, dtype=torch.uint8, device=dev)
    fp, keep1 = _ptr_array(f)
    sp, keep2 = _ptr_array(s2)
    check(_lib.lib().tfrt_line_triangle_intersect(
        nc, nr, fp, fs[0], fs[1], sp, ss[0], ss[1], float(epsilion), _p(x), _p(y), _p(z),
        _p(valid), _p(ru), _p(tu), _p(tv), _stream(x)), "tfrt_line_triangle_intersect")
    return x, y, z, valid.bool(), ru, tu, tv


def line_circle_intersect(lines, circles, epsilion, grid):
    nc, nr, f, fs, s2, ss, shape = _pairwise(lines, circles, grid)
    dev = f[0].device
    new = lambda: torch.empty(shape, dtype=torch.float64, device=dev)
    roots = []
    for _ in range(2):
        roots.append(([new(), new(), new(), new()], torch.empty(shape, dtype=torch.uint8, device=dev)))
    fp, keep1 = _ptr_array(f)
    sp, keep2 = _ptr_array(s2)
    pp, keep3 = _ptr_array(roots[0][0])
    mp, keep4 = _ptr_array(roots[1][0])
    check(_lib.lib().tfrt_line_circle_intersect(
        nc, nr, fp, fs[0], fs[1], sp, ss[0], ss[1], float(epsilion), pp, _p(roots[0][1]), mp,
        _p(roots[1][1]), _stream(roots[0][1])), "tfrt_line_circle_intersect")
    out = []
    for (x, y, u, v), valid in roots:
        out.append({"x": x, "y": y, "valid": valid.bool(), "u": u, "v": v})
    return out[0], out[1]
# ... 1556 lines not shown
```

Baseline: 129400 billion.

## Accumulate four linear face-gradient sums instead of nine vertex terms

The per-ray face-vertex gradient is linear in a 3-vector Cb and a scalar numb. So the backward chain kernels now accumulate only those four sums per face, in a smaller LDS buffer with fewer atomics, instead of all nine vertex terms. The parameter-face backward kernel expands the four sums into the nine vertex gradients once per face using the face vertices. This cuts the atomic traffic and LDS footprint of the hot backward pass, at the cost of extra recomputation in the gather kernel and a new code path limited to chain, non-deterministic, coherent mode.

```diff
diff --git a/include/tfrt_hip.h b/include/tfrt_hip.h
--- a/include/tfrt_hip.h
+++ b/include/tfrt_hip.h
@@ -75,6 +75,7 @@
   const int32_t* corner_list;
   int64_t n_vertices;
   double* grad_parameters;
+  const double* grad_face_sums;
 } tfrt_face_surface_grad;
 int tfrt_param_faces_forward_multi(const tfrt_face_surface* surfaces, int32_t n_surfaces,
                                    void* stream);
@@ -157,6 +158,7 @@
   int32_t in_place;
   const int32_t* ray_slot;
   const int32_t* wave_schedule;
+  int32_t face_sums;
 } tfrt_scene3d;
 
 typedef struct tfrt_ray_out {
diff --git a/tensorflowraytrace_amd/_lib.py b/tensorflowraytrace_amd/_lib.py
--- a/tensorflowraytrace_amd/_lib.py
+++ b/tensorflowraytrace_amd/_lib.py
@@ -26,6 +26,7 @@
         ("deterministic", c_i32), ("coherent_rays", c_i32), ("coherent_only", c_i32),
         ("grad_n_in", c_vp), ("grad_n_out", c_vp), ("clear_buffer", c_vp), ("clear_count", c_i64),
         ("in_place", c_i32), ("ray_slot", c_vp), ("wave_schedule", c_vp),
+        ("face_sums", c_i32),
     ]
 
 
@@ -60,7 +61,7 @@
                 ("face_verts", ctypes.c_void_p), ("update_mask", ctypes.c_void_p),
                 ("vectors", ctypes.c_void_p), ("corner_start", ctypes.c_void_p),
                 ("corner_list", ctypes.c_void_p), ("n_vertices", ctypes.c_int64),
-                ("grad_parameters", ctypes.c_void_p)]
+                ("grad_parameters", ctypes.c_void_p), ("grad_face_sums", ctypes.c_void_p)]
 
 
 class GoalPending(ctypes.Structure):
diff --git a/tensorflowraytrace_amd/csrc/tfrt_faces.hip b/tensorflowraytrace_amd/csrc/tfrt_faces.hip
--- a/tensorflowraytrace_amd/csrc/tfrt_faces.hip
+++ b/tensorflowraytrace_amd/csrc/tfrt_faces.hip
@@ -101,9 +101,19 @@
 
 __device__ inline void face_grad(const double* __restrict__ g_fverts,
                                  const double* __restrict__ g_norm,
-                                 const double* __restrict__ fverts, int64_t f, double g[9]) {
-#pragma unroll
-  for (int q = 0; q < 9; ++q) g[q] = g_fverts ? g_fverts[9 * f + q] : 0.0;
+                                 const double* __restrict__ fverts, int64_t f, double g[9],
+                                 const double* __restrict__ g_fsums = nullptr) {
+  if (g_fsums != nullptr) {
+    double P[9], S[4];
+#pragma unroll
+    for (int q = 0; q < 9; ++q) P[q] = fverts[9 * f + q];
+#pragma unroll
+    for (int q = 0; q < 4; ++q) S[q] = g_fsums[9 * f + q];
+    face_sums_expand(P, S, g);
+  } else {
+#pragma unroll
+    for (int q = 0; q < 9; ++q) g[q] = g_fverts ? g_fverts[9 * f + q] : 0.0;
+  }
   if (g_norm != nullptr) {
     double P[9], N[3], C[3], clen;
 #pragma unroll
@@ -261,7 +271,7 @@
       const int fc = u.corner_list[q], f = fc / 3, c = fc - 3 * f;
       if (u.update_mask != nullptr && u.update_mask[fc] == 0) continue;
       double g[9];
-      face_grad(u.grad_face_verts, u.grad_norm, u.face_verts, f, g);
+      face_grad(u.grad_face_verts, u.grad_norm, u.face_verts, f, g, u.grad_face_sums);
       acc += g[3 * c] * u.vectors[3 * v] + g[3 * c + 1] * u.vectors[3 * v + 1] +
              g[3 * c + 2] * u.vectors[3 * v + 2];
     }
@@ -455,7 +465,9 @@
     if (u.n_vertices < 0) return TFRT_E_BADARG;
     if (u.n_vertices > 0 &&
         (!u.vectors || !u.grad_parameters || !u.corner_start || !u.corner_list ||
-         (!u.grad_face_verts && !u.grad_norm) || (u.grad_norm && !u.face_verts)))
+         (!u.grad_face_verts && !u.grad_norm && !u.grad_face_sums) ||
+         (u.grad_face_verts && u.grad_face_sums) ||
+         ((u.grad_norm || u.grad_face_sums) && !u.face_verts)))
       return TFRT_E_BADARG;
     b.s[k] = u;
     blocks += cdiv(u.n_vertices * GATHER_LANES, BLOCK);
diff --git a/tensorflowraytrace_amd/csrc/tfrt_trace3d.hip b/tensorflowraytrace_amd/csrc/tfrt_trace3d.hip
--- a/tensorflowraytrace_amd/csrc/tfrt_trace3d.hip
+++ b/tensorflowraytrace_amd/csrc/tfrt_trace3d.hip
@@ -2542,34 +2542,54 @@
     int64_t out_stride, double gP[9]);
 
 
-constexpr int WSUM_SLOTS = 32, WSUM_CELLS = 592;
-__device__ __forceinline__ constexpr int wsum_stride(int copies) {
-  return WSUM_SLOTS * 9 * 2 / copies + 2;
-}
-static_assert(8 * wsum_stride(8) <= WSUM_CELLS && 4 * wsum_stride(4) <= WSUM_CELLS &&
-              2 * wsum_stride(2) <= WSUM_CELLS, "wacc holds every tier");
-
+constexpr int WSUM_SLOTS = 32, WSUM_ROW = 9;
+template <int TERMS>
+constexpr int wsum_stride(int copies) {
+  return WSUM_SLOTS * TERMS * 2 / copies + 2;
+}
+template <int TERMS>
+constexpr int wsum_cells() {
+  return 8 * wsum_stride<TERMS>(8);
+}
+template <int TERMS>
+struct WsumCheck {
+  static_assert(TERMS == 9 || TERMS == 4, "nine face-vertex terms or the four sums");
+  static_assert(4 * wsum_stride<TERMS>(4) <= wsum_cells<TERMS>() &&
+                    2 * wsum_stride<TERMS>(2) <= wsum_cells<TERMS>(),
+                "wacc holds every tier");
+  static_assert(wsum_stride<TERMS>(8) % 4 == 2 && wsum_stride<TERMS>(4) % 4 == 2 &&
+                    wsum_stride<TERMS>(2) % 4 == 2,
+                "the copies of one cell lie in different LDS banks");
+  static_assert(wsum_cells<TERMS>() % 2 == 0, "cleared two cells at a time");
+  static constexpr bool ok = true;
+};
+constexpr int WSUM_CELLS = wsum_cells<9>();
+static_assert(WSUM_CELLS == 592 && wsum_cells<4>() == 272 && WsumCheck<9>::ok && WsumCheck<4>::ok,
+              "the tiers of wave_face_sums");
+
+template <int TERMS>
 __device__ __forceinline__ void wsum_clear(double* wacc) {
-  for (int k = 2 * (threadIdx.x & 63); k < WSUM_CELLS; k += 128)
+  for (int k = 2 * (threadIdx.x & 63); k < wsum_cells<TERMS>(); k += 128)
     *reinterpret_cast<double2*>(wacc + k) = make_double2(0.0, 0.0);
   wave_fence();
 }
-template <int COPIES>
+template <int COPIES, int TERMS>
 __device__ __forceinline__ void wsum_fold(double* wacc, const int32_t* wface, int K, int lane,
                                           double* __restrict__ g_fverts) {
   for (int k = lane; k < K; k += 64) {
     double* w = wacc + k;
     double v = w[0];
 #pragma unroll
-    for (int c = 1; c < COPIES; ++c) v += w[c * wsum_stride(COPIES)];
-#pragma unroll
-    for (int c = 0; c < COPIES; ++c) w[c * wsum_stride(COPIES)] = 0.0;
+    for (int c = 1; c < COPIES; ++c) v += w[c * wsum_stride<TERMS>(COPIES)];
+#pragma unroll
+    for (int c = 0; c < COPIES; ++c) w[c * wsum_stride<TERMS>(COPIES)] = 0.0;
     if (v != 0.0) {
-      const int f = k / 9;
-      unsafeAtomicAdd(g_fverts + 9 * (int64_t)wface[f] + (k - 9 * f), v);
-    }
-  }
-}
+      const int f = k / TERMS;
+      unsafeAtomicAdd(g_fverts + WSUM_ROW * (int64_t)wface[f] + (k - TERMS * f), v);
+    }
+  }
+}
+template <int TERMS>
 __device__ __forceinline__ void wave_face_sums(int tri, const double gP[9], double* wacc,
                                                int32_t* wface, double* __restrict__ g_fverts) {
   const int lane = threadIdx.x & 63;
@@ -2588,21 +2608,21 @@
   const int copies = ns <= 8 ? 8 : (ns <= 16 ? 4 : 2);
   if (tri >= 0) {
     if (slot >= 0) {
-      double* w = &wacc[(lane & (copies - 1)) * wsum_stride(copies) + slot * 9];
-#pragma unroll
-      for (int c = 0; c < 9; ++c)
+      double* w = &wacc[(lane & (copies - 1)) * wsum_stride<TERMS>(copies) + slot * TERMS];
+#pragma unroll
+      for (int c = 0; c < TERMS; ++c)
         if (gP[c] != 0.0) unsafeAtomicAdd(w + c, gP[c]);
     } else {
-      double* gp = g_fverts + 9 * (int64_t)tri;
-#pragma unroll
-      for (int c = 0; c < 9; ++c)
+      double* gp = g_fverts + WSUM_ROW * (int64_t)tri;
+#pragma unroll
+      for (int c = 0; c < TERMS; ++c)
         if (gP[c] != 0.0) unsafeAtomicAdd(gp + c, gP[c]);
     }
   }
   wave_fence();
-  if (copies == 8) wsum_fold<8>(wacc, wface, ns * 9, lane, g_fverts);
-  else if (copies == 4) wsum_fold<4>(wacc, wface, ns * 9, lane, g_fverts);
-  else wsum_fold<2>(wacc, wface, ns * 9, lane, g_fverts);
+  if (copies == 8) wsum_fold<8, TERMS>(wacc, wface, ns * TERMS, lane, g_fverts);
+  else if (copies == 4) wsum_fold<4, TERMS>(wacc, wface, ns * TERMS, lane, g_fverts);
+  else wsum_fold<2, TERMS>(wacc, wface, ns * TERMS, lane, g_fverts);
   wave_fence();
 }
 
@@ -2629,7 +2649,7 @@
     __shared__ __align__(16) double wacc[BW][WSUM_CELLS];
     __shared__ int32_t wface[BW][WSUM_SLOTS];
     const int wave = threadIdx.x >> 6;
-    wsum_clear(wacc[wave]);
+    wsum_clear<9>(wacc[wave]);
     double gP[9];
     int tri = -1;
     if (i < n)
@@ -2637,7 +2657,7 @@
                             pass_counts, sc, L, dead_len, g_child, child_stride, g_fin, cap_fin,
                             g_act, cap_act, g_stp, cap_stp, g_dead, cap_dead, g_out, g_src_out,
                             out_stride, gP);
-    wave_face_sums(tri, gP, wacc[wave], wface[wave], g_fverts);
+    wave_face_sums<9>(tri, gP, wacc[wave], wface[wave], g_fverts);
     return;
   }
   if (i >= n) return;
@@ -2795,7 +2815,7 @@
   if (i == 0) *max_next = 0ull;
 }
 
-template <typename T, bool GN = true>
+template <typename T, bool GN = true, int TERMS = 9>
 __device__ __forceinline__ int backward_core(
     int i, int tape, int slot, const T* __restrict__ rays_in, int64_t stride_in,
     const int32_t* __restrict__ ray_id_in, const int32_t* __restrict__ rec_tri,
@@ -2877,7 +2897,7 @@
       const bool want_n = GN && has_child && sc.grad_n_in != nullptr && sc.n_table == nullptr;
       const int branch = ((tape & TAPE_INTERNAL) ? 1 : 0) | ((tape & TAPE_REFLECT) ? 2 : 0);
       adjoint3d(s, e, P, t_rec, has_child, n_in, n_out, L, g_s, g_h, g_ce, gs, ge, gP, gn, branch,
-                want_n);
+                want_n, true, nullptr, TERMS == 4);
       if (want_n) {
         if (gn[0] != 0.0) unsafeAtomicAdd(sc.grad_n_in + tri, gn[0]);
         if (gn[1] != 0.0) unsafeAtomicAdd(sc.grad_n_out + tri, gn[1]);
@@ -2888,7 +2908,7 @@
   return face_out;
 }
 
-template <bool FIN = true, bool CHILD = true>
+template <bool FIN = true, bool CHILD = true, int TERMS = 9>
 __device__ __forceinline__ int backward_core_loaded(
     int tape, int tri, bool child_pass, const double s[3], const double e[3], const double P[9],
     double t_rec, double n_a, double n_b, bool face_wanted, double L, const double child[6],
@@ -2917,7 +2937,7 @@
       const int branch = ((tape & TAPE_INTERNAL) ? 1 : 0) | ((tape & TAPE_REFLECT) ? 2 : 0);
       const double ratios[2] = {n_a, n_b};
       adjoint3d(s, e, P, t_rec, has_child, 1.0, 1.0, L, g_s, g_h, g_ce, gs, ge, gP, nullptr,
-                branch, false, face_wanted, ratios);
+                branch, false, face_wanted, ratios, TERMS == 4);
       if (face_wanted) face_out = tri;
     }
   }
@@ -3000,7 +3020,7 @@
 #ifndef TFRT_CHAIN_WAVES
 #define TFRT_CHAIN_WAVES 4
 #endif
-template <typename T, int BW, bool GOAL, bool GN>
+template <typename T, int BW, bool GOAL, bool GN, int TERMS>
 __global__ __launch_bounds__(64 * BW)
 __attribute__((amdgpu_waves_per_eu(TFRT_CHAIN_WAVES, TFRT_CHAIN_WAVES))) void k_backward_chain(
     ChainArgs<T> a, tfrt_scene3d sc) {
@@ -3014,13 +3034,13 @@
     }
     return;
   }
-  __shared__ __align__(16) double wacc[BW][WSUM_CELLS];
+  __shared__ __align__(16) double wacc[BW][wsum_cells<TERMS>()];
   __shared__ int32_t wface[BW][WSUM_SLOTS];
   extern __shared__ int4 chain_lds[];
   const int lane = threadIdx.x & 63, wave = threadIdx.x >> 6;
   const int P = a.P;
   int4* chain = chain_lds + (size_t)wave * P * 64;
-  wsum_clear(wacc[wave]);
+  wsum_clear<TERMS>(wacc[wave]);
   int last = -1;
   if (i0 < n0) {
     int j = i0;
@@ -3091,7 +3111,7 @@
         }
       }
       double gs[3], ge[3];
-      tri = backward_core<T, GN>(j, tape, slot, rin, sin, idin, a.rec_tri + off, a.rec_t + off,
+      tri = backward_core<T, GN, TERMS>(j, tape, slot, rin, sin, idin, a.rec_tri + off, a.rec_t + off,
                                  a.counts + (size_t)p * TFRT_COUNTS_PER_PASS, sc, a.L, a.dead_len,
                                  p < P - 1, child, GOAL ? seed : nullptr, a.g_fin, a.cap_fin, a.g_act,
                              a.cap_act, a.g_stp, a.cap_stp, a.g_dead, a.cap_dead, gs, ge, gP,
@@ -3105,7 +3125,7 @@
       n_fin += __popcll(__ballot(fin_here));
       n_entered += __popcll(__ballot(p <= last));
     }
-    wave_face_sums(tri, gP, wacc[wave], wface[wave], a.g_fverts);
+    wave_face_sums<TERMS>(tri, gP, wacc[wave], wface[wave], a.g_fverts);
   }
   if (a.g_src != nullptr && i0 < n0) {
     for (int k = 0; k < 6; ++k) a.g_src[k * a.N + i0] = child[k];
@@ -3178,7 +3198,7 @@
   return ld_scalar_base(base, (unsigned long long)(i * (uint32_t)sizeof(U)));
 }
 
-template <typename T, bool FIN, bool CHILD>
+template <typename T, bool FIN, bool CHILD, int TERMS>
 __device__ __forceinline__ int chain_goal_pass(const ChainGoalArgs<T>& a, int p, int wave, int lane,
                                                int tape, int face, bool fin_lane, double child[6],
                                                double& err, double gP[9]) {
@@ -3271,7 +3291,7 @@
     }
   }
   double gs[3], ge[3];
-  const int tri = backward_core_loaded<FIN, CHILD>(tape, face, child_pass, s0, e0, Pf, t_rec, n_a,
+  const int tri = backward_core_loaded<FIN, CHILD, TERMS>(tape, face, child_pass, s0, e0, Pf, t_rec, n_a,
                                                    n_b, mask_i != 0, a.L, child, seed, gs, ge, gP);
   for (int k = 0; k < 3; ++k) {
     child[k] = gs[k];
@@ -3280,7 +3300,7 @@
   return tri;
 }
 
-template <typename T>
+template <typename T, int TERMS>
 __global__ __launch_bounds__(64)
 __attribute__((amdgpu_waves_per_eu(TFRT_CHAIN_WAVES, TFRT_CHAIN_WAVES))) void k_backward_chain_goal_inplace(
     ChainGoalArgs<T> a) {
@@ -3301,11 +3321,11 @@
     return;
   }
   __builtin_assume(a.feta != nullptr);
-  __shared__ __align__(16) double wacc[WSUM_CELLS];
+  __shared__ __align__(16) double wacc[wsum_cells<TERMS>()];
   __shared__ int32_t wface[WSUM_SLOTS];
   extern __shared__ int2 chain_goal_lds[];
   int2* chain = chain_goal_lds;
-  wsum_clear(wacc);
+  wsum_clear<TERMS>(wacc);
   const int P = a.P;
   int last = -1;
   if (i0 < n0) {
@@ -3338,12 +3358,12 @@
     const unsigned long long fin_m = __ballot(fin_here);
     const bool fin_role = here && fin_m != 0ull && !(p < P - 1 && (tape & 3) == CLS_ACTIVE);
     if (fin_role)
-      tri = chain_goal_pass<T, true, false>(a, p, wave, lane, tape, face, fin_here, child, err, gP);
+      tri = chain_goal_pass<T, true, false, TERMS>(a, p, wave, lane, tape, face, fin_here, child, err, gP);
     if (here && !fin_role)
-      tri = chain_goal_pass<T, false, true>(a, p, wave, lane, tape, face, false, child, err, gP);
+      tri = chain_goal_pass<T, false, true, TERMS>(a, p, wave, lane, tape, face, false, child, err, gP);
     n_fin += __popcll(fin_m);
     n_entered += __popcll(__ballot(here));
-    wave_face_sums(tri, gP, wacc, wface, a.g_fverts);
+    wave_face_sums<TERMS>(tri, gP, wacc, wface, a.g_fverts);
   }
   if (a.g_src != nullptr && i0 < n0) {
     for (int k = 0; k < 6; ++k) a.g_src[k * a.N + i0] = child[k];
@@ -4056,8 +4076,6 @@
   const bool ordered = sc->deterministic != 0 && M > 0 && c.g_fverts != nullptr;
   const bool wave_sums = !ordered && sc->coherent_rays != 0 && M > 0 && c.g_fverts != nullptr;
   const bool stash = ordered || (!wave_sums && M > 0 && N >= 16384 && windows <= 32);
-  if (ordered)
-    (void)hipMemsetAsync(fix_acc, 0, lay.total - lay.fix_acc, st);
   int acc_chunk = 8192;
   while (acc_chunk > 1024 && (int64_t)cdiv(N, acc_chunk) * windows < 256) acc_chunk /= 2;
 
@@ -4073,21 +4091,30 @@
   if (chain && tape_mode == 3 &&
       (c.g_act || c.g_stp || c.g_dead || c.goal != nullptr || c.cap_fin < N))
     return TFRT_E_BADARG;
+  const bool four_sums = sc->face_sums != 0;
+  if (four_sums && !chain) return TFRT_E_UNSUPPORTED;
+  if (ordered)
+    (void)hipMemsetAsync(fix_acc, 0, lay.total - lay.fix_acc, st);
 
   if (chain) {
     const ChainArgs<T> a = chain_args_of<T>(c, tape, tape_mode);
     ProfScope prof_bwd(TFRT_PROF_BACKWARD, st);
     if (N > 0 && goal_inplace) {
-      hipLaunchKernelGGL((k_backward_chain_goal_inplace<T>), dim3(cdiv(N, 64)), dim3(64),
+      using Kernel = void (*)(ChainGoalArgs<T>);
+      const Kernel kernel[2] = {k_backward_chain_goal_inplace<T, 9>,
+                                k_backward_chain_goal_inplace<T, 4>};
+      hipLaunchKernelGGL(kernel[four_sums], dim3(cdiv(N, 64)), dim3(64),
                          (size_t)P * 64 * sizeof(int2), st, chain_goal_args_of(a, sc));
     } else if (N > 0) {
       using Kernel = void (*)(ChainArgs<T>, tfrt_scene3d);
-      const Kernel kernel[2][2] = {
-          {k_backward_chain<T, 1, false, false>, k_backward_chain<T, 1, false, true>},
-          {k_backward_chain<T, 1, true, false>, k_backward_chain<T, 1, true, true>}};
+      const Kernel kernel[2][2][2] = {
+          {{k_backward_chain<T, 1, false, false, 9>, k_backward_chain<T, 1, false, false, 4>},
+           {k_backward_chain<T, 1, false, true, 9>, k_backward_chain<T, 1, false, true, 4>}},
+          {{k_backward_chain<T, 1, true, false, 9>, k_backward_chain<T, 1, true, false, 4>},
+           {k_backward_chain<T, 1, true, true, 9>, k_backward_chain<T, 1, true, true, 4>}}};
       const size_t chain_lds = a.chain_in_lds ? (size_t)P * 64 * sizeof(int4) : 0;
-      hipLaunchKernelGGL(kernel[c.goal != nullptr][sc->grad_n_in != nullptr], dim3(cdiv(N, 64)),
-                         dim3(64), chain_lds, st, a, *sc);
+      hipLaunchKernelGGL(kernel[c.goal != nullptr][sc->grad_n_in != nullptr][four_sums],
+                         dim3(cdiv(N, 64)), dim3(64), chain_lds, st, a, *sc);
     }
     return hipGetLastError() == hipSuccess ? 0 : TFRT_E_LAUNCH;
   }
diff --git a/tensorflowraytrace_amd/csrc/trace_math.h b/tensorflowraytrace_amd/csrc/trace_math.h
--- a/tensorflowraytrace_amd/csrc/trace_math.h
+++ b/tensorflowraytrace_amd/csrc/trace_math.h
@@ -230,12 +230,32 @@
 #endif
 }
 
+TFRT_HD void face_terms_of(const double E1[3], const double E2[3], const double C[3],
+                           const double Cb[3], double numb, double g[9]) {
+  double E1b[3], E2b[3];
+  adj_cross3(E2, Cb, E1b);
+  adj_cross3(Cb, E1, E2b);
+  for (int i = 0; i < 3; ++i) {
+    g[3 + i] = E1b[i];
+    g[6 + i] = E2b[i];
+    g[i] = numb * C[i] - (E1b[i] + E2b[i]);
+  }
+}
+
+TFRT_HD void face_sums_expand(const double P[9], const double S[4], double g[9]) {
+  const double E1[3] = {P[3] - P[0], P[4] - P[1], P[5] - P[2]};
+  const double E2[3] = {P[6] - P[0], P[7] - P[1], P[8] - P[2]};
+  double C[3];
+  adj_cross3(E1, E2, C);
+  face_terms_of(E1, E2, C, S, S[3], g);
+}
+
 TFRT_HD void adjoint3d(const double s[3], const double e[3], const double P[9], double ray_u,
                        bool has_child, double n_in, double n_out, double L,
                        const double g_s[3], const double g_h[3], const double g_ce[3],
                        double gs[3], double ge[3], double gP[9], double* gn = nullptr,
                        int branch = -1, bool gn_wanted = true, bool face_terms = true,
-                       const double* ratios = nullptr) {
+                       const double* ratios = nullptr, bool face_sums = false) {
   if (gn != nullptr) gn[0] = gn[1] = 0.0;
   const double d[3] = {e[0] - s[0], e[1] - s[1], e[2] - s[2]};
   const double E1[3] = {P[3] - P[0], P[4] - P[1], P[5] - P[2]};
@@ -341,13 +361,11 @@
   if (face_terms) {
     double Cb[3];
     for (int i = 0; i < 3; ++i) Cb[i] = Cn[i] + (numb * (P[i] - s[i]) + denb * d[i]);
-    double E1b[3], E2b[3];
-    adj_cross3(E2, Cb, E1b);
-    adj_cross3(Cb, E1, E2b);
-    for (int i = 0; i < 3; ++i) {
-      gP[3 + i] = E1b[i];
-      gP[6 + i] = E2b[i];
-      gP[i] = numb * C[i] - (E1b[i] + E2b[i]);
+    if (face_sums) {
+      for (int i = 0; i < 3; ++i) gP[i] = Cb[i];
+      gP[3] = numb;
+    } else {
+      face_terms_of(E1, E2, C, Cb, numb, gP);
     }
   }
   for (int i = 0; i < 3; ++i) {
diff --git a/tensorflowraytrace_amd/fused_step.py b/tensorflowraytrace_amd/fused_step.py
--- a/tensorflowraytrace_amd/fused_step.py
+++ b/tensorflowraytrace_amd/fused_step.py
@@ -1,3 +1,4 @@
+import contextlib
 import ctypes
 import gc
 
@@ -593,6 +594,7 @@
     fold_backward = True
     folded_backward = False
     in_place = False
+    face_sums = False
     capture_collective = "auto"
     collective_in_graph = False
     schedule_min_waves = None
@@ -787,10 +789,11 @@
         self.folded_backward, self.in_place = folded, inplace
         st.perm = perm
         st.inplace = (block, self._lengths()[1]) if inplace else None
+        four = self.face_sums = self._four_sums(fv, sc, folded)
         clear = {"clear_buffer": st.g_fv.data_ptr(), "clear_count": st.g_fv.numel()} if folded \
             else {}
         sched = self._wave_schedule(st) if inplace else None
-        with _override(sc, in_place=1 if inplace else 0,
+        with _override(sc, in_place=1 if inplace else 0, face_sums=1 if four else 0,
                        wave_schedule=None if sched is None else sched.data_ptr()):
             with _override(sc, **clear):
                 self._trace_forward(st, sc, st.no_outs if inplace else st.outs)
@@ -800,7 +803,13 @@
             self._make_wave_schedule(st, perm)
         if not need_back:
             return None, st
-        return self._parameter_gradients(*self._outs3d(fv, st, index), tap_log), st
+        with ops.FaceSums() if four else contextlib.nullcontext():
+            return self._parameter_gradients(*self._outs3d(fv, st, index), tap_log), st
+
+    @staticmethod
+    def _four_sums(fv, sc, chain_sweep):
+        return bool(chain_sweep and not sc.deterministic and sc.coherent_rays
+                    and fv.requires_grad and ops.faces_from_param_update(fv))
 
     def _wave_schedule(self, st):
         given = self.opt.engine.wave_schedule
@@ -943,10 +952,11 @@
         self.folded_backward, self.in_place = False, True
         self._goal_pending = None
         st.perm, st.inplace = perm, (block, self._lengths()[1])
+        four = self.face_sums = self._four_sums(fv, sc, need_back)
         clear = {"clear_buffer": st.g_fv.data_ptr(), "clear_count": st.g_fv.numel()} if need_back \
             else {}
         grads = None
-        with _override(sc, in_place=2, **clear):
+        with _override(sc, in_place=2, face_sums=1 if four else 0, **clear):
             self._trace_forward(st, sc, st.row_outs)
             if isinstance(self.opt.error_function, (DensityError, SpotError)):
                 if isinstance(self.opt.error_function, DensityError):
@@ -960,7 +970,8 @@
             if g64 is not None:
                 with self._index_grads3d(sc, st, True):
                     self._trace3d_backward(st, sc, g64, g64.shape[1])
-                grads = self._parameter_gradients(*self._outs3d(fv, st, index), tap_log)
+                with ops.FaceSums() if four else contextlib.nullcontext():
+                    grads = self._parameter_gradients(*self._outs3d(fv, st, index), tap_log)
         return grads, st
 
     def _density_seeds3d(self, st, src, perm):
diff --git a/tensorflowraytrace_amd/ops.py b/tensorflowraytrace_amd/ops.py
--- a/tensorflowraytrace_amd/ops.py
+++ b/tensorflowraytrace_amd/ops.py
@@ -219,7 +219,10 @@
             if gp is None:
                 gp = torch.empty(shape, dtype=torch.float64, device=fv.device)
             d = _lib.FaceSurfaceGrad()
-            d.grad_face_verts = g_fv.data_ptr() + at * 72 if g_fv is not None else None
+            if g_fv is not None and FaceSums._active is not None:
+                d.grad_face_sums = g_fv.data_ptr() + at * 72
+            else:
+                d.grad_face_verts = g_fv.data_ptr() + at * 72 if g_fv is not None else None
             d.grad_norm = _p(g_norm)
             d.face_verts = fv.data_ptr() + at * 72
             d.update_mask, d.vectors = _p(mask), _p(vectors)
@@ -267,6 +270,24 @@
 
     def holds(self, t):
         return any(v.data_ptr() == t.data_ptr() and v.numel() == t.numel() for v in self.taken)
+
+
+class FaceSums:
+
+    _active = None
+
+    def __enter__(self):
+        self._prev, FaceSums._active = FaceSums._active, self
+        return self
+
+    def __exit__(self, *exc):
+        FaceSums._active = self._prev
+        return False
+
+
+def faces_from_param_update(fv):
+    fn = getattr(fv, "grad_fn", None)
+    return fn is not None and getattr(fn, "_forward_cls", None) is _ParamFacesMulti
 
 
 def current_faces_batch():
```

Measured after the change: 131600 billion (median of 6 runs). +1.7%, better.
